# thucz/splatter360

Measured on AMD Instinct MI355X. Metric: Msplats/s fwd+bwd @1M Gaussians, 1024x512 ERP, higher is better.
Workload: dtype f32; 1 GPU; BASELINE configs[2]: 1048576 encoder-like synthetic Gaussians (seed 0, deg-4 SH, from 2 context panoramas 1024x512), 1024x512 ERP = 6 faces 256x256 + stitch, fwdbwd, L2 loss on faces (fused epilogue, scalar reduced in the backward's first launch), lean tile lists; gaussians=1048576, face=256, views_per_gpu=1, parallelism=view-sharded x1, num_rendered=2237238, visible_pairs=1096454, split_lists=auto, split_quadrants=0, wide_rectangles=0, workspace_bytes_forward=1086434304, workspace_bytes_backward=1062934272, max_instances=2862083

## Files before the change

include/s360.h:

```cpp
#ifndef S360_H
#define S360_H

#include <stddef.h>
#include <stdint.h>

#ifdef __cplusplus
extern "C" {
#endif

#define S360_ABI_VERSION 24
#define S360_MAX_VIEWS 8
#define S360_TILE 16

enum {
    S360_OK = 0,
    S360_E_BADARG = -1,
    S360_E_WORKSPACE = -2,
    S360_E_LAUNCH = -3,
    S360_E_UNSUPPORTED = -4
};

#define S360_FLAG_SHARED_CAMPOS 1u
#define S360_FLAG_FORWARD_ONLY 8u
#define S360_FLAG_COV9 2u
#define S360_FLAG_SH_CHANNEL_MAJOR 4u

#define S360_FLAG_SH_DEG4_IGNORED 16u

#define S360_FLAG_SPHERICAL 32u

#define S360_FLAG_LEAN_LISTS 64u

#define S360_FLAG_DEFER_LOSS 128u

#define S360_FLAG_ATOMIC_GRADS 256u

#define S360_FLAG_SPLIT_LISTS 512u

#define S360_FLAG_RAW_INPUTS 1024u

#define S360_FLAG_COOP_WALK 2048u

typedef struct S360View {
    float viewmatrix[16];
    float projmatrix[16];
    float campos[3];
    float tanfovx, tanfovy;
    float bg[3];
    float scale;
    float near_plane, far_plane;
    float _pad;
} S360View;

typedef struct S360Params {
    int32_t P;
    int32_t V;
    int32_t H, W;
    int32_t sh_degree;
    int32_t M;
    uint32_t flags;
    uint32_t max_instances;
    uint32_t max_segments;
    uint32_t _reserved;
    void* header_mirror;
} S360Params;

typedef struct S360Layout {
    size_t total_bytes;
    size_t header;
    size_t tiles_touched;
    size_t vis_mask;
    size_t slot_base;
    size_t rec_a;
    size_t rec_b;
    size_t rec_c;
    size_t clamped;
    size_t depths;
    size_t tile_count;
    size_t slot_ticket;
    size_t merge_done;
    size_t seg_flag;
    size_t seg_arrive;
    size_t seg_arrive2;
    size_t tile_start;
    size_t tile_cursor;
    size_t chunk_start;
    size_t tile_order;
    size_t keys;
    size_t keys_alt;
    size_t list;
    size_t final_T;
    size_t n_contrib;
    size_t tile_max_contrib;
    size_t strip_last;
    size_t slot_pair;
    size_t long_pairs;
    size_t rgbc;
    size_t sh_jac;
    size_t surv;
    size_t surv_count;
    size_t part_c;
    size_t part_t;
    size_t part_e;
    size_t part_l;
    size_t part_n;
    size_t seg_c;
    size_t seg_t;
    size_t seg_cnt;
    size_t seg_info;
    size_t geo7;
    size_t backward_bytes;
} S360Layout;

typedef struct S360RawInputs {
    const float* extrinsics;
    const float* depths;
    const float* raw_gaussians;
    const float* sh_rotation;
    int32_t n_views, per_view;
    int32_t H, W, per_ray;
    int32_t erp_convention;
    float scale_min, scale_max, eps;
} S360RawInputs;

int s360_abi_version(void);
const char* s360_error_string(int code);

int s360_layout(const S360Params* prm, S360Layout* out);

int s360_forward(const S360Params* prm, const S360View* views, const float* means3D,
                 const float* cov6, const float* opacities, const float* shs,
                 const float* colors_precomp, float* images, int32_t* radii, void* workspace,
                 size_t workspace_bytes, void* stream);

#define S360_DEPTH_DEPTH 0
#define S360_DEPTH_DISPARITY 1
#define S360_DEPTH_RELATIVE_DISPARITY 2
#define S360_DEPTH_LOG 3
int s360_forward_depth(const S360Params* prm, const S360View* views, const float* means3D,
                       const float* cov6, const float* opacities, const float* shs,
                       const float* colors_precomp, float* images, float* depth_maps, int32_t depth_mode,
                       int32_t* radii, void* workspace, size_t workspace_bytes, void* stream);

int s360_forward_mse(const S360Params* prm, const S360View* views, const float* means3D,
                     const float* cov6, const float* opacities, const float* shs,
                     const float* colors_precomp, float* images, float* depth_maps, int32_t depth_mode,
                     int32_t* radii, const float* target, float grad_scale, float* d_images, float* partials,
                     float* loss_out, void* workspace, size_t workspace_bytes, void* stream);

int s360_backward(const S360Params* prm, const S360View* views, const float* means3D,
                  const float* cov6, const float* opacities, const float* shs,
                  const float* colors_precomp, const void* workspace, size_t workspace_bytes,
                  const float* dL_dimages, const float* dL_dimages_scale,
                  const float* dL_ddepth, int32_t depth_mode, float* d_means3D, float* d_means2D,
                  float* d_cov6, float* d_opacities, float* d_shs, float* d_colors, void* bwd_workspace,
                  size_t bwd_workspace_bytes, void* stream);

int s360_backward_split(const S360Params* prm, const S360View* views, const float* means3D,
                        const float* cov6, const float* opacities, const float* shs,
                        const void* workspace, size_t workspace_bytes,
                        const float* dL_dimages, const float* dL_dimages_scale, const float* dL_ddepth,
                        int32_t depth_mode, float* d_means3D, float* d_means2D, float* d_cov6,
                        float* d_opacities, float* d_rgb_sum, void* bwd_workspace,
                        size_t bwd_workspace_bytes, void* stream);
int s360_sh_backward(const S360Params* prm, int32_t n_groups, const S360View* views,
                     const float* means3D, const float* d_rgb_sums , float* d_shs,
                     void* stream);

int s360_backward_composite(const S360Params* prm, const S360View* views, const void* workspace, size_t workspace_bytes,
                            const float* dL_dimages, const float* dL_dimages_scale, const float* dL_ddepth, int32_t depth_mode,
                            void* bwd_workspace, size_t bwd_workspace_bytes, void* stream);
int s360_backward_gaussians(const S360Params* prm, const S360View* views, const float* means3D, const float* cov6,
                            const float* shs, const void* workspace, size_t workspace_bytes, int32_t with_depth,
                            int32_t depth_mode, int32_t g_begin, int32_t g_count, int32_t rank_stamp, float* d_packed,
                            float* d_means2D, float* d_rgb_sum, void* bwd_workspace, size_t bwd_workspace_bytes, void* stream);
int s360_unpack_gradients(const float* packed, int32_t P, int32_t cov9, float* d_means3D, float* d_cov, float* d_opacities,
                          void* stream);
int s360_reduce_unpack_gradients(const float* packed_blocks, int32_t n_blocks, int32_t g_begin, int32_t g_count, int32_t cov9,
                                 float* d_means3D, float* d_cov, float* d_opacities, void* stream);

int s360_pack_views(const float* extrinsics, const float* intrinsics, const float* near_planes,
                    const float* far_planes, const float* background, int32_t background_per_view,
                    int32_t n_views, int32_t scale_invariant, S360View* views_out, void* stream);
// ... 79 lines not shown
```

splatter360_amd/_lib.py:

```python
from __future__ import annotations

import ctypes as C
import os
import shutil
import subprocess
from pathlib import Path

_PKG = Path(__file__).resolve().parent
_CSRC = _PKG / "csrc"
LIB_PATH = _PKG / "libs360.so"
SOURCES = ("s360_forward.hip", "s360_backward.hip", "s360_backward_em.hip", "s360_stitch.hip", "s360_views.hip", "s360_adapter.hip", "s360_metrics.hip",
           "s360_depth_loss.hip", "s360_eval_scores.hip", "s360_cost_volume.hip")
SOURCE_FLAGS = {"s360_backward_em.hip": ("-fno-slp-vectorize",)}
HIPCC_FLAGS = ("--offload-arch=gfx950", "-O3", "-std=c++17", "-ffp-contract=off", "-fPIC", "-Wno-unused-result")

S360_MAX_VIEWS = 8
FLAG_SHARED_CAMPOS = 1
FLAG_COV9 = 2
FLAG_SH_CHANNEL_MAJOR = 4
FLAG_FORWARD_ONLY = 8
FLAG_SH_DEG4_IGNORED = 16
FLAG_SPHERICAL = 32
FLAG_LEAN_LISTS = 64
FLAG_DEFER_LOSS = 128
FLAG_ATOMIC_GRADS = 256
FLAG_SPLIT_LISTS = 512
FLAG_RAW_INPUTS = 1024
FLAG_COOP_WALK = 2048
ABI_VERSION = 24


class S360Params(C.Structure):
    _fields_ = [("P", C.c_int32), ("V", C.c_int32), ("H", C.c_int32), ("W", C.c_int32),
                ("sh_degree", C.c_int32), ("M", C.c_int32), ("flags", C.c_uint32),
                ("max_instances", C.c_uint32), ("max_segments", C.c_uint32), ("_reserved", C.c_uint32),
                ("header_mirror", C.c_void_p)]


class S360Layout(C.Structure):
    _fields_ = [(n, C.c_size_t) for n in (
        "total_bytes", "header", "tiles_touched", "vis_mask", "slot_base", "rec_a", "rec_b", "rec_c",
        "clamped", "depths", "tile_count", "slot_ticket", "merge_done", "seg_flag", "seg_arrive", "seg_arrive2", "tile_start", "tile_cursor", "chunk_start", "tile_order", "keys", "keys_alt", "list", "final_T", "n_contrib",
        "tile_max_contrib", "strip_last", "slot_pair", "long_pairs", "rgbc", "sh_jac", "surv", "surv_count", "part_c", "part_t", "part_e", "part_l", "part_n", "seg_c", "seg_t", "seg_cnt", "seg_info", "geo7", "backward_bytes")]


class S360RawInputs(C.Structure):
    _fields_ = [("extrinsics", C.c_void_p), ("depths", C.c_void_p), ("raw_gaussians", C.c_void_p), ("sh_rotation", C.c_void_p),
                ("n_views", C.c_int32), ("per_view", C.c_int32), ("H", C.c_int32), ("W", C.c_int32), ("per_ray", C.c_int32),
                ("erp_convention", C.c_int32), ("scale_min", C.c_float), ("scale_max", C.c_float), ("eps", C.c_float)]


EXPORTS = ("s360_forward_raw", "s360_backward_raw", "s360_backward_raw_tail", "s360_abi_version", "s360_error_string", "s360_layout", "s360_forward", "s360_forward_depth", "s360_forward_mse", "s360_backward", "s360_backward_split", "s360_backward_composite", "s360_backward_gaussians", "s360_unpack_gradients", "s360_reduce_unpack_gradients", "s360_sh_backward", "s360_pack_views", "s360_adapter_forward", "s360_adapter_backward", "s360_sh_rotation_blocks",
           "s360_cube2erp_forward", "s360_cube2erp_backward", "s360_count_contributions", "s360_count_backward_slots", "s360_profile_slots", "s360_profile_slot_name",
           "s360_profile_enable", "s360_profile_collect", "s360_ssim", "s360_erode", "s360_l1_sphere_forward",
           "s360_l1_sphere_backward", "s360_depth_metrics", "s360_psnr", "s360_cost_volume_forward", "s360_cost_volume_backward",
           "s360_cost_volume_warp")


def _hipcc() -> str:
    for cand in (os.environ.get("HIPCC"), shutil.which("hipcc"), "/opt/rocm/bin/hipcc"):
        if cand and Path(cand).exists():
            return cand
    raise RuntimeError("hipcc not found; cannot build libs360.so")


def needs_build() -> bool:
    if not LIB_PATH.exists():
        return True
    t = LIB_PATH.stat().st_mtime
    return any(d.stat().st_mtime > t for d in _dep_files())


def _dep_files():
    return sorted(list(_CSRC.glob("*.hip")) + list(_CSRC.glob("*.h")) + list((_PKG.parent / "include").glob("*.h")))


def source_hash() -> str:
    import hashlib
    h = hashlib.sha256()
    for f in _dep_files():
        h.update(f.name.encode())
        h.update(f.read_bytes())
    return h.hexdigest()[:16]


def build(force: bool = False, verbose: bool = False, out: Path = None, extra=()) -> Path:
    target = LIB_PATH if out is None else Path(out)
    if out is None and not force and not needs_build():
        return LIB_PATH
    extra = [*os.environ.get("S360_HIPCC_EXTRA", "").split(), *extra]
    from concurrent.futures import ThreadPoolExecutor
    objdir = _PKG / "build" if out is None else target.parent / "build"
    objdir.mkdir(parents=True, exist_ok=True)

    def compile_one(src: str):
        obj = objdir / (src + ".o")
        cmd = [_hipcc(), *HIPCC_FLAGS, *SOURCE_FLAGS.get(src, ()), *extra, "-c", str(_CSRC / src), "-o", str(obj)]
        r = subprocess.run(cmd, capture_output=True, text=True)
        return obj, cmd, r

    with ThreadPoolExecutor(max_workers=len(SOURCES)) as pool:
        results = list(pool.map(compile_one, SOURCES))
    for obj, cmd, r in results:
        if verbose or r.returncode:
            print(" ".join(cmd))
            print(r.stdout, r.stderr)
        if r.returncode:
            raise RuntimeError("hipcc failed building libs360.so:\n" + r.stderr[-4000:])
    cmd = [_hipcc(), "--offload-arch=gfx950", "-shared", "-fPIC", *[str(o) for o, _, _ in results], "-o", str(target)]
    r = subprocess.run(cmd, capture_output=True, text=True)
    if verbose or r.returncode:
        print(" ".join(cmd))
        print(r.stdout, r.stderr)
    if r.returncode:
        raise RuntimeError("hipcc failed linking libs360.so:\n" + r.stderr[-4000:])
    return target


_lib = None


def lib() -> C.CDLL:
    global _lib
    if _lib is not None:
        return _lib
    import torch
# ... 104 lines not shown
```

splatter360_amd/csrc/s360_backward.hip:

```cpp
#include "s360_device.h"
#include "s360_prof.h"
#include "s360_bwd_em.h"
#include "s360_adapter_math.h"

#include <cstdio>
#include <cstdlib>

namespace s360 {

constexpr int GREC = 4 * PREC_F4;

__device__ __forceinline__ void slot_sum(const float4* __restrict__ part, const uint32_t* __restrict__ valid_words, uint32_t i,
                                         float* s) {
    const uint32_t vw4 = valid_words[i];
#pragma unroll
    for (int k = 0; k < 10; ++k) s[k] = 0.f;
#pragma unroll
    for (int q = 0; q < 4; ++q) {
        if ((vw4 >> (8 * q)) & 0xFFu) {
            const float4* r = part + ((size_t)i * 4 + q) * PREC_F4;
            const float4 r0 = r[0], r1 = r[1], r2 = r[2];
            s[0] += r0.x; s[1] += r0.y; s[2] += r0.z; s[3] += r0.w;
            s[4] += r1.x; s[5] += r1.y; s[6] += r1.z; s[7] += r1.w;
            s[8] += r2.x; s[9] += r2.y;
// ... 625 lines not shown
#pragma unroll
            for (int k = 0; k < 25; ++k) orec[k] = acc[k];
        }
    }
    __syncthreads();
    const int nfl = nb * RAWB_C;
    float* dst = rb.d_raw + (size_t)g0 * RAWB_C;
    if ((((uintptr_t)dst) & 15) == 0) {
        const int n4 = nfl >> 2;
        typedef float f4v __attribute__((ext_vector_type(4)));
        for (int i = tid; i < n4; i += 192) __builtin_nontemporal_store(reinterpret_cast<const f4v*>(s_out)[i], reinterpret_cast<f4v*>(dst) + i);
        for (int i = (n4 << 2) + tid; i < nfl; i += 192) dst[i] = s_out[i];
    } else {
        for (int i = tid; i < nfl; i += 192) dst[i] = s_out[i];
    }
}

}

using namespace s360;

#ifdef S360_DEBUG_LAUNCH
#define S360_LAUNCH_DIAG(e) fprintf(stderr, "s360: %s at %s:%d\n", hipGetErrorString(e), __FILE__, __LINE__)
#else
#define S360_LAUNCH_DIAG(e) ((void)0)
#endif
#define S360_CHECK_LAUNCH()                                                                          \
    do {                                                                                             \
        hipError_t e_ = hipGetLastError();                                                           \
        if (e_ != hipSuccess) {                                                                      \
            S360_LAUNCH_DIAG(e_);                                                                    \
            return S360_E_LAUNCH;                                                                    \
        }                                                                                            \
    } while (0)

static int launch_sh_bwd(const KParams& kp, const S360View* views, const float* means3D, const float4* drgb, int n_groups,
                         float* d_shs, hipStream_t st) {
    const int wblk = (kp.P + 63) / 64;
    const size_t wlds = (size_t)64 * kp.M * 3 * 4;
    if (wlds > 64 * 1024) return S360_E_UNSUPPORTED;
    ProfScope ps(PS_SH_BWD, st);
    if (kp.flags & S360_FLAG_SH_CHANNEL_MAJOR)
        hipLaunchKernelGGL((k_sh_bwd<true>), dim3(wblk), dim3(64), wlds, st, kp, views, means3D, drgb, n_groups, d_shs);
    else
        hipLaunchKernelGGL((k_sh_bwd<false>), dim3(wblk), dim3(64), wlds, st, kp, views, means3D, drgb, n_groups, d_shs);
    return S360_OK;
}

struct BwdCtx {
    KParams kp;
    S360Layout L;
    int nt;
    float4* part;
    uint32_t* valid_words;
    uint32_t* order;
    float4* pairgrad;
    uint32_t* seg_list;
    size_t n_slots;
};

static int bwd_ctx(const S360Params* prm, const void* workspace, size_t workspace_bytes, void* bwd_workspace,
                   size_t bwd_workspace_bytes, BwdCtx& c) {
    if (!prm || !workspace || !bwd_workspace) return S360_E_BADARG;
    if (prm->flags & S360_FLAG_FORWARD_ONLY) return S360_E_BADARG;
    int rc = s360_layout(prm, &c.L);
    if (rc) return rc;
    if (workspace_bytes < c.L.total_bytes || bwd_workspace_bytes < c.L.backward_bytes) return S360_E_WORKSPACE;
    KParams& kp = c.kp;
    kp.P = prm->P; kp.V = prm->V; kp.H = prm->H; kp.W = prm->W; kp.deg = s360_effective_degree(prm); kp.M = prm->M;
    kp.gx = (prm->W + 15) / 16; kp.gy = (prm->H + 15) / 16; kp.T = kp.gx * kp.gy;
    kp.flags = prm->flags; kp.cap = prm->max_instances;
    const bool sph = (kp.flags & S360_FLAG_SPHERICAL) != 0;
    if (sph && (kp.V & 1)) return S360_E_BADARG;
    c.nt = (sph ? kp.V / 2 : kp.V) * kp.T;
    if (kp.flags & S360_FLAG_ATOMIC_GRADS) {
        c.part = nullptr;
        c.valid_words = nullptr;
        c.order = (uint32_t*)bwd_workspace;
    } else {
        c.part = (float4*)bwd_workspace;
        c.valid_words = (uint32_t*)((char*)bwd_workspace + (size_t)kp.cap * 4 * GREC * 4);
        c.order = c.valid_words + kp.cap;
    }
    c.pairgrad = (float4*)((char*)(c.order + c.nt * 4) + 256 - ((uintptr_t)(c.order + c.nt * 4) & 255));
    c.seg_list = nullptr;
    c.n_slots = seg_slots_of(prm);
    if (kp.flags & S360_FLAG_SPLIT_LISTS) {
        char* e = (char*)(c.pairgrad + (size_t)kp.V * (kp.P > 0 ? kp.P : 1) * 3 + (size_t)(kp.P > 0 ? kp.P : 1));
        c.seg_list = (uint32_t*)(e + 256 - ((uintptr_t)e & 255)) + 32;
    }
    return S360_OK;
}

static int backward_composite(const BwdCtx& c, const S360View* views, const void* workspace, const float* dL_dimages,
                              const float* dL_dimages_scale, const float* dL_ddepth, int depth_mode, hipStream_t st) {
    const KParams& kp = c.kp;
    const S360Layout& L = c.L;
    const char* ws = (const char*)workspace;
    const uint32_t* header = (const uint32_t*)(ws + L.header);
    const bool with_depth = dL_ddepth != nullptr;
    const uint32_t* surv_count = (const uint32_t*)(ws + L.surv_count);
    SegBwd sb{};
    if (c.seg_list) {
        sb.seg_flag = (const uint32_t*)(ws + L.seg_flag);
        sb.chunk_start = (const uint32_t*)(ws + L.chunk_start);
        sb.seg_c = (const float4*)(ws + L.seg_c);
        sb.seg_t = (const float*)(ws + L.seg_t);
        sb.seg_cnt = (const uint32_t*)(ws + L.seg_cnt);
        sb.seg_info = (const uint2*)(ws + L.seg_info);
        sb.seg_list = c.seg_list;
        sb.n_seg_blocks = (uint32_t)min((size_t)S360_SEG_BWD_BLOCKS, c.n_slots * 4);
        sb.dbg_base = (uint32_t)c.nt * 4u;
    }
    {
        ProfScope ps(PS_ORDER, st);
        hipLaunchKernelGGL(k_order_units, dim3(1 + 512), dim3(1024), 0, st, surv_count, c.order, c.nt * 4, c.valid_words, header, kp.cap,
                           (kp.flags & S360_FLAG_ATOMIC_GRADS) ? c.pairgrad : (float4*)nullptr, (const uint8_t*)(ws + L.vis_mask), kp.P, kp.V,
                           (const uint32_t*)(ws + L.seg_cnt), (const uint32_t*)(ws + L.chunk_start), c.seg_list, (const uint2*)(ws + L.seg_info), sb);
    }
    {
        ProfScope ps(PS_RENDER_BWD, st);
        launch_render_bwd_em(with_depth, c.nt * 4, st, kp, views, (const uint32_t*)(ws + L.tile_start), (const float4*)(ws + L.surv),
                             surv_count, (const uint2*)(ws + L.slot_base), (const float*)(ws + L.depths),
                             (const float*)(ws + L.final_T), (const uint32_t*)(ws + L.n_contrib), dL_dimages, dL_dimages_scale,
                             dL_ddepth, c.part, (uint8_t*)c.valid_words, c.order, depth_mode,
                             (kp.flags & S360_FLAG_ATOMIC_GRADS) ? (float*)c.pairgrad : (float*)nullptr,
#ifdef S360_DBG_TIMING
                             (uint32_t*)(ws + L.keys_alt), c.seg_list ? &sb : (const SegBwd*)nullptr, sb.n_seg_blocks);
#else
                             (uint32_t*)nullptr, c.seg_list ? &sb : (const SegBwd*)nullptr, sb.n_seg_blocks);
#endif
    }
    S360_CHECK_LAUNCH();
    if (kp.flags & S360_FLAG_ATOMIC_GRADS) return S360_OK;
    ProfScope ps(PS_GATHER, st);
    hipLaunchKernelGGL(k_gather_slots, dim3((unsigned)(((size_t)kp.cap + S360_BLOCK - 1) / S360_BLOCK)), dim3(S360_BLOCK), 0, st,
                       kp.cap, header, (const uint32_t*)(ws + L.slot_pair), c.part, c.valid_words, c.pairgrad,
                       (const uint32_t*)(ws + L.long_pairs), (const uint2*)(ws + L.slot_base), (const uint32_t*)(ws + L.tiles_touched));
    S360_CHECK_LAUNCH();
    return S360_OK;
}

static int backward_gaussians(const BwdCtx& c, const S360View* views, const float* means3D, const float* cov6, const float* shs,
                              const void* workspace, bool with_depth, int depth_mode, int g_begin, int g_end, float* d_means3D,
                              float* d_means2D, float* d_cov6, float* d_opacities, float* d_shs, float* d_colors, float* d_rgb_sum,
                              float* d_packed, int view_stamp, hipStream_t st) {
    const KParams& kp = c.kp;
    const S360Layout& L = c.L;
    const char* ws = (const char*)workspace;
    const uint8_t* vis_mask = (const uint8_t*)(ws + L.vis_mask);
    const uint8_t* clamped = (const uint8_t*)(ws + L.clamped);
    const int dmode = with_depth ? depth_mode : -1;
    const int n = g_end - g_begin;
    if (n <= 0) return S360_OK;
    const int nblk = (n + S360_BLOCK - 1) / S360_BLOCK;
    float4* drgb = d_rgb_sum ? (float4*)d_rgb_sum : c.pairgrad + (size_t)kp.V * kp.P * 3;
    if (shs) {
        const bool shared = (kp.flags & S360_FLAG_SHARED_CAMPOS) != 0;
        if ((d_rgb_sum || d_packed) && !shared) return S360_E_UNSUPPORTED;
        if (shared) {
            {
                ProfScope ps(PS_PREPROCESS_BWD, st);
                hipLaunchKernelGGL((k_preprocess_bwd<true, false>), dim3(nblk), dim3(S360_BLOCK), 0, st, kp, views, means3D, cov6, shs,
                                   vis_mask, clamped, c.pairgrad, d_means3D, d_means2D, d_cov6, d_opacities, d_shs,
                                   d_colors, drgb, dmode, (const float*)(ws + L.sh_jac), g_begin, g_end, d_packed, view_stamp);
            }
            if (!d_rgb_sum && d_shs) {
                if (g_begin != 0 || g_end != kp.P) return S360_E_UNSUPPORTED;
                const int rc2 = launch_sh_bwd(kp, views, means3D, drgb, 1, d_shs, st);
                if (rc2) return rc2;
            }
        } else {
            if (g_begin != 0 || g_end != kp.P) return S360_E_UNSUPPORTED;
            size_t lds = (size_t)S360_BLOCK * kp.M * 3 * 4 + (size_t)S360_BLOCK * kp.V * 3 * 4;
            if (lds > 160 * 1024) return S360_E_UNSUPPORTED;
            {
                static bool attr_done[64] = {};
                int dev = 0;
                if (hipGetDevice(&dev) == hipSuccess && dev >= 0 && dev < 64 && !attr_done[dev]) {
                    (void)hipFuncSetAttribute((const void*)k_preprocess_bwd<true, true>, hipFuncAttributeMaxDynamicSharedMemorySize, 160 * 1024);
                    (void)hipGetLastError();
                    attr_done[dev] = true;
                }
            }
            ProfScope ps(PS_PREPROCESS_BWD, st);
            hipLaunchKernelGGL((k_preprocess_bwd<true, true>), dim3(nblk), dim3(S360_BLOCK), lds, st, kp, views, means3D, cov6, shs,
                               vis_mask, clamped, c.pairgrad, d_means3D, d_means2D, d_cov6, d_opacities, d_shs,
                               d_colors, (float4*)nullptr, dmode, (const float*)nullptr, 0, kp.P, (float*)nullptr, -1);
        }
    } else {
        if (d_packed) return S360_E_UNSUPPORTED;
        ProfScope ps(PS_PREPROCESS_BWD, st);
        hipLaunchKernelGGL((k_preprocess_bwd<false, false>), dim3(nblk), dim3(S360_BLOCK), 0, st, kp, views, means3D, cov6, shs,
                           vis_mask, clamped, c.pairgrad, d_means3D, d_means2D, d_cov6, d_opacities, d_shs,
                           d_colors, (float4*)nullptr, dmode, (const float*)nullptr, g_begin, g_end, (float*)nullptr, -1);
    }
    S360_CHECK_LAUNCH();
    return S360_OK;
}

static int backward_impl(const S360Params* prm, const S360View* views, const float* means3D, const float* cov6,
                         const float* opacities, const float* shs, const float* colors_precomp,
                         const void* workspace, size_t workspace_bytes, const float* dL_dimages,
                         const float* dL_dimages_scale, const float* dL_ddepth, int depth_mode, float* d_means3D,
                         float* d_means2D, float* d_cov6, float* d_opacities, float* d_shs, float* d_colors,
                         float* d_rgb_sum, void* bwd_workspace, size_t bwd_workspace_bytes, void* stream_) {
    (void)opacities;
    if (!prm || !views || !workspace || !dL_dimages || !bwd_workspace) return S360_E_BADARG;
    if (prm->flags & S360_FLAG_FORWARD_ONLY) return S360_E_BADARG;
    if (prm->P > 0 && (shs == nullptr) == (colors_precomp == nullptr)) return S360_E_BADARG;
    if (prm->P > 0 && (!means3D || !cov6 || !d_means3D || !d_cov6 || !d_opacities)) return S360_E_BADARG;
    const bool with_depth = dL_ddepth != nullptr;
    if (with_depth && (depth_mode < 0 || depth_mode > 3)) return S360_E_BADARG;
// ... 389 lines not shown
```

splatter360_amd/csrc/s360_backward_em.hip:

```cpp
#define S360_EM_KERNEL_TU 1
#include "s360_bwd_em.h"

namespace s360 {

void launch_render_bwd_em(bool with_depth, int n_units, hipStream_t st, const KParams& kp, const S360View* views,
                          const uint32_t* tile_start, const float4* surv, const uint32_t* surv_count, const uint2* slot_info,
                          const float* depths, const float* final_T, const uint32_t* n_contrib, const float* dL_dimages,
                          const float* dL_dimages_scale, const float* dL_ddepth, float4* part, uint8_t* valid, const uint32_t* order, int depth_mode,
                          float* pairgrad_atomic, uint32_t* dbg, const SegBwd* sbp_host, uint32_t n_seg_blocks) {
    const SegBwd sbv = sbp_host ? *sbp_host : SegBwd{};
#define S360_LAUNCH_BWD(WD, SG)                                                                                                              \
    hipLaunchKernelGGL((k_render_bwd_em<WD, SG>), dim3(n_units + (SG ? n_seg_blocks : 0u)), dim3(64), 0, st, kp, views, tile_start, surv, surv_count, \
                       slot_info, depths, final_T, n_contrib, dL_dimages, dL_dimages_scale, dL_ddepth, part, valid, order, depth_mode,          \
                       pairgrad_atomic, dbg, sbv, SG ? n_seg_blocks : 0u)
    const bool seg = sbp_host != nullptr;
    if (with_depth) { if (seg) S360_LAUNCH_BWD(true, true); else S360_LAUNCH_BWD(true, false); }
    else { if (seg) S360_LAUNCH_BWD(false, true); else S360_LAUNCH_BWD(false, false); }
#undef S360_LAUNCH_BWD
}

}
```

splatter360_amd/csrc/s360_bwd_em.h:

```cpp
#pragma once
#include "s360_device.h"

namespace s360 {

constexpr int EM_QCAP = 128;


#define S360_SCAN4_STEP(op, ctrl)                                                                      \
    op " %0, %0, %0 " ctrl "\n" op " %1, %1, %1 " ctrl "\n" op " %2, %2, %2 " ctrl "\n" op " %3, %3, %3 " ctrl "\n"
#define S360_SCAN4(op, a, b, c, d)                                                        \
    asm volatile("s_nop 1\n"                                                              \
                 S360_SCAN4_STEP(op, "row_shr:1 row_mask:0xf bank_mask:0xf")              \
                 S360_SCAN4_STEP(op, "row_shr:2 row_mask:0xf bank_mask:0xf")              \
                 S360_SCAN4_STEP(op, "row_shr:4 row_mask:0xf bank_mask:0xf")              \
                 S360_SCAN4_STEP(op, "row_shr:8 row_mask:0xf bank_mask:0xf")              \
                 S360_SCAN4_STEP(op, "row_bcast:15 row_mask:0xa bank_mask:0xf")           \
                 S360_SCAN4_STEP(op, "row_bcast:31 row_mask:0xc bank_mask:0xf")           \
                 "s_nop 1\n"                                                              \
                 : "+v"(a), "+v"(b), "+v"(c), "+v"(d))

__device__ __forceinline__ void wave_shr1x4_zero(float& a, float& b, float& c, float& d) {
    float oa, ob, oc, od;
    asm volatile("s_nop 1\n"
                 "v_mov_b32_dpp %0, %4 wave_shr:1 row_mask:0xf bank_mask:0xf bound_ctrl:0\n"
                 "v_mov_b32_dpp %1, %5 wave_shr:1 row_mask:0xf bank_mask:0xf bound_ctrl:0\n"
                 "v_mov_b32_dpp %2, %6 wave_shr:1 row_mask:0xf bank_mask:0xf bound_ctrl:0\n"
                 "v_mov_b32_dpp %3, %7 wave_shr:1 row_mask:0xf bank_mask:0xf bound_ctrl:0\n"
                 : "=&v"(oa), "=&v"(ob), "=&v"(oc), "=&v"(od)
                 : "v"(a), "v"(b), "v"(c), "v"(d));
    a = oa; b = ob; c = oc; d = od;
}
__device__ __forceinline__ void wave_one_minus_shr1x4(float a, float b, float c, float d, float& oa, float& ob, float& oc,
                                                      float& od) {
    const float one = 1.0f;
    asm volatile("s_nop 1\n"
                 "v_subrev_f32_dpp %0, %4, %8 wave_shr:1 row_mask:0xf bank_mask:0xf bound_ctrl:0\n"
                 "v_subrev_f32_dpp %1, %5, %8 wave_shr:1 row_mask:0xf bank_mask:0xf bound_ctrl:0\n"
                 "v_subrev_f32_dpp %2, %6, %8 wave_shr:1 row_mask:0xf bank_mask:0xf bound_ctrl:0\n"
                 "v_subrev_f32_dpp %3, %7, %8 wave_shr:1 row_mask:0xf bank_mask:0xf bound_ctrl:0\n"
                 : "=&v"(oa), "=&v"(ob), "=&v"(oc), "=&v"(od)
                 : "v"(a), "v"(b), "v"(c), "v"(d), "v"(one));
}

__device__ __forceinline__ void wave_scan4_mul(float& a, float& b, float& c, float& d) { S360_SCAN4("v_mul_f32_dpp", a, b, c, d); }
__device__ __forceinline__ void wave_scan4_add(float& a, float& b, float& c, float& d) { S360_SCAN4("v_add_f32_dpp", a, b, c, d); }

__device__ __forceinline__ float depth_value_grad(float z, float nearp, float farp, int mode) {
    if (mode == 1) return -1.0f / (z * z);
    if (mode == 2) {
        const float eps = 1e-10f;
        const float disp_near = 1.0f / (nearp + eps), disp_far = 1.0f / (farp + eps), disp = 1.0f / (z + eps);
        return (disp * disp) / (disp_near - disp_far + eps);
    }
    if (mode == 3) return (z < nearp && z > farp) ? 1.0f / z : 0.0f;
    return 1.0f;
}

typedef SegBwdPod SegBwd;

#ifdef S360_EM_KERNEL_TU
template <bool WITH_DEPTH, bool SEG>
__global__ __launch_bounds__(64) void k_render_bwd_em(
    KParams kp, const S360View* __restrict__ views, const uint32_t* __restrict__ tile_start,
    const float4* __restrict__ surv, const uint32_t* __restrict__ surv_count, const uint2* __restrict__ slot_info,
    const float* __restrict__ depths, const float* __restrict__ final_T, const uint32_t* __restrict__ n_contrib,
    const float* __restrict__ dL_dimages, const float* __restrict__ dL_dimages_scale, const float* __restrict__ dL_ddepth,
    float4* __restrict__ part,
    uint8_t* __restrict__ valid, const uint32_t* __restrict__ order, int depth_mode, float* __restrict__ pairgrad_atomic,
    uint32_t* __restrict__ dbg, SegBwd sb, uint32_t n_seg_blocks) {
    static_assert(SUB_W == 8, "entry-major backward assumes 8x8 quadrants");
    __shared__ __attribute__((aligned(16))) float s_gr[64], s_gg[64], s_gb[64], s_gd[64];
    __shared__ __attribute__((aligned(16))) float s_T[64], s_R[64];
    __shared__ __attribute__((aligned(16))) float s_B[64];
    __shared__ __attribute__((aligned(16))) uint32_t s_last[64];

    const bool seg_blk = SEG && blockIdx.x < n_seg_blocks;
    const int lane = threadIdx.x;
  for (uint32_t sj = blockIdx.x;; sj += n_seg_blocks) {
#ifdef S360_DBG_TIMING
    const long long t_begin = wall_clock64();
#endif
    uint32_t unit, n_surv, kseg = 0;
    bool split_unit = false;
    size_t sli = 0;
    if (seg_blk) {
        if (sj >= sb.seg_list[0]) return;
        uint2 info = sb.seg_info[sb.seg_list[1 + sj]];
        info.y &= ~S360_SEG_CLAIM;
        unit = 4u * info.x + (info.y & 3u);
        kseg = info.y >> 2;
        const size_t su = ((size_t)SEG_PER_CHUNK * sb.chunk_start[info.x] + kseg) * 4 + (info.y & 3u);
        n_surv = sb.seg_cnt[su];
        split_unit = true;
        sli = su * 64;
    } else {
        unit = order ? order[blockIdx.x - n_seg_blocks] : blockIdx.x - n_seg_blocks;
        n_surv = surv_count[unit];
        if (n_surv == 0) return;
        if (SEG && sb.seg_flag[unit] == 1u) {
            split_unit = true;
            sli = ((size_t)SEG_PER_CHUNK * sb.chunk_start[unit >> 2] * 4 + (unit & 3u)) * 64;
        }
    }
    const int t = (int)(unit >> 2), wave = (int)(unit & 3u);
    const int v = t / kp.T, rem = t - v * kp.T;
    const int ty = rem / kp.gx, tx = rem - ty * kp.gx;
    const int qx = tx * 16 + sub_ox(wave), qy = ty * 16 + sub_oy(wave);
    const uint32_t start = min(tile_start[t], kp.cap), end = min(tile_start[t + 1], kp.cap);
    const float4* const sv = surv + 3 * ((size_t)4 * start + (size_t)wave * (end - start) + (size_t)kseg * SEG_LEN);
    const S360View& vw = views[view_of_image(kp, v)];

    int64_t top = (int64_t)n_surv - 1;
    float4 na = make_float4(0.f, 0.f, 0.f, 0.f), nb = na, nc = na;
    if (top - lane >= 0) {
        const float4* r = sv + 3 * (size_t)(top - lane);
        na = r[0]; nb = r[1]; nc = r[2];
    }

    {
        const int px = qx + (lane & 7), py = qy + (lane >> 3);
        const size_t hw = (size_t)kp.H * kp.W;
        float4 pa = make_float4(0.f, 0.f, 0.f, 0.f), pb = make_float4(1.0f, 0.f, 0.f, 0.f);
        uint32_t last = 0;
        if (px < kp.W && py < kp.H) {
            const size_t pix = (size_t)py * kp.W + px;
            const float T_final = final_T[(size_t)v * hw + pix];
            last = n_contrib[(size_t)v * hw + pix];
            const float* dimg = dL_dimages + (size_t)v * 3 * hw;
            const float gs = dL_dimages_scale ? *dL_dimages_scale : 1.0f;
            pa.x = dimg[pix] * gs;
            pa.y = dimg[hw + pix] * gs;
            pa.z = dimg[2 * hw + pix] * gs;
            if (WITH_DEPTH) pa.w = dL_ddepth[(size_t)v * hw + pix];
            pb.x = T_final;
            pb.z = T_final * (vw.bg[0] * pa.x + vw.bg[1] * pa.y + vw.bg[2] * pa.z);
            if (SEG && split_unit) {
                const float4 cb = sb.seg_c[sli + lane];
                pb.x = sb.seg_t[sli + lane];
                float r0 = cb.z * pa.z + (cb.y * pa.y + cb.x * pa.x);
                if (WITH_DEPTH) r0 = cb.w * pa.w + r0;
                pb.y = r0;
            }
        }
        s_gr[lane] = pa.x; s_gg[lane] = pa.y; s_gb[lane] = pa.z;
        if (WITH_DEPTH) s_gd[lane] = pa.w;
        s_T[lane] = pb.x; s_R[lane] = pb.y; s_B[lane] = pb.z;
        s_last[lane] = last;
    }
    f2 pxc[4];
#pragma unroll
    for (int c = 0; c < 4; ++c) pxc[c] = f2{(float)(qx + 2 * c), (float)(qx + 2 * c + 1)};
    const float inv_scale = WITH_DEPTH ? 1.0f / vw.scale : 0.f;
    const float v_near = WITH_DEPTH ? vw.near_plane : 0.f, v_far = WITH_DEPTH ? vw.far_plane : 0.f;

#ifdef S360_DBG_TIMING
    uint32_t dbg_halves = 0;
#endif
    for (; top >= 0; top -= 64) {
        const uint32_t n = (uint32_t)(top + 1 < 64 ? top + 1 : 64);
        const float4 qa = na, qb = nb, qc = nc;
        if (top - 64 - lane >= 0) {
            const float4* r = sv + 3 * (size_t)(top - 64 - lane);
            na = r[0]; nb = r[1]; nc = r[2];
        }
        const bool lane_ok = (uint32_t)lane < n;
        const float ex = qa.x, ey = qa.y, cA = qa.z, cB = qa.w, cC = qb.x, op = qb.y, c0 = qb.z, c1 = qb.w, c2 = qc.x;
        const int erad = __float_as_int(qc.y);
        const uint32_t pos = lane_ok ? __float_as_uint(qc.z) : 0xFFFFFFFFu;
        const uint32_t pair = __float_as_uint(qc.w);
        uint2 sinfo = make_uint2(0u, 0u);
        float zv = 0.f;
        if (lane_ok) {
            if (!pairgrad_atomic) sinfo = slot_info[pair];
            if (WITH_DEPTH) zv = depth_value(depths[pair] * inv_scale, v_near, v_far, depth_mode);
        }
        const uint32_t pos_min = (uint32_t)__builtin_amdgcn_readlane((int)pos, (int)n - 1);
        f2 g_op = f2{0.f, 0.f}, X = g_op, Y = g_op, XX = g_op, XY = g_op, YY = g_op, g_r = g_op, g_g = g_op, g_b = g_op, g_z = g_op;
        bool anyc = false;
        uint32_t qmask;
        {
            const uint4 l4 = *reinterpret_cast<const uint4*>(&s_last[(lane & 15) * 4]);
            qmask = (uint32_t)__ballot(max(max(l4.x, l4.y), max(l4.z, l4.w)) > pos_min) & 0xFFFFu;
        }
        const f2 ex2 = f2{ex, ex}, cA2 = f2{cA, cA}, cB2 = f2{cB, cB}, op2 = f2{op, op}, c02 = f2{c0, c0}, c12 = f2{c1, c1},
                 c22 = f2{c2, c2}, zv2 = f2{zv, zv}, one2 = f2{1.0f, 1.0f};
#pragma unroll 1
        for (int row = 0; row < 8; ++row) {
            const float pyf = (float)(qy + row);
            const float dy = ey - pyf;
            const float cdy = cC * dy;
            const float cdy2 = cdy * dy;
            const float cdy_2 = 2.0f * cdy;
            const f2 dy2 = f2{dy, dy}, cdy2_2 = f2{cdy2, cdy2}, cdy_22 = f2{cdy_2, cdy_2};
#pragma unroll
            for (int half = 0; half < 2; ++half) {
                const int p0 = row * 8 + half * 4;
                if (!((qmask >> (row * 2 + half)) & 1u)) continue;
#ifdef S360_DBG_TIMING
                ++dbg_halves;
#endif
                const float4 vr = *reinterpret_cast<const float4*>(&s_gr[p0]), vg = *reinterpret_cast<const float4*>(&s_gg[p0]),
                             vb = *reinterpret_cast<const float4*>(&s_gb[p0]), vT = *reinterpret_cast<const float4*>(&s_T[p0]),
                             vR = *reinterpret_cast<const float4*>(&s_R[p0]), vB = *reinterpret_cast<const float4*>(&s_B[p0]);
                const uint4 vL = *reinterpret_cast<const uint4*>(&s_last[p0]);
                float4 vd = make_float4(0.f, 0.f, 0.f, 0.f);
                if (WITH_DEPTH) vd = *reinterpret_cast<const float4*>(&s_gd[p0]);
                const f2 gr[2] = {f2{vr.x, vr.y}, f2{vr.z, vr.w}}, gg[2] = {f2{vg.x, vg.y}, f2{vg.z, vg.w}},
                         gb[2] = {f2{vb.x, vb.y}, f2{vb.z, vb.w}}, gd[2] = {f2{vd.x, vd.y}, f2{vd.z, vd.w}},
                         Tr[2] = {f2{vT.x, vT.y}, f2{vT.z, vT.w}}, Rr[2] = {f2{vR.x, vR.y}, f2{vR.z, vR.w}},
                         Bg[2] = {f2{vB.x, vB.y}, f2{vB.z, vB.w}};
                const uint32_t lastk[4] = {vL.x, vL.y, vL.z, vL.w};
                f2 dx[2], pxd[2], Gm[2], a2[2];
                float a[4];
#pragma unroll
                for (int j = 0; j < 2; ++j) {
                    dx[j] = ex2 - pxc[half * 2 + j];
                    const f2 adx = cA2 * dx[j];
                    const f2 tq = pk_fma(cB2, dy2, adx);
                    pxd[j] = tq + adx;
                    const f2 pw = pk_fma(tq, dx[j], cdy2_2);
                    const f2 G = f2{__builtin_amdgcn_exp2f(pw.x), __builtin_amdgcn_exp2f(pw.y)};
                    const f2 og = op2 * G;
                    const float al0 = fminf(0.99f, og.x), al1 = fminf(0.99f, og.y);
                    const bool act0 = pos < lastk[2 * j] && !(pw.x > 0.0f) && !(al0 < 1.0f / 255.0f);
                    const bool act1 = pos < lastk[2 * j + 1] && !(pw.y > 0.0f) && !(al1 < 1.0f / 255.0f);
// ... 6 lines not shown
                float Qx[4];
                wave_one_minus_shr1x4(a[0], a[1], a[2], a[3], Qx[0], Qx[1], Qx[2], Qx[3]);
                wave_scan4_mul(Qx[0], Qx[1], Qx[2], Qx[3]);
                f2 Tj[2], rc[2], cdp[2], w[2];
                float S[4];
#pragma unroll
                for (int j = 0; j < 2; ++j) {
                    const f2 Qx2 = f2{Qx[2 * j], Qx[2 * j + 1]};
                    const f2 Q = Qx2 * (one2 - a2[j]);
                    f2 r = f2{__builtin_amdgcn_rcpf(Q.x), __builtin_amdgcn_rcpf(Q.y)};
                    r = pk_fma(pk_fma(-Q, r, one2), r, r);
                    Tj[j] = Tr[j] * r;
                    rc[j] = Qx2 * r;
                    f2 d = pk_fma(c22, gb[j], pk_fma(c12, gg[j], c02 * gr[j]));
                    if (WITH_DEPTH) d = pk_fma(zv2, gd[j], d);
                    cdp[j] = d;
                    w[j] = a2[j] * Tj[j];
                    const f2 s2 = w[j] * d;
                    S[2 * j] = s2.x;
                    S[2 * j + 1] = s2.y;
                }
                wave_scan4_add(S[0], S[1], S[2], S[3]);
                float Sx[4] = {S[0], S[1], S[2], S[3]};
                wave_shr1x4_zero(Sx[0], Sx[1], Sx[2], Sx[3]);
#pragma unroll
                for (int j = 0; j < 2; ++j) {
                    const f2 Rj = Rr[j] + f2{Sx[2 * j], Sx[2 * j + 1]};
                    const f2 dLda = pk_fma(Tj[j], cdp[j], -((Rj + Bg[j]) * rc[j]));
                    g_op = pk_fma(Gm[j], dLda, g_op);
                    const f2 h = (op2 * dLda) * Gm[j];
                    const f2 hx = h * dx[j], hy = h * dy2;
                    X = pk_fma(h, pxd[j], X);
                    Y = pk_fma(h, pk_fma(cB2, dx[j], cdy_22), Y);
                    XX = pk_fma(hx, dx[j], XX);
                    XY = pk_fma(hx, dy2, XY);
                    YY = pk_fma(hy, dy2, YY);
                    g_r = pk_fma(w[j], gr[j], g_r);
                    g_g = pk_fma(w[j], gg[j], g_g);
                    g_b = pk_fma(w[j], gb[j], g_b);
                    if (WITH_DEPTH) g_z = pk_fma(w[j], gd[j], g_z);
                }
                if (lane == 63) {
                    *reinterpret_cast<float4*>(&s_T[p0]) = make_float4(Tj[0].x, Tj[0].y, Tj[1].x, Tj[1].y);
                    *reinterpret_cast<float4*>(&s_R[p0]) = make_float4(vR.x + S[0], vR.y + S[1], vR.z + S[2], vR.w + S[3]);
                }
            }
        }
        if (pairgrad_atomic) {
            if (lane_ok && anyc) {
                const float ln2 = 0.6931471805599453f;
                float* pg = pairgrad_atomic + 12 * (size_t)pair;
                unsafeAtomicAdd(pg + 0, ln2 * (X.x + X.y));
                unsafeAtomicAdd(pg + 1, ln2 * (Y.x + Y.y));
                unsafeAtomicAdd(pg + 2, -0.5f * (XX.x + XX.y));
                unsafeAtomicAdd(pg + 3, -(XY.x + XY.y));
                unsafeAtomicAdd(pg + 4, -0.5f * (YY.x + YY.y));
                unsafeAtomicAdd(pg + 5, g_op.x + g_op.y);
                unsafeAtomicAdd(pg + 6, g_r.x + g_r.y);
                unsafeAtomicAdd(pg + 7, g_g.x + g_g.y);
                unsafeAtomicAdd(pg + 8, g_b.x + g_b.y);
                if (WITH_DEPTH) unsafeAtomicAdd(pg + 9, g_z.x + g_z.y);
            }
            continue;
        }
        uint32_t inst = 0xFFFFFFFFu;
        if (lane_ok && anyc) {
            int minx, miny, maxx, maxy;
            tile_rect(ex, ey, erad, kp.gx, kp.gy, minx, miny, maxx, maxy);
            const uint32_t idx = (uint32_t)((ty - miny) * (maxx - minx) + (tx - minx));
            const bool masked = (kp.flags & S360_FLAG_LEAN_LISTS) && (maxx - minx) * (maxy - miny) <= 32;
            inst = sinfo.x + (masked ? (uint32_t)__builtin_popcount(sinfo.y & ((1u << idx) - 1u)) : idx);
        }
        if (lane_ok && anyc && inst < kp.cap) {
            const float ln2 = 0.6931471805599453f;
            float4* o = part + ((size_t)inst * 4 + wave) * PREC_F4;
            o[0] = make_float4(ln2 * (X.x + X.y), ln2 * (Y.x + Y.y), -0.5f * (XX.x + XX.y), -(XY.x + XY.y));
            o[1] = make_float4(-0.5f * (YY.x + YY.y), g_op.x + g_op.y, g_r.x + g_r.y, g_g.x + g_g.y);
            o[2] = make_float4(g_b.x + g_b.y, g_z.x + g_z.y, 0.f, 0.f);
            valid[(size_t)inst * 4 + wave] = 1;
        }
    }
#ifdef S360_DBG_TIMING
    if (lane == 0 && dbg) {
        const size_t di = seg_blk ? (size_t)sb.dbg_base + sb.seg_list[1 + sj] : (size_t)unit;
        dbg[4 * di] = (uint32_t)t_begin;
        dbg[4 * di + 1] = (uint32_t)(wall_clock64() - t_begin);
        dbg[4 * di + 2] = n_surv;
        dbg[4 * di + 3] = (dbg_halves << 16) | min(n_surv, 65535u);
    }
#endif
    if (!SEG || !seg_blk) return;
  }
}
#endif

void launch_render_bwd_em(bool with_depth, int n_units, hipStream_t st, const KParams& kp, const S360View* views,
                          const uint32_t* tile_start, const float4* surv, const uint32_t* surv_count, const uint2* slot_info,
                          const float* depths, const float* final_T, const uint32_t* n_contrib, const float* dL_dimages,
                          const float* dL_dimages_scale, const float* dL_ddepth, float4* part, uint8_t* valid, const uint32_t* order, int depth_mode,
                          float* pairgrad_atomic, uint32_t* dbg, const SegBwd* sbp_host, uint32_t n_seg_blocks);

}
```

splatter360_amd/csrc/s360_device.h:

```cpp
#pragma once
#include <hip/hip_runtime.h>
#include <stdint.h>

#include "../../include/s360.h"

#define S360_WAVE 64
#define S360_BLOCK 256

#ifndef S360_SUB_W
#define S360_SUB_W 8
#endif

static inline int s360_effective_degree(const S360Params* prm) {
    return (prm->sh_degree > 3 && (prm->flags & S360_FLAG_SH_DEG4_IGNORED)) ? 3 : prm->sh_degree;
}

#ifndef S360_PREC_F4
#define S360_PREC_F4 4
#endif

namespace s360 {

constexpr int PREC_F4 = S360_PREC_F4;
constexpr int SUB_W = S360_SUB_W, SUB_H = 64 / S360_SUB_W;
__device__ __forceinline__ int sub_ox(int w) { return SUB_W == 16 ? 0 : 8 * (w & 1); }
__device__ __forceinline__ int sub_oy(int w) { return SUB_W == 16 ? 4 * w : 8 * (w >> 1); }


struct KParams {
    int P, V, H, W, deg, M;
    int gx, gy, T;
    uint32_t flags, cap;
};

#ifndef S360_SEG_LEN
#define S360_SEG_LEN 512
#endif
#ifndef S360_SEG_HEAD
#define S360_SEG_HEAD 1024
#endif
#ifndef S360_SEG_BWD_BLOCKS
#define S360_SEG_BWD_BLOCKS 256
#endif
#ifndef S360_SEG_MIN_REST
#define S360_SEG_MIN_REST 512
#endif
constexpr uint32_t SEG_LEN = S360_SEG_LEN, SEG_HEAD = S360_SEG_HEAD, SEG_MIN_REST = S360_SEG_MIN_REST, SEG_PER_CHUNK = 4096 / SEG_LEN;
constexpr uint32_t SEG_K0 = SEG_HEAD / SEG_LEN;
static_assert(4096 % SEG_LEN == 0 && SEG_HEAD % SEG_LEN == 0 && SEG_LEN % 64 == 0 && SEG_K0 >= 1, "segments tile the sort's 4 096-key chunks; slot 0 holds the head's state");
__device__ constexpr float SEG_T_FAR = 1.0f / 16.0f;
__host__ __device__ inline size_t seg_slots(size_t cap) { return (size_t)SEG_PER_CHUNK * (cap / 2048 + 1); }
__host__ __device__ inline size_t seg_slots_of(const S360Params* prm) {
    return prm->max_segments ? (size_t)prm->max_segments : seg_slots(prm->max_instances ? prm->max_instances : 1);
}
#define S360_HDR_SPLIT 5
#define S360_HDR_SEGWORK 6
#define S360_HDR_TILES_DONE 24
#define S360_HDR_NLONG 25
#define S360_SEG_CLAIM 0x80000000u
#define S360_HDR_SEGBUFS 32

inline int device_cu_count() {
    static int cached[64] = {};
    int dev = 0;
    if (hipGetDevice(&dev) != hipSuccess || dev < 0 || dev >= 64) return 256;
    if (!cached[dev]) {
        int n = 0;
        if (hipDeviceGetAttribute(&n, hipDeviceAttributeMultiprocessorCount, dev) != hipSuccess || n <= 0) { (void)hipGetLastError(); n = 256; }
        cached[dev] = n;
    }
    return cached[dev];
}

inline int resident_blocks(const void* fn, int block_threads, int slot) {
    static int cached[64][16] = {};
    int dev = 0;
    if (hipGetDevice(&dev) != hipSuccess || dev < 0 || dev >= 64 || slot < 0 || slot >= 16) return 4 * 256;
    if (!cached[dev][slot]) {
        int per_cu = 0;
        if (hipOccupancyMaxActiveBlocksPerMultiprocessor(&per_cu, fn, block_threads, 0) != hipSuccess || per_cu <= 0) { (void)hipGetLastError(); per_cu = 4; }
        cached[dev][slot] = per_cu * device_cu_count();
    }
    return cached[dev][slot];
}

__device__ constexpr float kC0 = 0.28209479177387814f;
__device__ constexpr float kC1 = 0.4886025119029199f;
__device__ constexpr float kC2[5] = {1.0925484305920792f, -1.0925484305920792f, 0.31539156525252005f,
                                     -1.0925484305920792f, 0.5462742152960396f};
__device__ constexpr float kC3[7] = {-0.5900435899266435f, 2.890611442640554f, -0.4570457994644658f,
                                     0.3731763325901154f, -0.4570457994644658f, 1.445305721320277f,
                                     -0.5900435899266435f};
__device__ constexpr float kC4[9] = {2.5033429417967046f, -1.7701307697799304f, 0.9461746957575601f,
                                     -0.6690465435572892f, 0.10578554691520431f, -0.6690465435572892f,
                                     0.47308734787878004f, -1.7701307697799304f, 0.6258357354491761f};

__device__ __forceinline__ void sh_basis(int deg, float x, float y, float z, float* Y) {
    Y[0] = kC0;
    if (deg > 0) {
        Y[1] = -kC1 * y;
        Y[2] = kC1 * z;
        Y[3] = -kC1 * x;
        if (deg > 1) {
            float xx = x * x, yy = y * y, zz = z * z, xy = x * y, yz = y * z, xz = x * z;
            Y[4] = kC2[0] * xy;
            Y[5] = kC2[1] * yz;
            Y[6] = kC2[2] * (2.0f * zz - xx - yy);
            Y[7] = kC2[3] * xz;
            Y[8] = kC2[4] * (xx - yy);
            if (deg > 2) {
                Y[9] = kC3[0] * y * (3.0f * xx - yy);
                Y[10] = kC3[1] * xy * z;
                Y[11] = kC3[2] * y * (4.0f * zz - xx - yy);
                Y[12] = kC3[3] * z * (2.0f * zz - 3.0f * xx - 3.0f * yy);
                Y[13] = kC3[4] * x * (4.0f * zz - xx - yy);
                Y[14] = kC3[5] * z * (xx - yy);
                Y[15] = kC3[6] * x * (xx - 3.0f * yy);
                if (deg > 3) {
                    Y[16] = kC4[0] * xy * (xx - yy);
                    Y[17] = kC4[1] * yz * (3.0f * xx - yy);
                    Y[18] = kC4[2] * xy * (7.0f * zz - 1.0f);
                    Y[19] = kC4[3] * yz * (7.0f * zz - 3.0f);
                    Y[20] = kC4[4] * (zz * (35.0f * zz - 30.0f) + 3.0f);
                    Y[21] = kC4[5] * xz * (7.0f * zz - 3.0f);
                    Y[22] = kC4[6] * (xx - yy) * (7.0f * zz - 1.0f);
                    Y[23] = kC4[7] * xz * (xx - 3.0f * yy);
                    Y[24] = kC4[8] * (xx * (xx - 3.0f * yy) - yy * (3.0f * xx - yy));
                }
            }
        }
    }
}

__device__ __forceinline__ void sh_basis_grad(int deg, float x, float y, float z, float* dx, float* dy,
                                              float* dz) {
#pragma unroll
    for (int k = 0; k < 25; ++k) dx[k] = dy[k] = dz[k] = 0.0f;
    if (deg > 0) {
        dy[1] = -kC1;
        dz[2] = kC1;
        dx[3] = -kC1;
        if (deg > 1) {
// ... 271 lines not shown

__device__ __forceinline__ float depth_value(float z, float nearp, float farp, int mode) {
    if (mode == 1) return 1.0f / z;
    if (mode == 2) {
        const float eps = 1e-10f;
        const float disp_near = 1.0f / (nearp + eps), disp_far = 1.0f / (farp + eps), disp = 1.0f / (z + eps);
        return 1.0f - (disp - disp_far) / (disp_near - disp_far + eps);
    }
    if (mode == 3) return __logf(fmaxf(fminf(z, nearp), farp));
    return z;
}

__device__ __forceinline__ void tile_rect(float px, float py, int radius, int gx, int gy, int& minx, int& miny,
                                          int& maxx, int& maxy) {
    const float rr = (float)radius;
    minx = min(gx, max(0, (int)((px - rr) / 16.0f)));
    miny = min(gy, max(0, (int)((py - rr) / 16.0f)));
    maxx = min(gx, max(0, (int)((px + rr + 15.0f) / 16.0f)));
    maxy = min(gy, max(0, (int)((py + rr + 15.0f) / 16.0f)));
}

__device__ __forceinline__ float rl(float v, int l) {
    return __int_as_float(__builtin_amdgcn_readlane(__float_as_int(v), l));
}

__device__ __forceinline__ float wave_sum1_lane63(float a) {
    asm volatile(
        "s_nop 1\n"
        "v_add_f32_dpp %0, %0, %0 quad_perm:[1,0,3,2] row_mask:0xf bank_mask:0xf\n"
        "s_nop 1\n"
        "v_add_f32_dpp %0, %0, %0 quad_perm:[2,3,0,1] row_mask:0xf bank_mask:0xf\n"
        "s_nop 1\n"
        "v_add_f32_dpp %0, %0, %0 row_half_mirror row_mask:0xf bank_mask:0xf\n"
        "s_nop 1\n"
        "v_add_f32_dpp %0, %0, %0 row_mirror row_mask:0xf bank_mask:0xf\n"
        "s_nop 1\n"
        "v_add_f32_dpp %0, %0, %0 row_bcast:15 row_mask:0xa bank_mask:0xf\n"
        "s_nop 1\n"
        "v_add_f32_dpp %0, %0, %0 row_bcast:31 row_mask:0xc bank_mask:0xf\n"
        "s_nop 1\n"
        : "+v"(a));
    return a;
}

__device__ __forceinline__ uint32_t wave_max_u32(uint32_t v) {
#pragma unroll
    for (int o = 32; o > 0; o >>= 1) v = max(v, (uint32_t)__shfl_xor((int)v, o));
    return v;
}

__device__ __forceinline__ int lane_id() { return threadIdx.x & 63; }

template <int THREADS>
__device__ __forceinline__ void order_units_body(const uint32_t* __restrict__ weight, uint32_t* __restrict__ order, int n) {
    __shared__ uint32_t s_max;
    __shared__ uint32_t s_cnt[64];
    __shared__ uint32_t s_base[64];
    if (threadIdx.x == 0) s_max = 1;
    if (threadIdx.x < 64) s_cnt[threadIdx.x] = 0;
    __syncthreads();
    uint32_t mx = 0;
    for (int i = threadIdx.x; i < n; i += THREADS) mx = max(mx, weight[i]);
    mx = wave_max_u32(mx);
    if ((threadIdx.x & 63) == 0) atomicMax(&s_max, mx);
    __syncthreads();
    const uint32_t wmax = s_max;
    for (int i = threadIdx.x; i < n; i += THREADS) atomicAdd(&s_cnt[63 - (uint32_t)(((uint64_t)weight[i] * 63) / wmax)], 1u);
    __syncthreads();
    if (threadIdx.x == 0) {
        uint32_t run = 0;
        for (int b = 0; b < 64; ++b) {
            s_base[b] = run;
            run += s_cnt[b];
        }
    }
    __syncthreads();
    for (int i = threadIdx.x; i < n; i += THREADS) {
        const uint32_t b = 63 - (uint32_t)(((uint64_t)weight[i] * 63) / wmax);
        order[atomicAdd(&s_base[b], 1u)] = (uint32_t)i;
    }
}

template <int THREADS>
__device__ __forceinline__ void order_quadrants_body(const uint32_t* __restrict__ weight, uint32_t* __restrict__ order, int nt) {
    __shared__ uint32_t s_max;
    __shared__ uint32_t s_cnt[64];
    __shared__ uint32_t s_base[64];
    if (threadIdx.x == 0) s_max = 1;
    if (threadIdx.x < 64) s_cnt[threadIdx.x] = 0;
    __syncthreads();
    uint32_t mx = 0;
    for (int i = threadIdx.x; i < nt; i += THREADS) {
        const uint4 w = reinterpret_cast<const uint4*>(weight)[i];
        mx = max(mx, max(max(w.x, w.y), max(w.z, w.w)));
    }
    mx = wave_max_u32(mx);
    if ((threadIdx.x & 63) == 0) atomicMax(&s_max, mx);
    __syncthreads();
    const uint32_t wmax = s_max;
    for (int i = threadIdx.x; i < nt; i += THREADS) {
        const uint4 w = reinterpret_cast<const uint4*>(weight)[i];
        atomicAdd(&s_cnt[63 - (uint32_t)(((uint64_t)max(max(w.x, w.y), max(w.z, w.w)) * 63) / wmax)], 1u);
    }
    __syncthreads();
    if (threadIdx.x == 0) {
        uint32_t run = 0;
        for (int b = 0; b < 64; ++b) {
            s_base[b] = run;
            run += s_cnt[b];
        }
    }
    __syncthreads();
    const uint32_t full = (uint32_t)nt / 8u * 8u, tail = (uint32_t)nt - full;
    for (int i = threadIdx.x; i < nt; i += THREADS) {
        const uint4 w = reinterpret_cast<const uint4*>(weight)[i];
        const uint32_t b = 63 - (uint32_t)(((uint64_t)max(max(w.x, w.y), max(w.z, w.w)) * 63) / wmax);
        const uint32_t r = atomicAdd(&s_base[b], 1u);
#pragma unroll
        for (uint32_t q = 0; q < 4; ++q) {
            const uint32_t slot = r < full ? (r / 8u) * 32u + q * 8u + (r & 7u) : full * 4u + q * tail + (r - full);
            order[slot] = 4u * (uint32_t)i + q;
        }
    }
}

constexpr int MSE_BLOCK = 1024;
__device__ __forceinline__ void mse_finish_body(const float* __restrict__ partials, int n_per_view, int V, float loss_scale,
                                                float inv_elems, float* __restrict__ out) {
    constexpr int VG = 8;
    __shared__ float s_w[MSE_BLOCK / 64][VG][2];
    const int lane = lane_id(), wave = threadIdx.x >> 6;
    float total = 0.f;
    for (int v0 = 0; v0 < V; v0 += VG) {
        float a[VG], b[VG];
#pragma unroll
        for (int j = 0; j < VG; ++j) a[j] = b[j] = 0.f;
        for (int i = threadIdx.x; i < n_per_view; i += MSE_BLOCK) {
            float2 q[VG];
#pragma unroll
            for (int j = 0; j < VG; ++j)
                q[j] = v0 + j < V ? reinterpret_cast<const float2*>(partials)[(size_t)(v0 + j) * n_per_view + i] : make_float2(0.f, 0.f);
#pragma unroll
            for (int j = 0; j < VG; ++j) {
                a[j] += q[j].x;
                b[j] += q[j].y;
            }
        }
#pragma unroll
        for (int j = 0; j < VG; ++j) {
#pragma unroll
            for (int o = 32; o > 0; o >>= 1) {
                a[j] += __shfl_xor(a[j], o);
                b[j] += __shfl_xor(b[j], o);
            }
            if (lane == 0) {
                s_w[wave][j][0] = a[j];
                s_w[wave][j][1] = b[j];
            }
        }
        __syncthreads();
        if (threadIdx.x == 0) {
            for (int j = 0; j < VG && v0 + j < V; ++j) {
                float sa = 0.f, sb = 0.f;
                for (int w = 0; w < MSE_BLOCK / 64; ++w) {
                    sa += s_w[w][j][0];
                    sb += s_w[w][j][1];
                }
                total += sa;
                out[1 + v0 + j] = sb * inv_elems;
            }
        }
        __syncthreads();
    }
    if (threadIdx.x == 0) out[0] = total * loss_scale;
}


#define S360_HDR_LOSS 16

struct SegBwdPod {
    const uint32_t* seg_flag;
    const uint32_t* chunk_start;
    const float4* seg_c;
    const float* seg_t;
    const uint32_t* seg_cnt;
    const uint2* seg_info;
    const uint32_t* seg_list;
    uint32_t n_seg_blocks;
    uint32_t dbg_base;
};
static_assert(sizeof(SegBwdPod) <= 32 * 4, "parked in the 32 words in front of seg_list");

static __global__ __launch_bounds__(1024) void k_order_units(const uint32_t* __restrict__ weight, uint32_t* __restrict__ order, int n,
                                                     uint32_t* __restrict__ valid_words, const uint32_t* __restrict__ header,
                                                     uint32_t cap, float4* __restrict__ pairgrad_atomic,
                                                     const uint8_t* __restrict__ vis_mask, int P, int V,
                                                     const uint32_t* __restrict__ seg_cnt, const uint32_t* __restrict__ chunk_start,
                                                     uint32_t* __restrict__ seg_list, const uint2* __restrict__ seg_info, SegBwdPod sbpod) {
    if (blockIdx.x == 2 && seg_list) {
        if (threadIdx.x == 0) *reinterpret_cast<SegBwdPod*>(seg_list - 32) = sbpod;
        __shared__ uint32_t s_n;
        if (threadIdx.x == 0) s_n = 0u;
        __syncthreads();
        const uint32_t n = header[S360_HDR_SEGWORK];
        for (uint32_t i = threadIdx.x; i < n; i += 1024) {
            uint2 w = seg_info[i];
            w.y &= ~S360_SEG_CLAIM;
            if (seg_cnt[((size_t)SEG_PER_CHUNK * chunk_start[w.x] + (w.y >> 2)) * 4 + (w.y & 3u)]) seg_list[1u + atomicAdd(&s_n, 1u)] = i;
        }
        __syncthreads();
        if (threadIdx.x == 0) seg_list[0] = s_n;
    }
    if (blockIdx.x == 1) {
        const uint64_t pp = (uint64_t)header[S360_HDR_LOSS] | ((uint64_t)header[S360_HDR_LOSS + 1] << 32);
        const uint64_t po = (uint64_t)header[S360_HDR_LOSS + 2] | ((uint64_t)header[S360_HDR_LOSS + 3] << 32);
        if (pp && po)
            mse_finish_body(reinterpret_cast<const float*>(pp), (int)header[S360_HDR_LOSS + 4], (int)header[S360_HDR_LOSS + 5],
                            __uint_as_float(header[S360_HDR_LOSS + 6]), __uint_as_float(header[S360_HDR_LOSS + 7]), reinterpret_cast<float*>(po));
    }
    if (blockIdx.x > 0) {
        const size_t stride = (size_t)(gridDim.x - 1) * 1024;
        if (pairgrad_atomic) {
            const float4 z = make_float4(0.f, 0.f, 0.f, 0.f);
            for (size_t g = (size_t)(blockIdx.x - 1) * 1024 + threadIdx.x; g < (size_t)P; g += stride)
                for (uint32_t m = vis_mask[g]; m; m &= m - 1) {
                    float4* r = pairgrad_atomic + 3 * ((size_t)__builtin_ctz(m) * P + g);
                    r[0] = z; r[1] = z; r[2] = z;
                }
            return;
        }
        const size_t nv = (size_t)min(header[0], cap);
        for (size_t i = (size_t)(blockIdx.x - 1) * 1024 + threadIdx.x; i < nv; i += stride) valid_words[i] = 0u;
        return;
    }
    if (!order) return;
    order_quadrants_body<1024>(weight, order, n / 4);
}


}
```

splatter360_amd/csrc/s360_forward.hip:

```cpp
#include "s360_device.h"
#include "s360_prof.h"
#include "s360_adapter_math.h"

#include <cstdio>
#include <cstdlib>

namespace s360 {

typedef float f4v __attribute__((ext_vector_type(4)));

template <bool CH_MAJOR, bool JAC>
__global__ __launch_bounds__(S360_BLOCK) void k_sh_eval(KParams kp, const S360View* __restrict__ views,
                                                       const float* __restrict__ means, const float* __restrict__ shs,
                                                       float4* __restrict__ rgbc, float* __restrict__ sh_jac,
                                                       uint32_t* __restrict__ zero_ptr, int zero_words) {
    const int g = blockIdx.x * S360_BLOCK + threadIdx.x;
    if (g < zero_words) zero_ptr[g] = 0u;
    if (g >= kp.P) return;
    const bool fast = kp.M == 25 && kp.deg == 4;
    const float* sh = shs + (size_t)g * kp.M * 3;
    float c[75];
    if (fast) load75(sh, c);
    const S360View& vw = views[0];
    const float sc = vw.scale;
// ... 634 lines not shown
constexpr int LDSM_E = 32;
__device__ __forceinline__ uint32_t merge_passes_of(uint32_t nch) { return nch <= 1 ? 0u : nch <= LDSM_CHUNKS ? 1u : ceil_log2_u32(nch); }

struct SegBufs {
    const uint32_t* chunk_start;
    uint32_t* seg_flag;
    uint32_t* seg_arrive;
    uint32_t* seg_arrive2;
    uint32_t n_slots;
    float4* part_c;
    float* part_t;
    float* part_e;
    uint32_t* part_l;
    uint32_t* part_n;
    float4* seg_c;
    float* seg_t;
    uint32_t* seg_cnt;
    uint2* seg_info;
    uint32_t* header;
};
static_assert(sizeof(SegBufs) <= (64 - S360_HDR_SEGBUFS) * 4, "SegBufs is parked in the workspace header");

constexpr int TS_BLOCK = 1024;
__global__ __launch_bounds__(TS_BLOCK) void k_tile_scan(const uint32_t* __restrict__ tile_count, uint32_t* __restrict__ tile_start,
                                                         uint32_t* __restrict__ tile_cursor, uint32_t* __restrict__ tile_max_contrib,
                                                         int nt, uint32_t cap, uint32_t* __restrict__ header,
                                                         uint32_t* __restrict__ chunk_start, unsigned long long* __restrict__ header_mirror,
                                                         SegBufs sg_in) {
    __shared__ uint32_t lds[TS_BLOCK / 64];
    __shared__ uint32_t lds_max, lds_nlong;
    if (threadIdx.x == 0) { lds_max = 0; lds_nlong = 0; }
    __syncthreads();
    uint32_t carry = 0, mx = 0, ccarry = 0;
    for (int b = 0; b < nt; b += 2 * TS_BLOCK) {
        const int i0 = b + 2 * (int)threadIdx.x, i1 = i0 + 1;
        uint32_t v0 = 0u, v1 = 0u;
        if (i1 < nt) {
            const uint2 vv = *reinterpret_cast<const uint2*>(tile_count + i0);
            v0 = vv.x; v1 = vv.y;
        } else if (i0 < nt) {
            v0 = tile_count[i0];
        }
        mx = max(mx, max(v0, v1));
        uint32_t tot;
        const uint32_t ex0 = block_exclusive_scan<TS_BLOCK / 64>(v0 + v1, lds, tot), ex1 = ex0 + v0;
        const uint32_t nc0 = min(carry + ex0 + v0, cap) - min(carry + ex0, cap), nc1 = min(carry + ex1 + v1, cap) - min(carry + ex1, cap);
        const uint32_t nch0 = nc0 > SORT_SHORT ? (nc0 + SORT_CHUNK - 1) / SORT_CHUNK : 0u;
        const uint32_t nch1 = nc1 > SORT_SHORT ? (nc1 + SORT_CHUNK - 1) / SORT_CHUNK : 0u;
        if (nch0 || nch1) atomicAdd(&lds_nlong, (nch0 ? 1u : 0u) + (nch1 ? 1u : 0u));
        uint32_t ctot;
        const uint32_t cex0 = block_exclusive_scan<TS_BLOCK / 64>(nch0 + nch1, lds, ctot), cex1 = cex0 + nch0;
        if (i0 < nt) {
            tile_start[i0] = carry + ex0;
            tile_cursor[i0] = 0;
            tile_max_contrib[i0] = 0;
            chunk_start[i0] = ccarry + cex0;
        }
        if (i1 < nt) {
            tile_start[i1] = carry + ex1;
            tile_cursor[i1] = 0;
            tile_max_contrib[i1] = 0;
            chunk_start[i1] = ccarry + cex1;
        }
        carry += tot;
        ccarry += ctot;
    }
    atomicMax(&lds_max, mx);
    __syncthreads();
    if (threadIdx.x == 0) {
        chunk_start[nt] = ccarry;
        tile_start[nt] = carry;
        header[0] = carry;
        header[1] = carry > cap ? 1u : 0u;
        header[2] = lds_max;
        {
            const uint32_t nmax = min(lds_max, cap);
            const uint32_t nch = nmax > SORT_SHORT ? (nmax + SORT_CHUNK - 1) / SORT_CHUNK : 0u;
            header[3] = merge_passes_of(nch);
        }
        header[4] = 0;
        *reinterpret_cast<SegBufs*>(header + S360_HDR_SEGBUFS) = sg_in;
        header[S360_HDR_SPLIT] = 0;
        header[6] = header[7] = 0;
        if (header_mirror) __hip_atomic_store(header_mirror, (unsigned long long)carry | ((unsigned long long)(carry > cap ? 1u : 0u) << 32) |
                                                             ((unsigned long long)ccarry << 33),
                                              __ATOMIC_RELAXED, __HIP_MEMORY_SCOPE_SYSTEM);
        header[S360_HDR_NLONG] = lds_nlong;
        for (int i = 8; i < 25; ++i) header[i] = 0;
    }
}

#ifndef S360_EMIT_PPT
#define S360_EMIT_PPT 4
#endif
constexpr int EMIT_PPT = S360_EMIT_PPT;

template <bool LDS_BIN, bool COOP = false>
__global__ __launch_bounds__(S360_BLOCK) void k_emit(KParams kp, const uint32_t* __restrict__ tiles_touched,
                                                    const uint8_t* __restrict__ vis_mask, const float4* __restrict__ recA, const float4* __restrict__ recC,
                                                    const float* __restrict__ depths, const uint32_t* __restrict__ tile_start,
                                                    uint32_t* __restrict__ tile_cursor, uint64_t* __restrict__ keys,
                                                    uint2* __restrict__ slot_info, uint32_t* __restrict__ slot_pair,
                                                    uint32_t* __restrict__ slot_ticket, uint32_t* __restrict__ header,
                                                    uint32_t* __restrict__ long_pairs) {
    extern __shared__ __attribute__((aligned(16))) uint32_t lds_bin[];
    __shared__ uint32_t s_scan[S360_BLOCK / 64];
    __shared__ uint32_t s_slot0;
    const int v = blockIdx.y;
    const int g0 = blockIdx.x * (S360_BLOCK * EMIT_PPT) + threadIdx.x;
    const size_t tb = (size_t)image_of_view(kp, v) * kp.T;
    uint32_t* cnt = lds_bin;
    uint32_t* base = lds_bin + kp.T;
    const bool lean = (kp.flags & S360_FLAG_LEAN_LISTS) != 0;
    if (LDS_BIN) {
        for (int i = threadIdx.x; i < kp.T; i += S360_BLOCK) cnt[i] = 0u;
        __syncthreads();
    }
    __shared__ uint32_t s_p[S360_BLOCK * EMIT_PPT];
    uint32_t vis = 0;
#pragma unroll
    for (int j = 0; j < EMIT_PPT; ++j) {
        const int g = g0 + j * S360_BLOCK;
        if (g < kp.P && ((vis_mask[g] >> v) & 1u)) vis |= 1u << j;
    }
    uint32_t nvis;
    {
        uint32_t off = block_exclusive_scan((uint32_t)__builtin_popcount(vis), s_scan, nvis);
        for (uint32_t m = vis; m; m &= m - 1) s_p[off++] = (uint32_t)v * (uint32_t)kp.P + (uint32_t)(g0 + __builtin_ctz(m) * S360_BLOCK);
    }
    __syncthreads();
    uint32_t pr[EMIT_PPT], tt[EMIT_PPT], rlo[EMIT_PPT], rhi[EMIT_PPT], dbits[EMIT_PPT], hm[EMIT_PPT];
#pragma unroll
    for (int j = 0; j < EMIT_PPT; ++j) {
        const uint32_t e = threadIdx.x + j * S360_BLOCK;
        tt[j] = 0u; pr[j] = 0u; rlo[j] = rhi[j] = dbits[j] = 0u; hm[j] = 0xFFFFFFFFu;
        if (e < nvis) {
            const uint32_t p = s_p[e];
            const float4 rc = recA[3 * (size_t)p + 2];
            const float4 ra = recA[3 * (size_t)p];
            pr[j] = p;
            tt[j] = tiles_touched[p];
            dbits[j] = __float_as_uint(depths[p]);
            int minx, miny, maxx, maxy;
            tile_rect(ra.x, ra.y, __float_as_int(rc.y), kp.gx, kp.gy, minx, miny, maxx, maxy);
            rlo[j] = (uint32_t)minx | ((uint32_t)miny << 16);
            rhi[j] = (uint32_t)maxx | ((uint32_t)maxy << 16);
            if (lean && (maxx - minx) * (maxy - miny) <= 32) hm[j] = slot_info[p].y;
        }
    }
    uint32_t sl[EMIT_PPT], ticket = 0;
#pragma unroll
    for (int j = 0; j < EMIT_PPT; ++j) sl[j] = 0u;
    if (slot_pair) {
        uint32_t carry = 0;
#pragma unroll
        for (int j = 0; j < EMIT_PPT; ++j) {
            if ((uint32_t)j * S360_BLOCK >= nvis) break;
            uint32_t tot;
            sl[j] = carry + block_exclusive_scan(tt[j], s_scan, tot);
            carry += tot;
        }
        if (threadIdx.x == 0 && carry) ticket = tile_start[tb] + atomicAdd(&slot_ticket[image_of_view(kp, v) * 64], carry);
    }
    const int lane = threadIdx.x & 63;
    if (LDS_BIN) {
#pragma unroll
// ... 655 lines not shown
                        const float test_T = T * om[e];
                        const bool stop = v && test_T < 0.0001f;
                        const bool contrib = v && !stop;
                        done = done || stop;
                        const float w = contrib ? al[e] * T : 0.0f;
                        const f2 w2 = f2{w, w};
                        C01 = C01 + rg[e] * w2;
                        if (WITH_DEPTH) C2D = C2D + bz[e] * w2;
                        else C2D.x = C2D.x + bz[e].x * w;
                        T = contrib ? test_T : T;
                        last = contrib ? posk[e] : last;
                    }
                }
            }
        } else {
            unsigned long long am = act;
            while (am) {
                const int pl = __builtin_ctzll(am);
                am &= am - 1;
                const float ppx = rl(pxf, pl), ppy = rl(pyf, pl);
                const float dx = ea.x - ppx, dy = ea.y - ppy;
                const float power = power2(ea.z, ea.w, eb.x, dx, dy);
                const float alpha = fminf(0.99f, eb.y * __builtin_amdgcn_exp2f(power));
                unsigned long long vm = __ballot(hit && !(power > 0.0f) && !(alpha < 1.0f / 255.0f));
                const bool mine = lane == pl;
                while (vm) {
                    const int eb_ = __builtin_ctzll(vm);
                    vm &= vm - 1;
                    const float a_s = rl(alpha, eb_);
                    const float test_T = T * (1.0f - a_s);
                    const bool stop = mine && test_T < 0.0001f;
                    const bool contrib = mine && !stop;
                    if (!T_ONLY) {
                        const float w = contrib ? a_s * T : 0.0f;
                        C01.x += rl(eb.z, eb_) * w;
                        C01.y += rl(eb.w, eb_) * w;
                        C2D.x += rl(ec, eb_) * w;
                        if (WITH_DEPTH) C2D.y += rl(ez, eb_) * w;
                        last = contrib ? rel + (uint32_t)eb_ + 1u : last;
                    }
                    T = contrib ? test_T : T;
                    done = done || stop;
                    if (__ballot(stop) != 0ull) break;
                }
            }
        }
    }
}

template <bool WITH_DEPTH, bool COH>
__device__ __forceinline__ void seg_item(const KParams& kp, const S360View* __restrict__ views, const uint32_t* __restrict__ tile_start,
                                         const uint32_t* __restrict__ list, const float4* __restrict__ recA, float* __restrict__ images,
                                         float* __restrict__ final_T, uint32_t* __restrict__ n_contrib, uint32_t* __restrict__ tile_max_contrib,
                                         uint32_t* __restrict__ strip_last, const float* __restrict__ depths, float* __restrict__ depth_maps,
                                         int depth_mode, const MseEp& ep, float4* __restrict__ surv, uint32_t* __restrict__ surv_count,
                                         const SegBufs& sg, int nt, uint32_t* __restrict__ dbg, const WaveLds& L, int lane, uint2 item, uint32_t wi,
                                         uint32_t nwork);

#ifndef S360_SPLIT_WAVES
#define S360_SPLIT_WAVES 4
#endif
#ifndef S360_P1_GRID
#define S360_P1_GRID 1024
#endif
#ifndef S360_P1_FIRST
#define S360_P1_FIRST 0
#endif
#ifndef S360_P2_GRID
#define S360_P2_GRID 1024
#endif
#ifndef S360_SEGS_SPINS
#define S360_SEGS_SPINS 600
#endif
template <bool WITH_DEPTH, bool SPLIT>
__global__ __launch_bounds__(S360_BLOCK) __attribute__((amdgpu_waves_per_eu(SPLIT ? S360_SPLIT_WAVES : 6, SPLIT ? S360_SPLIT_WAVES : 6))) void k_render(KParams kp, const S360View* __restrict__ views,
                                                      const uint32_t* __restrict__ tile_start, const uint32_t* __restrict__ list,
                                                      const float4* __restrict__ recA, const float4* __restrict__ recB,
                                                      const float4* __restrict__ recC, float* __restrict__ images,
                                                      float* __restrict__ final_T, uint32_t* __restrict__ n_contrib,
                                                      uint32_t* __restrict__ tile_max_contrib, uint32_t* __restrict__ strip_last,
                                                      uint32_t* __restrict__ dbg, const float* __restrict__ depths,
                                                      float* __restrict__ depth_maps, int depth_mode, MseEp ep,
                                                      const uint32_t* __restrict__ tile_order, float4* __restrict__ surv,
                                                      uint32_t* __restrict__ surv_count, uint32_t* __restrict__ hdr_loss,
                                                      const SegBufs* __restrict__ sgp, const uint32_t* __restrict__ chunk_start,
                                                      unsigned long long* __restrict__ cand_mirror, int nt, const uint32_t* __restrict__ list_all,
                                                      const float* __restrict__ depths_all) {
#ifdef S360_DBG_TIMING
    const long long t_begin = wall_clock64();
#endif
    __shared__ __attribute__((aligned(16))) float s_x[S360_BLOCK / 64][68], s_y[S360_BLOCK / 64][68], s_a[S360_BLOCK / 64][68],
        s_b[S360_BLOCK / 64][68], s_c[S360_BLOCK / 64][68], s_o[S360_BLOCK / 64][68];
    __shared__ __attribute__((aligned(16))) float2 s_rg[S360_BLOCK / 64][68], s_bz[S360_BLOCK / 64][68];
    __shared__ __attribute__((aligned(16))) uint32_t s_pos[S360_BLOCK / 64][68];
    if (hdr_loss && blockIdx.x == 0 && threadIdx.x == 0) {
        const uint64_t pp = (uint64_t)(uintptr_t)ep.partials, po = (uint64_t)(uintptr_t)ep.loss_out;
        hdr_loss[0] = (uint32_t)pp; hdr_loss[1] = (uint32_t)(pp >> 32);
        hdr_loss[2] = (uint32_t)po; hdr_loss[3] = (uint32_t)(po >> 32);
        hdr_loss[4] = (uint32_t)(kp.T * 4); hdr_loss[5] = (uint32_t)kp.V;
        hdr_loss[6] = __float_as_uint(0.5f * ep.grad_scale);
        hdr_loss[7] = __float_as_uint(1.0f / (3.0f * (float)kp.H * (float)kp.W));
        for (int i = 0; i <= kp.V; ++i) ep.loss_out[i] = __uint_as_float(0x7FC00000u);
    }
    __shared__ uint32_t s_retired;
    uint32_t tile_slot = blockIdx.x;
    if (SPLIT) {
        const SegBufs& sgr = *sgp;
        const uint32_t n_long = S360_P1_FIRST ? sgr.header[S360_HDR_NLONG] : (uint32_t)nt;
        const uint32_t b = blockIdx.x;
        if (b >= n_long && b < n_long + (uint32_t)S360_P1_GRID) {
            const SegBufs sg = sgr;
            const int pwave = threadIdx.x >> 6, lane = threadIdx.x & 63;
            const WaveLds L{s_x[pwave], s_y[pwave], s_a[pwave], s_b[pwave], s_c[pwave], s_o[pwave], s_rg[pwave], s_bz[pwave], s_pos[pwave]};
            const uint32_t nunits = min((uint32_t)(SEG_PER_CHUNK * chunk_start[nt]), sg.n_slots);
            for (uint32_t u = b - n_long; u < nunits; u += (uint32_t)S360_P1_GRID) {
#ifdef S360_DBG_TIMING
                const long long t_p1 = wall_clock64();
#endif
                const ChunkUnit cu = chunk_unit(tile_start, chunk_start, nt, kp.cap, u / SEG_PER_CHUNK);
                const uint32_t k = cu.k * SEG_PER_CHUNK + (u % SEG_PER_CHUNK);
                if (!cu.valid || k < SEG_K0 || k * SEG_LEN >= cu.n || cu.n < SEG_HEAD + SEG_MIN_REST) continue;
                const int t1 = (int)cu.t, v1 = t1 / kp.T, rem1 = t1 - v1 * kp.T;
                const int ty1 = rem1 / kp.gx, tx1 = rem1 - ty1 * kp.gx;
                const int px1 = tx1 * 16 + sub_ox(pwave) + lane % SUB_W, py1 = ty1 * 16 + sub_oy(pwave) + lane / SUB_W;
                const bool inside1 = px1 < kp.W && py1 < kp.H;
                float T1 = 1.0f;
                f2 c01 = f2{0.f, 0.f}, c2d = f2{0.f, 0.f};
                uint32_t last1 = 0, cnt1 = 0;
                bool done1 = !inside1;
                const uint32_t b0 = cu.s + k * SEG_LEN, b1 = min(b0 + SEG_LEN, cu.s + cu.n);
                composite_segment<WITH_DEPTH, true>(list, recA, depths, cu.s, b0, b1, (float)px1, (float)py1, (float)(tx1 * 16 + sub_ox(pwave)),
                                                    (float)(ty1 * 16 + sub_oy(pwave)), lane, L, 0.f, 0.f, 0.f, depth_mode, T1, c01, c2d, last1, done1,
                                                    nullptr, cnt1);
                st_devf(sg.part_t + ((size_t)u * 4 + pwave) * 64 + lane, (done1 && inside1) ? 0.0f : T1);
                asm volatile("s_waitcnt vmcnt(0)" ::: "memory");
                if (lane == 0) __hip_atomic_fetch_add(&sg.seg_arrive[4 * t1 + pwave], 1u, __ATOMIC_RELAXED, __HIP_MEMORY_SCOPE_AGENT);
#ifdef S360_DBG_TIMING
                if (lane == 0) {
                    const size_t di = 4 * ((size_t)4 * nt + (size_t)4 * sg.n_slots + (size_t)u * 4 + pwave);
                    dbg[di] = (uint32_t)t_begin; dbg[di + 1] = (uint32_t)t_p1; dbg[di + 2] = (uint32_t)(wall_clock64() - t_p1);
                    dbg[di + 3] = ((uint32_t)t1 << 8) | k;
                }
#endif
            }
            return;
        }
        if (b >= (uint32_t)nt + (uint32_t)S360_P1_GRID) {
            const SegBufs sg = sgr;
            const int pwave = threadIdx.x >> 6, lane = threadIdx.x & 63;
            const WaveLds L{s_x[pwave], s_y[pwave], s_a[pwave], s_b[pwave], s_c[pwave], s_o[pwave], s_rg[pwave], s_bz[pwave], s_pos[pwave]};
            const uint32_t n_items_cap = sg.n_slots * 4u;
            const uint32_t stride = (S360_BLOCK / 64) * (uint32_t)S360_P2_GRID;
            uint32_t wi = (uint32_t)pwave * (uint32_t)S360_P2_GRID + (b - (uint32_t)nt - (uint32_t)S360_P1_GRID);
#ifdef S360_DBG_TIMING
            if (lane == 0) dbg[4 * ((size_t)4 * nt + (size_t)8 * sg.n_slots) + wi] = (uint32_t)t_begin;
#endif
            uint32_t spins = 0;
            while (wi < n_items_cap) {
                uint2 item = ld_dev64(sg.seg_info + wi);
                item.x = (uint32_t)__shfl((int)item.x, 0);
                item.y = (uint32_t)__shfl((int)item.y, 0);
                if (item.y == 0u) {
                    bool finished = false;
                    if ((spins & 3u) == 0u) {
                        uint32_t td = ld_dev32(sg.header + S360_HDR_TILES_DONE);
                        td = (uint32_t)__shfl((int)td, 0);
                        if (td >= (uint32_t)nt) {
                            uint32_t nw = ld_dev32(sg.header + S360_HDR_SEGWORK);
                            nw = (uint32_t)__shfl((int)nw, 0);
                            finished = wi >= nw;
                        }
                    }
                    if (finished || ++spins > (uint32_t)S360_SEGS_SPINS) break;
                    __builtin_amdgcn_s_sleep(64);
                    continue;
                }
                if (item.y & S360_SEG_CLAIM) { wi += stride; continue; }
                const int ti = (int)item.x, q = (int)(item.y & 3u);
                bool ready = (uint32_t)ti < (uint32_t)nt;
                if (ready) {
                    const uint32_t n = min(tile_start[ti + 1], kp.cap) - min(tile_start[ti], kp.cap);
                    const uint32_t need = (n + SEG_LEN - 1) / SEG_LEN - SEG_K0;
                    uint32_t w2 = 0;
                    for (;;) {
                        uint32_t got = ld_dev32(sg.seg_arrive + 4 * ti + q);
                        got = (uint32_t)__shfl((int)got, 0);
                        if (got >= need) break;
                        if (++w2 > (uint32_t)S360_SEGS_SPINS) { ready = false; break; }
                        __builtin_amdgcn_s_sleep(32);
                    }
                }
                if (!ready) break;
                uint32_t old = 0;
                if (lane == 0) old = __hip_atomic_fetch_or(reinterpret_cast<uint32_t*>(sg.seg_info + wi) + 1, S360_SEG_CLAIM, __ATOMIC_RELAXED, __HIP_MEMORY_SCOPE_AGENT);
                old = (uint32_t)__shfl((int)old, 0);
                if (!(old & S360_SEG_CLAIM))
                    seg_item<WITH_DEPTH, true>(kp, views, tile_start, list, recA, images, final_T, n_contrib, tile_max_contrib, strip_last, depths, depth_maps,
                                               depth_mode, ep, surv, surv_count, sg, nt, dbg, L, lane, item, wi, 0xFFFFFFFFu);
                wi += stride;
                spins = 0;
            }
            return;
        }
        tile_slot = b < n_long ? b : b - (uint32_t)S360_P1_GRID;
        if (threadIdx.x == 0) s_retired = 0u;
        __syncthreads();
    }
    const int t = tile_order ? (int)tile_order[tile_slot] : (int)tile_slot;
    const int v = t / kp.T, rem = t - v * kp.T;
    const int ty = rem / kp.gx, tx = rem - ty * kp.gx;
    const int wave = threadIdx.x >> 6, lane = threadIdx.x & 63;
    const int lx = sub_ox(wave) + lane % SUB_W, ly = sub_oy(wave) + lane / SUB_W;
    const int px = tx * 16 + lx, py = ty * 16 + ly;
    const bool inside = px < kp.W && py < kp.H;
    const float pxf = (float)px, pyf = (float)py;
    const float x0 = (float)(tx * 16 + sub_ox(wave)), ys0 = (float)(ty * 16 + sub_oy(wave));

    const uint32_t start = min(tile_start[t], kp.cap), end = min(tile_start[t + 1], kp.cap);
    float T = 1.0f;
    f2 C01 = f2{0.f, 0.f}, C2D = f2{0.f, 0.f};
    uint32_t last = 0;
    bool done = !inside;
    float4* const sv = surv ? surv + 3 * ((size_t)4 * start + (size_t)wave * (end - start)) : nullptr;
    uint32_t scount = 0, sv_cnt = 0, sv_rel = 0;
    unsigned long long sv_m = 0ull;
    const int vcam = view_of_image(kp, v);
    const float inv_scale = WITH_DEPTH ? 1.0f / views[vcam].scale : 0.f;
    const float v_near = WITH_DEPTH ? views[vcam].near_plane : 0.f, v_far = WITH_DEPTH ? views[vcam].far_plane : 0.f;

    uint32_t p_n1 = 0, p_n2 = 0;
    if (start + lane < end) p_n1 = list[start + lane];
    if (start + 64 + lane < end) p_n2 = list[start + 64 + lane];
    float4 na = make_float4(0.f, 0.f, 0.f, 0.f), nb = na, nc = na;
    float nz = 0.f;
    if (start + lane < end) {
        na = recA[3 * (size_t)(p_n1)];
        nb = recA[3 * (size_t)(p_n1) + 1];
        nc = recA[3 * (size_t)(p_n1) + 2];
        if (WITH_DEPTH) nz = depths[p_n1];
    }
    const uint32_t split_at = ((SPLIT || cand_mirror) && end - start >= SEG_HEAD + SEG_MIN_REST && end - start > SORT_SHORT) ? start + SEG_HEAD : 0xFFFFFFFFu;
    bool went = false;
    for (uint32_t b = start; b < end; b += 64) {
        const unsigned long long act = __ballot(!done);
        if (act == 0ull) break;
        if (b == split_at) {
            const bool far_px = !done && T >= SEG_T_FAR;
            if (__ballot(far_px) != 0ull) {
                if (cand_mirror && lane == 0) __hip_atomic_store(cand_mirror, 1ull, __ATOMIC_RELAXED, __HIP_MEMORY_SCOPE_SYSTEM);
                if (SPLIT && (SEG_PER_CHUNK * chunk_start[t] + (end - start + SEG_LEN - 1) / SEG_LEN) <= sgp->n_slots) {
                    went = true;
                    break;
                }
            }
        }
        const float4 ea = na, eb = nb;
        float ez = 0.f;
        if (WITH_DEPTH) ez = depth_value(nz * inv_scale, v_near, v_far, depth_mode);
        const float ec = nc.x, erad = nc.y, eka = nc.z, ekb = nc.w;
        const bool ev = b + lane < end;
        const uint32_t epair = p_n1;
        p_n1 = p_n2;
        if (b + 64 + lane < end) {
            na = recA[3 * (size_t)(p_n1)];
            nb = recA[3 * (size_t)(p_n1) + 1];
            nc = recA[3 * (size_t)(p_n1) + 2];
            if (WITH_DEPTH) nz = depths[p_n1];
        }
        if (b + 128 + lane < end) p_n2 = list[b + 128 + lane];

        const bool hit = ev && quadrant_hit(ea.x, ea.y, ea.z, ea.w, eb.x, eb.y, eka, ekb, x0, ys0);
        unsigned long long m = __ballot(hit);
#ifdef S360_DBG_COUNT
        {
            const unsigned long long qe = __ballot(ev);
            if (lane == 0) atomicAdd(&dbg[3], (uint32_t)__popcll(qe));
        }
#endif
        if (m == 0ull) continue;
        const uint32_t rel = b - start;
        const uint32_t rank = __builtin_amdgcn_mbcnt_hi((uint32_t)(m >> 32), __builtin_amdgcn_mbcnt_lo((uint32_t)m, 0u));
        if (sv && hit) {
            float4* o = sv + 3 * (size_t)(scount + rank);
            o[0] = ea;
            o[1] = eb;
            o[2] = make_float4(ec, erad, __uint_as_float(rel + (uint32_t)lane), __uint_as_float(epair));
        }
        if (__popcll(act) > SPARSE_PIXELS) {
            const uint32_t cnt = (uint32_t)__popcll(m);
            {
                if (hit) {
                    s_x[wave][rank] = ea.x; s_y[wave][rank] = ea.y; s_a[wave][rank] = ea.z; s_b[wave][rank] = ea.w;
                    s_c[wave][rank] = eb.x; s_o[wave][rank] = eb.y;
                    s_rg[wave][rank] = make_float2(eb.z, eb.w);
                    s_bz[wave][rank] = make_float2(ec, ez);
                    s_pos[wave][rank] = rel + (uint32_t)lane + 1u;
                }
                if (lane < 3) {
                    s_x[wave][cnt + lane] = 0.f; s_y[wave][cnt + lane] = 0.f; s_a[wave][cnt + lane] = 0.f; s_b[wave][cnt + lane] = 0.f;
                    s_c[wave][cnt + lane] = 0.f; s_o[wave][cnt + lane] = 0.f;
                    s_rg[wave][cnt + lane] = make_float2(0.f, 0.f);
                    s_bz[wave][cnt + lane] = make_float2(0.f, 0.f);
                    s_pos[wave][cnt + lane] = 0u;
                }
            }
            const f2 pxf2 = f2{pxf, pxf}, pyf2 = f2{pyf, pyf};
            for (uint32_t i = 0; i < cnt; i += 4) {
                const float4 vx = *reinterpret_cast<const float4*>(&s_x[wave][i]), vy = *reinterpret_cast<const float4*>(&s_y[wave][i]),
                             va = *reinterpret_cast<const float4*>(&s_a[wave][i]), vb = *reinterpret_cast<const float4*>(&s_b[wave][i]),
                             vc = *reinterpret_cast<const float4*>(&s_c[wave][i]), vo = *reinterpret_cast<const float4*>(&s_o[wave][i]);
                const float4 rg01 = *reinterpret_cast<const float4*>(&s_rg[wave][i]), rg23 = *reinterpret_cast<const float4*>(&s_rg[wave][i + 2]);
                const float4 bz01 = *reinterpret_cast<const float4*>(&s_bz[wave][i]), bz23 = *reinterpret_cast<const float4*>(&s_bz[wave][i + 2]);
                const uint4 vp = *reinterpret_cast<const uint4*>(&s_pos[wave][i]);
                float al[4], om[4];
                bool ok[4];
                bool any_ok = false;
#pragma unroll
                for (int j = 0; j < 2; ++j) {
                    const f2 X = j ? f2{vx.z, vx.w} : f2{vx.x, vx.y}, Y = j ? f2{vy.z, vy.w} : f2{vy.x, vy.y};
                    const f2 A = j ? f2{va.z, va.w} : f2{va.x, va.y}, B = j ? f2{vb.z, vb.w} : f2{vb.x, vb.y};
                    const f2 Cc = j ? f2{vc.z, vc.w} : f2{vc.x, vc.y}, O = j ? f2{vo.z, vo.w} : f2{vo.x, vo.y};
                    const f2 dx = X - pxf2, dy = Y - pyf2;
                    const f2 t = pk_fma(B, dy, A * dx);
                    const f2 pw = pk_fma(t, dx, (Cc * dy) * dy);
                    const f2 og = O * f2{__builtin_amdgcn_exp2f(pw.x), __builtin_amdgcn_exp2f(pw.y)};
                    al[2 * j] = fminf(0.99f, og.x);
                    al[2 * j + 1] = fminf(0.99f, og.y);
                    const f2 o2 = f2{1.0f, 1.0f} - f2{al[2 * j], al[2 * j + 1]};
                    om[2 * j] = o2.x;
                    om[2 * j + 1] = o2.y;
                    ok[2 * j] = !done && !(pw.x > 0.0f) && !(al[2 * j] < 1.0f / 255.0f);
                    ok[2 * j + 1] = !done && !(pw.y > 0.0f) && !(al[2 * j + 1] < 1.0f / 255.0f);
                    any_ok = any_ok || ok[2 * j] || ok[2 * j + 1];
                }
#ifdef S360_DBG_COUNT
                if (lane == 0) atomicAdd(&dbg[0], min(4u, cnt - i));
#endif
// ... 44 lines not shown
                    last = contrib ? rel + (uint32_t)eb_ + 1u : last;
                    done = done || stop;
                    if (__ballot(stop) != 0ull) break;
                }
            }
        }
        if (sv) {
            if (__ballot(last > rel) != 0ull) {
                sv_m = m;
                sv_cnt = scount;
                sv_rel = rel;
            }
            scount += (uint32_t)__popcll(m);
        }
    }
    if (SPLIT && went) {
        const SegBufs sg = *sgp;
        const size_t slot = (size_t)SEG_PER_CHUNK * chunk_start[t];
        const size_t li = (slot * 4 + wave) * 64 + lane;
        st_dev_f4(sg.part_c + li, make_float4(C01.x, C01.y, C2D.x, C2D.y));
        st_devf(sg.part_t + li, T);
        st_dev32(sg.part_l + li, last | (done ? 0x80000000u : 0u));
        const uint32_t wmh = wave_max_u32(inside ? last : 0u);
        const uint32_t nseg = (end - start + SEG_LEN - 1) / SEG_LEN - SEG_K0;
        uint32_t wbase = 0;
        if (lane == 0) {
            st_dev32(sg.part_n + slot * 4 + wave, scount);
            st_dev32(sg.seg_cnt + slot * 4 + wave, wmh ? sv_cnt + (uint32_t)__popcll(sv_m & ((2ull << (wmh - 1u - sv_rel)) - 1ull)) : 0u);
            st_dev32(sg.seg_flag + 4 * t + wave, 1u);
            atomicAdd(&sg.header[S360_HDR_SPLIT], 1u);
            wbase = atomicAdd(&sg.header[S360_HDR_SEGWORK], nseg);
        }
        wbase = (uint32_t)__shfl((int)wbase, 0);
        asm volatile("s_waitcnt vmcnt(0)" ::: "memory");
        for (uint32_t i = (uint32_t)lane; i < nseg; i += 64u) st_dev64(sg.seg_info + wbase + i, make_uint2((uint32_t)t, ((SEG_K0 + i) << 2) | (uint32_t)wave));
#ifdef S360_DBG_TIMING
        if (lane == 0) {
            dbg[4 * (4 * t + wave)] = (uint32_t)t_begin;
            dbg[4 * (4 * t + wave) + 1] = (uint32_t)(wall_clock64() - t_begin);
            dbg[4 * (4 * t + wave) + 2] = __builtin_amdgcn_s_getreg((31 << 11) | (0 << 6) | 4);
            dbg[4 * (4 * t + wave) + 3] = __builtin_amdgcn_s_getreg((31 << 11) | (0 << 6) | 20);
        }
#endif
        asm volatile("s_waitcnt vmcnt(0)" ::: "memory");
        if (lane == 0 && atomicAdd(&s_retired, 1u) == 3u) __hip_atomic_fetch_add(&sg.header[S360_HDR_TILES_DONE], 1u, __ATOMIC_RELAXED, __HIP_MEMORY_SCOPE_AGENT);
        return;
    }
    float sq = 0.f, sqc = 0.f;
    if (inside) {
        const S360View& vw = views[vcam];
        const size_t hw = (size_t)kp.H * kp.W;
        const size_t pix = (size_t)py * kp.W + px;
        float* img = images + (size_t)v * 3 * hw;
        const float o0 = C01.x + T * vw.bg[0], o1 = C01.y + T * vw.bg[1], o2 = C2D.x + T * vw.bg[2];
        img[pix] = o0;
        img[hw + pix] = o1;
        img[2 * hw + pix] = o2;
        if (ep.target) {
            const float* gt = ep.target + (size_t)v * 3 * hw;
            float* dg = ep.d_images + (size_t)v * 3 * hw;
            const float g0 = gt[pix], g1 = gt[hw + pix], g2 = gt[2 * hw + pix];
            const float d0 = o0 - g0, d1 = o1 - g1, d2 = o2 - g2;
            dg[pix] = ep.grad_scale * d0;
            dg[hw + pix] = ep.grad_scale * d1;
            dg[2 * hw + pix] = ep.grad_scale * d2;
            sq = d0 * d0 + d1 * d1 + d2 * d2;
            const float c0 = fminf(fmaxf(g0, 0.f), 1.f) - fminf(fmaxf(o0, 0.f), 1.f);
            const float c1 = fminf(fmaxf(g1, 0.f), 1.f) - fminf(fmaxf(o1, 0.f), 1.f);
            const float c2 = fminf(fmaxf(g2, 0.f), 1.f) - fminf(fmaxf(o2, 0.f), 1.f);
            sqc = c0 * c0 + c1 * c1 + c2 * c2;
        }
        final_T[(size_t)v * hw + pix] = T;
        n_contrib[(size_t)v * hw + pix] = last;
        if (WITH_DEPTH) depth_maps[(size_t)v * hw + pix] = C2D.y;
    }
    if (ep.target) {
        const float s0 = wave_sum1_lane63(sq), s1 = wave_sum1_lane63(sqc);
        if (lane == 63) {
            ep.partials[2 * (4 * (size_t)t + wave)] = s0;
            ep.partials[2 * (4 * (size_t)t + wave) + 1] = s1;
        }
    }
    const uint32_t wm = wave_max_u32(inside ? last : 0u);
    if (lane == 0) {
        strip_last[4 * t + wave] = wm;
        if (wm) atomicMax(&tile_max_contrib[t], wm);
        if (surv_count) surv_count[4 * t + wave] = wm ? sv_cnt + (uint32_t)__popcll(sv_m & ((2ull << (wm - 1u - sv_rel)) - 1ull)) : 0u;
    }
#ifdef S360_DBG_TIMING
    if (lane == 0) {
        dbg[4 * (4 * t + wave)] = (uint32_t)t_begin;
        dbg[4 * (4 * t + wave) + 1] = (uint32_t)(wall_clock64() - t_begin);
        dbg[4 * (4 * t + wave) + 2] = __builtin_amdgcn_s_getreg((31 << 11) | (0 << 6) | 4);
        dbg[4 * (4 * t + wave) + 3] = __builtin_amdgcn_s_getreg((31 << 11) | (0 << 6) | 20);
    }
#endif
    if (SPLIT) {
        if (lane == 0 && atomicAdd(&s_retired, 1u) == 3u)
            __hip_atomic_fetch_add(&sgp->header[S360_HDR_TILES_DONE], 1u, __ATOMIC_RELAXED, __HIP_MEMORY_SCOPE_AGENT);
    }
}


#ifndef S360_TAIL_GRID
#define S360_TAIL_GRID 1024
#endif
#ifndef S360_TAIL_WAVES
#define S360_TAIL_WAVES 4
#endif
template <bool WITH_DEPTH, bool COH>
__device__ __forceinline__ void seg_item(const KParams& kp, const S360View* __restrict__ views, const uint32_t* __restrict__ tile_start,
                                         const uint32_t* __restrict__ list, const float4* __restrict__ recA, float* __restrict__ images,
                                         float* __restrict__ final_T, uint32_t* __restrict__ n_contrib, uint32_t* __restrict__ tile_max_contrib,
                                         uint32_t* __restrict__ strip_last, const float* __restrict__ depths, float* __restrict__ depth_maps,
                                         int depth_mode, const MseEp& ep, float4* __restrict__ surv, uint32_t* __restrict__ surv_count,
                                         const SegBufs& sg, int nt, uint32_t* __restrict__ dbg, const WaveLds& L, int lane, uint2 item, uint32_t wi,
                                         uint32_t nwork) {
#ifdef S360_DBG_TIMING
        const long long t_begin = wall_clock64();
#endif
        const int t = (int)item.x, wave = (int)(item.y & 3u);
        const uint32_t k = item.y >> 2;
        if ((uint32_t)t >= (uint32_t)nt) {
            if (lane == 0 && atomicAdd(&sg.header[7], 0x10000u) == 0u) {
                sg.header[8] = item.x; sg.header[9] = item.y; sg.header[12] = wi; sg.header[13] = nwork;
            }
            return;
        }
        const uint32_t start = min(tile_start[t], kp.cap), end = min(tile_start[t + 1], kp.cap), n = end - start;
        if (k < SEG_K0 || k * SEG_LEN >= n || (COH ? ld_dev32(sg.seg_flag + 4 * t + wave) : sg.seg_flag[4 * t + wave]) != 1u) {
            if (lane == 0 && atomicAdd(&sg.header[7], 0x100u) == 0u) {
                sg.header[8] = item.x; sg.header[9] = item.y; sg.header[10] = n; sg.header[12] = wi; sg.header[13] = nwork;
            }
            return;
        }
        const size_t u = (size_t)SEG_PER_CHUNK * sg.chunk_start[t] + k;
        const int v = t / kp.T, rem = t - v * kp.T;
        const int ty = rem / kp.gx, tx = rem - ty * kp.gx;
        const int lx = sub_ox(wave) + lane % SUB_W, ly = sub_oy(wave) + lane / SUB_W;
        const int px = tx * 16 + lx, py = ty * 16 + ly;
        const bool inside = px < kp.W && py < kp.H;
        const float pxf = (float)px, pyf = (float)py;
        const float x0 = (float)(tx * 16 + sub_ox(wave)), ys0 = (float)(ty * 16 + sub_oy(wave));
        const int vcam = view_of_image(kp, v);
        const float inv_scale = WITH_DEPTH ? 1.0f / views[vcam].scale : 0.f;
        const float v_near = WITH_DEPTH ? views[vcam].near_plane : 0.f, v_far = WITH_DEPTH ? views[vcam].far_plane : 0.f;
        const uint32_t K = (n + SEG_LEN - 1) / SEG_LEN;
        const uint32_t b0 = start + k * SEG_LEN, b1 = min(b0 + SEG_LEN, end);
        const size_t slot0 = u - k;
        const size_t li0 = (slot0 * 4 + wave) * 64 + lane, li = ((size_t)u * 4 + wave) * 64 + lane;
        float T;
        bool head_done;
        {
            const uint32_t l = COH ? ld_dev32(sg.part_l + li0) : sg.part_l[li0];
            head_done = (l >> 31) != 0u || !inside;
            T = COH ? ld_devf(sg.part_t + li0) : sg.part_t[li0];
#pragma unroll 8
            for (uint32_t kk = SEG_K0; kk < k; ++kk) {
                const float* q = sg.part_t + ((slot0 + kk) * 4 + wave) * 64 + lane;
                T = T * (COH ? ld_devf(q) : *q);
            }
        }
        {
            f2 C01 = f2{0.f, 0.f}, C2D = f2{0.f, 0.f};
            uint32_t last = 0, scount = 0;
            bool done = head_done || T < 0.0001f;
            const bool live_in = !done;
            float4* const sv_unit = surv ? surv + 3 * ((size_t)4 * start + (size_t)wave * n) : nullptr;
            composite_segment<WITH_DEPTH, false>(list, recA, depths, start, b0, b1, pxf, pyf, x0, ys0, lane, L, inv_scale, v_near, v_far, depth_mode, T,
                                                 C01, C2D, last, done, sv_unit ? sv_unit + 3 * (size_t)(k * SEG_LEN) : nullptr, scount);
// ... 156 lines not shown
            dbg[di + 3] |= 0x80000000u;
        }
#endif
}

template <bool WITH_DEPTH>
__global__ __launch_bounds__(S360_BLOCK) __attribute__((amdgpu_waves_per_eu(S360_TAIL_WAVES, S360_TAIL_WAVES))) void k_render_tail(KParams kp, const S360View* __restrict__ views, const uint32_t* __restrict__ tile_start,
                                                            const uint32_t* __restrict__ list, const float4* __restrict__ recA,
                                                            float* __restrict__ images, float* __restrict__ final_T, uint32_t* __restrict__ n_contrib,
                                                            uint32_t* __restrict__ tile_max_contrib, uint32_t* __restrict__ strip_last,
                                                            const float* __restrict__ depths, float* __restrict__ depth_maps, int depth_mode, MseEp ep,
                                                            float4* __restrict__ surv, uint32_t* __restrict__ surv_count, SegBufs sg, int nt,
                                                            uint32_t* __restrict__ dbg) {
    __shared__ __attribute__((aligned(16))) float s_x[S360_BLOCK / 64][68], s_y[S360_BLOCK / 64][68], s_a[S360_BLOCK / 64][68],
        s_b[S360_BLOCK / 64][68], s_c[S360_BLOCK / 64][68], s_o[S360_BLOCK / 64][68];
    __shared__ __attribute__((aligned(16))) float2 s_rg[S360_BLOCK / 64][68], s_bz[S360_BLOCK / 64][68];
    __shared__ __attribute__((aligned(16))) uint32_t s_pos[S360_BLOCK / 64][68];
    if (sg.header[S360_HDR_SPLIT] == 0u) return;
    const int pwave = threadIdx.x >> 6, lane = threadIdx.x & 63;
    const WaveLds L{s_x[pwave], s_y[pwave], s_a[pwave], s_b[pwave], s_c[pwave], s_o[pwave], s_rg[pwave], s_bz[pwave], s_pos[pwave]};
    const uint32_t nwork = sg.header[S360_HDR_SEGWORK];
    for (uint32_t wi = (uint32_t)pwave * gridDim.x + blockIdx.x; wi < nwork; wi += (S360_BLOCK / 64) * gridDim.x) {
        uint2 item = sg.seg_info[wi];
        if (item.y & S360_SEG_CLAIM) continue;
        seg_item<WITH_DEPTH, false>(kp, views, tile_start, list, recA, images, final_T, n_contrib, tile_max_contrib, strip_last, depths, depth_maps,
                                    depth_mode, ep, surv, surv_count, sg, nt, dbg, L, lane, item, wi, nwork);
    }
}

}

using namespace s360;

static inline size_t align_up(size_t x, size_t a = 256) { return (x + a - 1) / a * a; }

extern "C" int s360_layout(const S360Params* prm, S360Layout* out) {
    if (!prm || !out) return S360_E_BADARG;
    if (prm->P < 0 || prm->V < 1 || prm->V > S360_MAX_VIEWS || prm->H < 1 || prm->W < 1) return S360_E_BADARG;
    if ((uint64_t)prm->V * (uint64_t)prm->P >= (1ull << 31)) return S360_E_BADARG;
    const size_t np = (size_t)prm->V * (size_t)(prm->P > 0 ? prm->P : 1);
    const size_t gx = (prm->W + 15) / 16, gy = (prm->H + 15) / 16;
    const size_t nt = (size_t)prm->V * gx * gy;
    const size_t cap = prm->max_instances ? prm->max_instances : 1;
    const size_t npix = (size_t)prm->V * prm->H * prm->W;
    const bool fwd_only = (prm->flags & S360_FLAG_FORWARD_ONLY) != 0;
    size_t o = 0;
    auto take = [&](size_t bytes) {
        size_t r = o;
        o = align_up(o + bytes);
        return r;
    };
    out->header = take(64 * 4);
    out->tiles_touched = take(np * 4);
    out->vis_mask = take((size_t)(prm->P > 0 ? prm->P : 1));
    out->slot_base = take(np * 8);
    out->rec_a = take(np * 48);
    out->rec_b = out->rec_a + 16;
    out->rec_c = out->rec_a + 32;
    out->clamped = take(np);
    out->depths = take(np * 4);
    out->tile_count = take(nt * 4);
    out->slot_ticket = take((size_t)prm->V * 256);
    out->merge_done = take((nt * MAX_PASSES + 1) * 4);
    out->seg_flag = take(nt * 4 * 4);
    out->seg_arrive = take(nt * 4 * 4);
    out->seg_arrive2 = take((nt * 4 + 1) * 4);
    out->tile_start = take((nt + 1) * 4);
    out->tile_cursor = take(nt * 4);
    out->chunk_start = take((nt + 1) * 4);
    out->tile_order = take(nt * 4);
    out->keys = take(cap * 8);
    out->keys_alt = take(cap * 8);
    out->list = take(cap * 4);
    out->final_T = take(npix * 4);
    out->n_contrib = take(npix * 4);
    out->tile_max_contrib = take(nt * 4);
    out->strip_last = take(nt * 4 * 4);
    out->slot_pair = take(cap * 4);
    out->long_pairs = take(fwd_only ? 16 : (cap / 32 + 1) * 4);
    out->rgbc = take((size_t)(prm->P > 0 ? prm->P : 1) * 16);
    out->sh_jac = take((size_t)(prm->P > 0 ? prm->P : 1) * 36);
    out->surv = take(fwd_only ? 16 : cap * 4 * 48);
    out->surv_count = take(nt * 4 * 4);
    {
        const bool split = (prm->flags & S360_FLAG_SPLIT_LISTS) != 0;
        const size_t ns = split ? seg_slots_of(prm) : 1, nl = ns * 4 * 64;
        out->part_c = take(nl * 16);
        out->part_t = take(nl * 4);
        out->part_e = take(nl * 4);
        out->part_l = take(nl * 4);
        out->part_n = take(ns * 4 * 4);
        out->seg_c = take(nl * 16);
        out->seg_t = take(nl * 4);
        out->seg_cnt = take(ns * 4 * 4);
        out->seg_info = take(ns * 4 * 8);
    }
    out->geo7 = take((prm->flags & S360_FLAG_RAW_INPUTS) && !fwd_only ? (size_t)(prm->P > 0 ? prm->P : 1) * 28 : 16);
    out->total_bytes = o;
    const bool atomic = (prm->flags & S360_FLAG_ATOMIC_GRADS) != 0;
    out->backward_bytes = (atomic ? 0 : align_up(cap * 4 * (size_t)(16 * S360_PREC_F4)) + align_up(cap * 4)) + align_up(nt * 4 * 4) + 512 +
                          align_up(np * 48) + align_up((size_t)(prm->P > 0 ? prm->P : 1) * 16) + 256 +
                          ((prm->flags & S360_FLAG_SPLIT_LISTS) ? align_up((seg_slots_of(prm) * 4 + 64 + 32) * 4) + 256 : 0);
    return S360_OK;
}

#ifdef S360_DEBUG_LAUNCH
#define S360_LAUNCH_DIAG(e) fprintf(stderr, "s360: %s at %s:%d\n", hipGetErrorString(e), __FILE__, __LINE__)
#else
#define S360_LAUNCH_DIAG(e) ((void)0)
#endif
#define S360_CHECK_LAUNCH()                                                                          \
    do {                                                                                             \
        hipError_t e_ = hipGetLastError();                                                           \
        if (e_ != hipSuccess) {                                                                      \
            S360_LAUNCH_DIAG(e_);                                                                    \
            return S360_E_LAUNCH;                                                                    \
        }                                                                                            \
    } while (0)

static int forward_impl(const S360Params* prm, const S360View* views, const float* means3D, const float* cov6,
                        const float* opacities, const float* shs, const float* colors_precomp, float* images,
                        float* depth_maps, int depth_mode, int32_t* radii, void* workspace, size_t workspace_bytes,
                        void* stream_, MseEp ep = MseEp{nullptr, nullptr, nullptr, 0.f, nullptr}, const RawIn* rawin = nullptr) {
    if (!prm || !views || !images || !workspace) return S360_E_BADARG;
    if (prm->P > 0 && (shs == nullptr) == (colors_precomp == nullptr)) return S360_E_BADARG;
    if (((prm->flags & S360_FLAG_RAW_INPUTS) != 0) != (rawin != nullptr)) return S360_E_BADARG;
    if (prm->P > 0 && (!means3D || !cov6 || !opacities)) return S360_E_BADARG;
    if (shs && (prm->M < 1 || prm->sh_degree < 0 || prm->sh_degree > 4 ||
                (prm->sh_degree + 1) * (prm->sh_degree + 1) > prm->M))
        return S360_E_BADARG;
    if (prm->W > 65535 * 16 || prm->H > 65535 * 16) return S360_E_UNSUPPORTED;
    S360Layout L;
    int rc = s360_layout(prm, &L);
    if (rc) return rc;
    if (workspace_bytes < L.total_bytes) return S360_E_WORKSPACE;
    hipStream_t st = (hipStream_t)stream_;
    char* ws = (char*)workspace;

    KParams kp;
    kp.P = prm->P; kp.V = prm->V; kp.H = prm->H; kp.W = prm->W; kp.deg = s360_effective_degree(prm); kp.M = prm->M;
    kp.gx = (prm->W + 15) / 16; kp.gy = (prm->H + 15) / 16; kp.T = kp.gx * kp.gy;
    kp.flags = prm->flags; kp.cap = prm->max_instances;
    const bool sph = (kp.flags & S360_FLAG_SPHERICAL) != 0;
    if (sph && (kp.V & 1)) return S360_E_BADARG;
    const int nt = (sph ? kp.V / 2 : kp.V) * kp.T;
    const size_t np = (size_t)kp.V * kp.P;

    uint32_t* header = (uint32_t*)(ws + L.header);
    uint32_t* tiles_touched = (uint32_t*)(ws + L.tiles_touched);
    uint8_t* vis_mask = (uint8_t*)(ws + L.vis_mask);
    uint2* slot_info = (uint2*)(ws + L.slot_base);
    uint32_t* slot_ticket = (uint32_t*)(ws + L.slot_ticket);
    float4* recA = (float4*)(ws + L.rec_a);
    float4* recB = (float4*)(ws + L.rec_b);
    float4* recC = (float4*)(ws + L.rec_c);
    uint8_t* clamped = (uint8_t*)(ws + L.clamped);
    float* depths = (float*)(ws + L.depths);
    uint32_t* tile_count = (uint32_t*)(ws + L.tile_count);
    uint32_t* tile_start = (uint32_t*)(ws + L.tile_start);
    uint32_t* tile_cursor = (uint32_t*)(ws + L.tile_cursor);
    uint64_t* keys = (uint64_t*)(ws + L.keys);
    uint64_t* keys_alt = (uint64_t*)(ws + L.keys_alt);
    uint32_t* chunk_start = (uint32_t*)(ws + L.chunk_start);
    uint32_t* tile_order = (uint32_t*)(ws + L.tile_order);
    uint32_t* list = (uint32_t*)(ws + L.list);
    float* final_T = (float*)(ws + L.final_T);
    uint32_t* n_contrib = (uint32_t*)(ws + L.n_contrib);
    uint32_t* tile_max_contrib = (uint32_t*)(ws + L.tile_max_contrib);
    uint32_t* strip_last = (uint32_t*)(ws + L.strip_last);

    const bool eager_sh = kp.P > 0 && shs && (kp.flags & S360_FLAG_SHARED_CAMPOS) && (!(kp.flags & S360_FLAG_FORWARD_ONLY) || kp.V >= 2 || rawin);
    const size_t zero_words_sz = (L.tile_start - L.tile_count) / 4;
    const bool fold_clear = eager_sh && zero_words_sz <= (size_t)kp.P;
    uint32_t* zero_ptr = fold_clear ? tile_count : (uint32_t*)nullptr;
    const int zero_words = fold_clear ? (int)zero_words_sz : 0;
    if (!fold_clear && hipMemsetAsync(tile_count, 0, L.tile_start - L.tile_count, st) != hipSuccess) return S360_E_LAUNCH;
    if (kp.P > 0) {
        {
        const int nblk = (kp.P + S360_BLOCK - 1) / S360_BLOCK;
        const int lds_hist = (size_t)nt * 4 <= 48 * 1024 ? 1 : ((size_t)kp.T * 4 <= 48 * 1024 ? 2 : 0);
        const size_t hist_bytes = lds_hist == 2 ? (size_t)kp.T * 4 : (size_t)nt * 4;
        const bool eager = eager_sh;
        float4* rgbc = (float4*)(ws + L.rgbc);
// ... 29 lines not shown
                                   opacities, shs, colors_precomp, radii, tiles_touched, recA, recB, recC, clamped, depths,
                                   tile_count, lds_hist, rgbc, vis_mask, slot_info);
            else if (eager)
                hipLaunchKernelGGL((k_preprocess<true, true, true>), dim3(nblk), dim3(S360_BLOCK), lds, st, kp, views, means3D, cov6,
                                   opacities, shs, colors_precomp, radii, tiles_touched, recA, recB, recC, clamped, depths,
                                   tile_count, lds_hist, rgbc, vis_mask, slot_info);
            else if (kp.flags & S360_FLAG_SH_CHANNEL_MAJOR)
                hipLaunchKernelGGL((k_preprocess<true, true>), dim3(nblk), dim3(S360_BLOCK), lds, st, kp, views, means3D, cov6,
                                   opacities, shs, colors_precomp, radii, tiles_touched, recA, recB, recC, clamped, depths,
                                   tile_count, lds_hist, rgbc, vis_mask, slot_info);
            else
                hipLaunchKernelGGL((k_preprocess<true, false>), dim3(nblk), dim3(S360_BLOCK), lds, st, kp, views, means3D, cov6,
                                   opacities, shs, colors_precomp, radii, tiles_touched, recA, recB, recC, clamped, depths,
                                   tile_count, lds_hist, rgbc, vis_mask, slot_info);
        } else {
            hipLaunchKernelGGL((k_preprocess<false, false>), dim3(nblk), dim3(S360_BLOCK), lds_hist ? hist_bytes : 0, st, kp, views,
                               means3D, cov6, opacities, shs, colors_precomp, radii, tiles_touched, recA, recB, recC, clamped,
                               depths, tile_count, lds_hist, rgbc, vis_mask, slot_info);
        }
        }
        S360_CHECK_LAUNCH();
    }
    {
        ProfScope ps(PS_TILE_SCAN, st);
        const bool split0 = kp.P > 0 && (kp.flags & S360_FLAG_SPLIT_LISTS);
        SegBufs sg0{split0 ? chunk_start : (const uint32_t*)nullptr, (uint32_t*)(ws + L.seg_flag), (uint32_t*)(ws + L.seg_arrive),
                    (uint32_t*)(ws + L.seg_arrive2), (uint32_t)seg_slots_of(prm),
                    (float4*)(ws + L.part_c), (float*)(ws + L.part_t), (float*)(ws + L.part_e), (uint32_t*)(ws + L.part_l), (uint32_t*)(ws + L.part_n),
                    (float4*)(ws + L.seg_c), (float*)(ws + L.seg_t), (uint32_t*)(ws + L.seg_cnt), (uint2*)(ws + L.seg_info), header};
        hipLaunchKernelGGL(k_tile_scan, dim3(1), dim3(TS_BLOCK), 0, st, tile_count, tile_start, tile_cursor, tile_max_contrib, nt, kp.cap, header,
                           chunk_start, (unsigned long long*)prm->header_mirror, sg0);
    }
    S360_CHECK_LAUNCH();
    if (kp.P > 0) {
        const dim3 egrid((kp.P + S360_BLOCK * EMIT_PPT - 1) / (S360_BLOCK * EMIT_PPT), kp.V);
        uint32_t* slot_pair = (kp.flags & S360_FLAG_FORWARD_ONLY) ? nullptr : (uint32_t*)(ws + L.slot_pair);
        {
        ProfScope ps(PS_EMIT, st);
        if ((size_t)kp.T * 8 <= 64 * 1024 && (kp.flags & S360_FLAG_COOP_WALK))
            hipLaunchKernelGGL((k_emit<true, true>), egrid, dim3(S360_BLOCK), (size_t)kp.T * 8, st, kp, tiles_touched, vis_mask, recA, recC,
                               depths, tile_start, tile_cursor, keys, slot_info, slot_pair, slot_ticket, header, (uint32_t*)(ws + L.long_pairs));
        else if ((size_t)kp.T * 8 <= 64 * 1024)
            hipLaunchKernelGGL(k_emit<true>, egrid, dim3(S360_BLOCK), (size_t)kp.T * 8, st, kp, tiles_touched, vis_mask, recA, recC,
                               depths, tile_start, tile_cursor, keys, slot_info, slot_pair, slot_ticket, header, (uint32_t*)(ws + L.long_pairs));
        else
            hipLaunchKernelGGL(k_emit<false>, egrid, dim3(S360_BLOCK), 0, st, kp, tiles_touched, vis_mask, recA, recC, depths, tile_start,
                               tile_cursor, keys, slot_info, slot_pair, slot_ticket, header, (uint32_t*)(ws + L.long_pairs));
        }
        S360_CHECK_LAUNCH();
        ProfScope ps(PS_SORT, st);
        {
            const size_t cap_keys = kp.cap < (uint32_t)kp.P ? kp.cap : (size_t)kp.P;
            uint32_t passes = 0;
            while (passes < MAX_PASSES && ((size_t)SORT_CHUNK << passes) < cap_keys) ++passes;
            const uint32_t global_lo = SORT_CHUNK << passes;
            const unsigned cgrid = (unsigned)min((size_t)1024, (size_t)kp.cap / SORT_CHUNK + (size_t)kp.cap / SORT_SHORT + 2);
            const size_t lds512 = (size_t)(SORT_CHUNK + SORT_CHUNK / 8) * 8;
            hipLaunchKernelGGL(k_sort_stage1, dim3(cgrid + nt + 1), dim3(SORT_THREADS), lds512, st, tile_start, chunk_start, nt, keys, keys_alt, list,
                               kp.cap, passes, cgrid, tile_count, tile_order, header,
                               prm->header_mirror ? (unsigned long long*)prm->header_mirror + 2 : (unsigned long long*)nullptr);
            if (passes > 0) {
                const unsigned mgrid = cgrid < (unsigned)S360_MERGE_GRID ? cgrid : (unsigned)S360_MERGE_GRID;
                {
                    static bool attr_done[64] = {};
                    int dev = 0;
                    if (hipGetDevice(&dev) == hipSuccess && dev >= 0 && dev < 64 && !attr_done[dev]) {
                        (void)hipFuncSetAttribute((const void*)k_merge_all, hipFuncAttributeMaxDynamicSharedMemorySize, (int)LDSM_LDS_BYTES);
                        (void)hipGetLastError();
                        attr_done[dev] = true;
                    }
                }
                hipLaunchKernelGGL(k_merge_all, dim3(mgrid), dim3(SORT_THREADS), LDSM_LDS_BYTES, st, tile_start, chunk_start, nt, keys, keys_alt, list,
                                   kp.cap, passes, header, (uint32_t*)(ws + L.merge_done), (size_t)global_lo < cap_keys ? global_lo : 0xFFFFFFFFu);
            }
        }
        S360_CHECK_LAUNCH();
    }
    {
        ProfScope ps(PS_RENDER, st);
        const dim3 rgrid(nt), rblock(S360_BLOCK);
        const bool training = !(kp.flags & S360_FLAG_FORWARD_ONLY);
        float4* surv = training ? (float4*)(ws + L.surv) : nullptr;
        uint32_t* surv_count = training ? (uint32_t*)(ws + L.surv_count) : nullptr;
#ifdef S360_DBG_TIMING
        uint32_t* dbg = (uint32_t*)keys_alt;
#else
        uint32_t* dbg = header + 8;
#endif
        const bool defer = training && kp.P > 0 && ep.target && ep.loss_out && (kp.flags & S360_FLAG_DEFER_LOSS);
        uint32_t* hdr_loss = defer ? header + S360_HDR_LOSS : nullptr;
        const bool split = kp.P > 0 && (kp.flags & S360_FLAG_SPLIT_LISTS);
        SegBufs sg{split ? chunk_start : (const uint32_t*)nullptr, (uint32_t*)(ws + L.seg_flag), (uint32_t*)(ws + L.seg_arrive),
                   (uint32_t*)(ws + L.seg_arrive2), (uint32_t)seg_slots_of(prm),
                   (float4*)(ws + L.part_c), (float*)(ws + L.part_t), (float*)(ws + L.part_e), (uint32_t*)(ws + L.part_l), (uint32_t*)(ws + L.part_n),
                   (float4*)(ws + L.seg_c), (float*)(ws + L.seg_t), (uint32_t*)(ws + L.seg_cnt), (uint2*)(ws + L.seg_info), header};
        unsigned long long* cand = prm->header_mirror ? (unsigned long long*)prm->header_mirror + 1 : nullptr;
        const SegBufs* sgp = split ? (const SegBufs*)(header + S360_HDR_SEGBUFS) : (const SegBufs*)nullptr;
        if (split && hipMemsetAsync(ws + L.seg_info, 0, seg_slots_of(prm) * 4 * 8, st) != hipSuccess) return S360_E_LAUNCH;
#define S360_LAUNCH_RENDER(WD, SP)                                                                                                         \
    hipLaunchKernelGGL((k_render<WD, SP>), SP ? dim3(nt + S360_P1_GRID + S360_P2_GRID) : rgrid, rblock, 0, st, kp, views, tile_start, list, recA, recB, recC, images, final_T, n_contrib,      \
                       tile_max_contrib, strip_last, dbg, depths, depth_maps, depth_mode, ep, kp.P > 0 ? tile_order : (const uint32_t*)nullptr, \
                       surv, surv_count, hdr_loss, sgp, chunk_start, cand, nt, list, depths)
        if (depth_maps) { if (split) S360_LAUNCH_RENDER(true, true); else S360_LAUNCH_RENDER(true, false); }
        else { if (split) S360_LAUNCH_RENDER(false, true); else S360_LAUNCH_RENDER(false, false); }
#undef S360_LAUNCH_RENDER
        if (split) {
            const unsigned tgrid = (unsigned)min((size_t)S360_TAIL_GRID, seg_slots_of(prm));
            if (depth_maps)
                hipLaunchKernelGGL(k_render_tail<true>, dim3(tgrid), rblock, 0, st, kp, views, tile_start, list, recA, images, final_T, n_contrib,
                                   tile_max_contrib, strip_last, depths, depth_maps, depth_mode, ep, surv, surv_count, sg, nt, dbg);
            else
                hipLaunchKernelGGL(k_render_tail<false>, dim3(tgrid), rblock, 0, st, kp, views, tile_start, list, recA, images, final_T, n_contrib,
                                   tile_max_contrib, strip_last, depths, depth_maps, depth_mode, ep, surv, surv_count, sg, nt, dbg);
        }
        if (ep.target && ep.loss_out && !defer)
            hipLaunchKernelGGL(k_mse_finish, dim3(1), dim3(MSE_BLOCK), 0, st, ep.partials, kp.T * 4, kp.V, 0.5f * ep.grad_scale,
                               1.0f / (3.0f * (float)kp.H * (float)kp.W), ep.loss_out);
    }
    S360_CHECK_LAUNCH();
    return S360_OK;
}

extern "C" int s360_forward(const S360Params* prm, const S360View* views, const float* means3D, const float* cov6,
                            const float* opacities, const float* shs, const float* colors_precomp, float* images,
                            int32_t* radii, void* workspace, size_t workspace_bytes, void* stream_) {
    return forward_impl(prm, views, means3D, cov6, opacities, shs, colors_precomp, images, nullptr, 0, radii, workspace,
                        workspace_bytes, stream_);
}

extern "C" int s360_forward_depth(const S360Params* prm, const S360View* views, const float* means3D, const float* cov6,
                                  const float* opacities, const float* shs, const float* colors_precomp, float* images,
                                  float* depth_maps, int32_t depth_mode, int32_t* radii, void* workspace,
                                  size_t workspace_bytes, void* stream_) {
    if (!depth_maps || depth_mode < 0 || depth_mode > 3) return S360_E_BADARG;
    return forward_impl(prm, views, means3D, cov6, opacities, shs, colors_precomp, images, depth_maps, depth_mode, radii,
                        workspace, workspace_bytes, stream_);
}

extern "C" int s360_forward_mse(const S360Params* prm, const S360View* views, const float* means3D, const float* cov6,
                                const float* opacities, const float* shs, const float* colors_precomp, float* images,
                                float* depth_maps, int32_t depth_mode, int32_t* radii, const float* target,
                                float grad_scale, float* d_images, float* partials, float* loss_out, void* workspace,
                                size_t workspace_bytes, void* stream_) {
    if (!target || !d_images || !partials) return S360_E_BADARG;
    if (depth_maps && (depth_mode < 0 || depth_mode > 3)) return S360_E_BADARG;
    return forward_impl(prm, views, means3D, cov6, opacities, shs, colors_precomp, images, depth_maps, depth_mode, radii,
                        workspace, workspace_bytes, stream_, s360::MseEp{target, d_images, partials, grad_scale, loss_out});
}

extern "C" int s360_forward_raw(const S360Params* prm, const S360View* views, const S360RawInputs* raw, const float* opacities,
                                float* means_out, float* cov6_out, float* images, float* depth_maps, int32_t depth_mode, int32_t* radii,
                                const float* target, float grad_scale, float* d_images, float* partials, float* loss_out, void* workspace,
                                size_t workspace_bytes, void* stream_) {
    if (!prm || !raw || !means_out || !cov6_out) return S360_E_BADARG;
    if (!(prm->flags & S360_FLAG_RAW_INPUTS) || !(prm->flags & S360_FLAG_SHARED_CAMPOS) || (prm->flags & (S360_FLAG_COV9 | S360_FLAG_SPHERICAL)))
        return S360_E_BADARG;
    if (prm->M != 25 || prm->sh_degree != 4) return S360_E_UNSUPPORTED;
    if (prm->P > 0 && (!raw->extrinsics || !raw->depths || !raw->raw_gaussians)) return S360_E_BADARG;
    if (raw->n_views < 0 || raw->per_view < 0 || raw->H < 1 || raw->W < 1 || raw->per_ray < 1 ||
        (long long)raw->n_views * raw->per_view != (long long)prm->P || (long long)raw->H * raw->W * raw->per_ray != (long long)raw->per_view)
        return S360_E_BADARG;
    if (raw->erp_convention < 0 || raw->erp_convention > 3 || (raw->erp_convention != 0 && (raw->H < 2 || raw->W < 2))) return S360_E_BADARG;
    if (depth_maps && (depth_mode < 0 || depth_mode > 3)) return S360_E_BADARG;
    if (target && (!d_images || !partials)) return S360_E_BADARG;
    s360::RawIn rin{raw->extrinsics, raw->depths, raw->raw_gaussians, raw->sh_rotation, means_out, cov6_out, nullptr,
                    raw->per_view > 0 ? raw->per_view : 1, raw->H, raw->W, raw->per_ray, raw->erp_convention, raw->scale_min, raw->scale_max, raw->eps};
    const float* dummy_sh = reinterpret_cast<const float*>(raw->raw_gaussians ? raw->raw_gaussians : (const float*)workspace);
    return forward_impl(prm, views, means_out, cov6_out, opacities, dummy_sh, nullptr, images, depth_maps, depth_mode, radii, workspace,
                        workspace_bytes, stream_, target ? s360::MseEp{target, d_images, partials, grad_scale, loss_out}
                                                         : s360::MseEp{nullptr, nullptr, nullptr, 0.f, nullptr}, &rin);
}
```

splatter360_amd/rasterizer.py:

```python
from __future__ import annotations

import ctypes as C
import os
from typing import NamedTuple, Optional

import torch
from torch import Tensor, nn

from . import _lib

VIEW_FLOATS = 44

SH_DEG4_IGNORED = bool(int(os.environ.get("S360_SH_DEG4_IGNORED", "0")))


class GaussianRasterizationSettings(NamedTuple):
    image_height: int
    image_width: int
    tanfovx: float
    tanfovy: float
    bg: Tensor
    scale_modifier: float
    viewmatrix: Tensor
    projmatrix: Tensor
    sh_degree: int
    campos: Tensor
    prefiltered: bool
    debug: bool


LEAN_LISTS = bool(int(os.environ.get("S360_LEAN_LISTS", "1")))

_sl = os.environ.get("S360_SPLIT_LISTS", "auto")
if _sl not in ("auto", "0", "1"):
    raise RuntimeError(f"S360_SPLIT_LISTS must be 'auto', '0' or '1', got {_sl!r}")
SPLIT_LONG_LISTS = "auto" if _sl == "auto" else bool(int(_sl))

DETERMINISTIC = bool(int(os.environ.get("S360_DETERMINISTIC", "0")))

LAZY_SHRINK = bool(int(os.environ.get("S360_LAZY_SHRINK", "0")))

ATOMIC_GRADS = bool(int(os.environ.get("S360_ATOMIC_GRADS", "0")))

DROPIN_CHECK = os.environ.get("S360_DROPIN_CHECK", "sync")
if DROPIN_CHECK not in ("sync", "lazy"):
    raise RuntimeError(f"S360_DROPIN_CHECK must be 'sync' or 'lazy', got {DROPIN_CHECK!r}")

DEPTH_MODES = {"depth": 0, "disparity": 1, "relative_disparity": 2, "log": 3}


def pack_views(viewmatrix: Tensor, projmatrix: Tensor, campos: Tensor, tanfovx, tanfovy, bg: Tensor,
               scale=1.0, near=0.0, far=0.0) -> Tensor:
    vm = viewmatrix.reshape(-1, 16).float()
    v = vm.shape[0]
    dev = vm.device
    pm = projmatrix.reshape(-1, 16).float().to(dev)
    cp = campos.reshape(-1, 3).float().to(dev)
    b = bg.reshape(-1, 3).float().to(dev).expand(v, 3)

    def col(t):
        if isinstance(t, Tensor):
            return t.reshape(-1, 1).float().to(dev).expand(v, 1)
        return torch.full((v, 1), float(t), dtype=torch.float32, device=dev)

    pad = torch.zeros((v, 1), dtype=torch.float32, device=dev)
    return torch.cat([vm, pm, cp.expand(v, 3), col(tanfovx), col(tanfovy), b, col(scale), col(near), col(far), pad],
                     dim=1).contiguous()


def pack_views_native(extrinsics: Tensor, intrinsics: Tensor, near: Tensor, far: Tensor, background: Tensor,
                      scale_invariant: bool = True) -> Tensor:
    ext = _f32c(extrinsics, "extrinsics").reshape(-1, 4, 4)
    n = int(ext.shape[0])
    dev = ext.device
    k = _f32c(intrinsics, "intrinsics").reshape(-1, 3, 3)
    nr = _f32c(near, "near").reshape(-1).expand(n).contiguous()
    fr = _f32c(far, "far").reshape(-1).expand(n).contiguous()
    bg = background.detach().float().to(dev).contiguous()
    per_view = bg.dim() == 2 and int(bg.shape[0]) == n
    if not per_view and bg.numel() != 3:
        raise RuntimeError(f"background must be [3] or [{n},3], got {tuple(bg.shape)}")
    if int(k.shape[0]) != n:
        raise RuntimeError("extrinsics / intrinsics view counts differ")
    out = torch.empty((n, VIEW_FLOATS), dtype=torch.float32, device=dev)
    with torch.cuda.device(dev):
        stream = C.c_void_p(torch.cuda.current_stream(dev).cuda_stream)
        rc = _lib.lib().s360_pack_views(_ptr(ext), _ptr(k), _ptr(nr), _ptr(fr), _ptr(bg), int(bool(per_view)), n,
                                        int(bool(scale_invariant)), _ptr(out), stream)
    _lib.check(rc, "s360_pack_views")
    return out


def pack_views_spherical(pano_c2w: Tensor, background: Tensor, scale=1.0, near=0.0, far=0.0) -> Tensor:
    c2w = pano_c2w.reshape(-1, 4, 4).float().clone()
    n = c2w.shape[0]
    dev = c2w.device
    sc = scale if isinstance(scale, Tensor) else torch.full((n,), float(scale), device=dev)
    sc = sc.reshape(-1).float().to(dev).expand(n)
    c2w[:, :3, 3] = c2w[:, :3, 3] * sc[:, None]
    vm = torch.linalg.inv_ex(c2w, check_errors=False).inverse.transpose(1, 2).contiguous()
    one = torch.ones(n, device=dev)
    v = pack_views(vm, torch.eye(4, device=dev).expand(n, 4, 4), c2w[:, :3, 3], one, one, background, scale=sc, near=near, far=far)
    return v.repeat_interleave(2, dim=0).contiguous()


_CAPACITY_HINT: dict = {}


def _hint_key(dev, p: int, v: int, h: int, w: int, lean: bool):
    d = torch.device(dev) if dev is not None else None
    return (None if d is None else (d.type, d.index), p, v, h, w, bool(lean))


_MIRRORS: dict = {}


def _mirror(key) -> Tensor:
    m = _MIRRORS.get(key)
    if m is None:
        m = torch.tensor([-1, 0, -1], dtype=torch.int64).pin_memory()
        _MIRRORS[key] = m
    return m


def _poll_mirror(key, warn: bool = True) -> None:
    m = _MIRRORS.get(key)
    if m is None:
        return
    word = int(m[0])
# ... 31 lines not shown
def coop_decision(key, mode=None) -> bool:
    mode = COOP_WALK if mode is None else mode
    if mode is True or mode is False:
        return mode
    m = _MIRRORS.get(key)
    return m is not None and int(m[2]) >= AUTO_COOP_MIN_PAIRS


AUTO_SPLIT_MAX_WAVES = 24576


def split_decision(key, mode, quadrant_waves: int = 0) -> bool:
    if mode is True or mode is False:
        return mode
    if quadrant_waves > AUTO_SPLIT_MAX_WAVES:
        return False
    if DETERMINISTIC:
        return True
    m = _MIRRORS.get(key)
    if m is not None and int(m[1]) != 0:
        m[1] = 0
        _SPLIT_AGE[key] = 0
    else:
        _SPLIT_AGE[key] = _SPLIT_AGE.get(key, 1 << 30) + 1
    return _SPLIT_AGE[key] <= 16


def default_segments(key) -> int:
    c = _CHUNK_HINT.get(key)
    return 0 if (c is None or DETERMINISTIC) else SEG_PER_CHUNK * (2 * c + 64)


def default_capacity(p: int, v: int, h: int = 0, w: int = 0, *, device=None, lean: bool = False, lazy: bool = False) -> int:
    first = (3 * p * v) // 2 + (1 << 18)
    guess = first
    key = _hint_key(device, p, v, h, w, lean)
    if lazy:
        _poll_mirror(key)
    hint = _CAPACITY_HINT.get(key)
    if hint is not None:
        guess = hint + hint // 4 + (1 << 16)
        if lazy and (DETERMINISTIC or not LAZY_SHRINK):
            guess = max(guess, first)
    return int(min(2**32 - 1, max(1 << 16, guess)))


class RasterState:

    def __init__(self, prm: _lib.S360Params, lay: _lib.S360Layout, workspace: Tensor):
        self.prm, self.layout, self.workspace = prm, lay, workspace

    def _arr(self, off: int, count: int, dtype: torch.dtype) -> Tensor:
        nbytes = count * torch.empty((), dtype=dtype).element_size()
        return self.workspace[off:off + nbytes].view(dtype)

    def header(self) -> Tensor:
        return self._arr(self.layout.header, 64, torch.int32)

    def tensors(self) -> dict:
        p, l = self.prm, self.layout
        npair = p.V * p.P
        gx, gy = (p.W + 15) // 16, (p.H + 15) // 16
        nt = p.V * gx * gy
        cap = p.max_instances
        return dict(
            header=self.header(),
            tiles_touched=self._tiles_touched(),
            vis_mask=self._arr(l.vis_mask, p.P, torch.uint8),
            slot_base=self._arr(l.slot_base, 2 * npair, torch.int32).view(p.V, p.P, 2)[..., 0],
            hit_mask=self._arr(l.slot_base, 2 * npair, torch.int32).view(p.V, p.P, 2)[..., 1],
            slot_pair=self._arr(l.slot_pair, cap, torch.int32),
            rec_a=self._arr(l.rec_a, npair * 12, torch.float32).view(p.V, p.P, 12)[..., 0:4],
            rec_b=self._arr(l.rec_a, npair * 12, torch.float32).view(p.V, p.P, 12)[..., 4:8],
            rec_c=self._arr(l.rec_a, npair * 12, torch.float32).view(p.V, p.P, 12)[..., 8:12],
            clamped=self._arr(l.clamped, npair, torch.uint8).view(p.V, p.P),
            depths=self._arr(l.depths, npair, torch.float32).view(p.V, p.P),
            tile_count=self._arr(l.tile_count, nt, torch.int32),
            tile_start=self._arr(l.tile_start, nt + 1, torch.int32),
            keys=self._arr(l.keys, cap, torch.int64),
            list=self._arr(l.list, cap, torch.int32),
            final_T=self._arr(l.final_T, p.V * p.H * p.W, torch.float32).view(p.V, p.H, p.W),
            n_contrib=self._arr(l.n_contrib, p.V * p.H * p.W, torch.int32).view(p.V, p.H, p.W),
            tile_max_contrib=self._arr(l.tile_max_contrib, nt, torch.int32),
            seg_flag=self._arr(l.seg_flag, nt * 4, torch.int32),
        )

    def _tiles_touched(self) -> Tensor:
        p, l = self.prm, self.layout
        raw = self._arr(l.tiles_touched, p.V * p.P, torch.int32).view(p.V, p.P)
        vis = self._arr(l.vis_mask, p.P, torch.uint8).to(torch.int32)
        bits = (vis[None, :] >> torch.arange(p.V, device=vis.device, dtype=torch.int32)[:, None]) & 1
        return torch.where(bits.bool(), raw, torch.zeros_like(raw))

    def _read_header(self):
        h = self.header()[:2].cpu()
        n, over = int(h[0]) & 0xFFFFFFFF, bool(int(h[1]))
        p = self.prm
        key = _hint_key(self.workspace.device, p.P, p.V, p.H, p.W, bool(p.flags & _lib.FLAG_LEAN_LISTS))
        _CAPACITY_HINT[key] = max(n, _CAPACITY_HINT.get(key, 0))
        _poll_mirror(key, warn=False)
        return n, over

    def count_contributions(self):
        out = torch.zeros(2, dtype=torch.int64, device=self.workspace.device)
        with torch.cuda.device(self.workspace.device):
            stream = C.c_void_p(torch.cuda.current_stream(self.workspace.device).cuda_stream)
            _lib.check(_lib.lib().s360_count_contributions(C.byref(self.prm), _ptr(self.workspace), self.layout.total_bytes, _ptr(out), stream),
                       "s360_count_contributions")
        a, b = out.cpu().tolist()
        return int(a), int(b)

    def count_backward_slots(self) -> dict:
        out = torch.zeros(32, dtype=torch.int64, device=self.workspace.device)
        with torch.cuda.device(self.workspace.device):
            stream = C.c_void_p(torch.cuda.current_stream(self.workspace.device).cuda_stream)
            _lib.check(_lib.lib().s360_count_backward_slots(C.byref(self.prm), _ptr(self.workspace), self.layout.total_bytes, _ptr(out), stream),
                       "s360_count_backward_slots")
        c = [int(x) for x in out.cpu().tolist()]
        return dict(executed=c[0], padding=c[1], stopped=c[2], miss=c[3], contributing=c[4], skipped_runs=c[5], units=c[6], groups=c[7],
                    by_unit_hit_decile=c[8:18], runs_by_active_records=dict(zip(("0", "1-4", "5-8", "9-16", "17-24", "25-32", "33-48", "49-64"), c[18:26])),
                    records=c[29], reach_upper_half=c[26], reach_lower_half=c[27], reach_both_halves=c[28], half_wave_iterations=c[30])

    def split_errors(self) -> int:
        return int(self.header()[7].item())

    def mopup_items(self) -> int:
        n = int(self.header()[6].item())
        if n == 0:
            return 0
        second = self._arr(self.layout.seg_info, 2 * n, torch.int32).view(n, 2)[:, 1].to(torch.int64)
        return int(((second & 0x80000000) == 0).sum().item())

    def num_rendered(self) -> int:
        return self._read_header()[0]

    def overflowed(self) -> bool:
        return self._read_header()[1]


def _ptr(t: Optional[Tensor]):
    return None if t is None else C.c_void_p(t.data_ptr())


def _f32c(t: Tensor, name: str) -> Tensor:
    if not t.is_cuda:
        raise RuntimeError(f"{name} must live on the GPU (hip device); the rasteriser has no CPU path")
    return t.detach().float().contiguous()


def _forward_call(prm, views, means3D, cov6, opac, shs, colors, want_radii: bool, depth_mode=None, mse=None):
    lay = _lib.layout(prm)
    dev = means3D.device
    ws = torch.empty(lay.total_bytes, dtype=torch.uint8, device=dev)
    n_img = prm.V // 2 if (prm.flags & _lib.FLAG_SPHERICAL) else prm.V
    images = torch.empty((n_img, 3, prm.H, prm.W), dtype=torch.float32, device=dev)
    radii = torch.empty((prm.V, prm.P), dtype=torch.int32, device=dev) if want_radii else None
    stream = C.c_void_p(torch.cuda.current_stream(dev).cuda_stream)
    depth = None
    if mse is not None:
        target, grad_scale = mse
        if depth_mode is not None:
            depth = torch.empty((prm.V, prm.H, prm.W), dtype=torch.float32, device=dev)
        d_images = torch.empty_like(images)
        nquads = prm.V * ((prm.H + 15) // 16) * ((prm.W + 15) // 16) * 4
        partials = torch.empty((nquads, 2), dtype=torch.float32, device=dev)
        loss_out = torch.empty((1 + prm.V,), dtype=torch.float32, device=dev)
        rc = _lib.lib().s360_forward_mse(C.byref(prm), _ptr(views), _ptr(means3D), _ptr(cov6), _ptr(opac), _ptr(shs),
                                         _ptr(colors), _ptr(images), _ptr(depth), DEPTH_MODES.get(depth_mode, 0), _ptr(radii),
                                         _ptr(target), C.c_float(grad_scale), _ptr(d_images), _ptr(partials), _ptr(loss_out),
                                         _ptr(ws), lay.total_bytes, stream)
        _lib.check(rc, "s360_forward_mse")
        st = RasterState(prm, lay, ws)
        st.d_images, st.mse_partials, st.mse_out = d_images, partials, loss_out
        return images, radii, st, depth
    if depth_mode is None:
        rc = _lib.lib().s360_forward(C.byref(prm), _ptr(views), _ptr(means3D), _ptr(cov6), _ptr(opac), _ptr(shs),
                                     _ptr(colors), _ptr(images), _ptr(radii), _ptr(ws), lay.total_bytes, stream)
    else:
        depth = torch.empty((n_img, prm.H, prm.W), dtype=torch.float32, device=dev)
        rc = _lib.lib().s360_forward_depth(C.byref(prm), _ptr(views), _ptr(means3D), _ptr(cov6), _ptr(opac), _ptr(shs),
                                           _ptr(colors), _ptr(images), _ptr(depth), DEPTH_MODES[depth_mode], _ptr(radii),
                                           _ptr(ws), lay.total_bytes, stream)
    _lib.check(rc, "s360_forward")
    return images, radii, RasterState(prm, lay, ws), depth


class _RasterizeViews(torch.autograd.Function):

    @staticmethod
    def forward(ctx, means3D, means2D, shs, colors_precomp, opacities, cov6, views, cfg, mse_target=None):
        (h, w, sh_degree, shared_campos, max_instances, check, want_radii, cov9, sh_channel_major, keep_slots, depth_mode,
         defer_sh, mse_weight, mse_count, spherical, exchange, lean, mse_defer, atomic_grads, split_lists) = cfg
        if exchange is not None and (shs is None or not (shared_campos or int(views.shape[0]) == 1) or defer_sh):
            raise RuntimeError("exchange=: the chunked gradient exchange needs SH colours and views sharing one camera centre "
                               "(and replaces defer_sh)")
        ctx.exchange = exchange
        if spherical and (mse_target is not None or int(views.shape[0]) % 2):
            raise RuntimeError("spherical mode: views come in (camera, seam ghost) pairs; the fused loss epilogue is cube-face only")
        if not means3D.is_cuda:
            raise RuntimeError("means3D must live on the GPU (hip device); the rasteriser has no CPU path")
        with torch.cuda.device(means3D.device):
            m3 = _f32c(means3D, "means3D")
            c6 = _f32c(cov6, "cov3D_precomp")
            op = _f32c(opacities, "opacities").reshape(-1)
            sh = None if shs is None else _f32c(shs, "shs")
            col = None if colors_precomp is None else _f32c(colors_precomp, "colors_precomp")
            vw = _f32c(views, "views")
            p, v = int(m3.shape[0]), int(vw.shape[0])
            if v > _lib.S360_MAX_VIEWS:
                raise RuntimeError(f"at most {_lib.S360_MAX_VIEWS} views per call")
            prm = _lib.S360Params()
            prm.P, prm.V, prm.H, prm.W = p, v, int(h), int(w)
            prm.sh_degree = int(sh_degree)
            prm.M = 0 if sh is None else int(sh.shape[2] if sh_channel_major else sh.shape[1])
            if sh is not None and p == 0:
                prm.M = max(prm.M, (int(sh_degree) + 1) ** 2)
            needs_bwd = any(ctx.needs_input_grad[:6])
            hkey = _hint_key(m3.device, p, v, int(h), int(w), lean)
            _mirror(hkey)
            split_lists = split_decision(hkey, split_lists, v * ((int(h) + 15) // 16) * ((int(w) + 15) // 16) * 4) and not spherical
            prm.flags = (_lib.FLAG_SHARED_CAMPOS if (shared_campos or v == 1) else 0) | (
                _lib.FLAG_COV9 if cov9 else 0) | (_lib.FLAG_SH_CHANNEL_MAJOR if sh_channel_major else 0) | (
                0 if (needs_bwd or keep_slots) else _lib.FLAG_FORWARD_ONLY) | (
                _lib.FLAG_SH_DEG4_IGNORED if SH_DEG4_IGNORED else 0) | (_lib.FLAG_SPHERICAL if spherical else 0) | (
                _lib.FLAG_LEAN_LISTS if lean else 0) | (
                _lib.FLAG_DEFER_LOSS if (mse_defer and mse_target is not None and needs_bwd) else 0) | (
                _lib.FLAG_ATOMIC_GRADS if (atomic_grads and needs_bwd) else 0) | (
                _lib.FLAG_SPLIT_LISTS if (split_lists and not (atomic_grads and needs_bwd)) else 0) | (
                _lib.FLAG_COOP_WALK if coop_decision(hkey) else 0)
            prm.max_instances = int(max_instances) if max_instances else default_capacity(
                p, v, int(h), int(w), device=m3.device, lean=lean, lazy=(check != "sync"))
            prm.header_mirror = _mirror(hkey).data_ptr()
            prm.max_segments = default_segments(hkey) if split_lists else 0
            mse = None
            if mse_target is not None:
                tgt = _f32c(mse_target, "mse_target")
                if tuple(tgt.shape) != (v, 3, int(h), int(w)):
                    raise RuntimeError(f"mse_target must be [{v},3,{h},{w}], got {tuple(tgt.shape)}")
                n_mean = int(mse_count) if mse_count else v * 3 * int(h) * int(w)
                mse = (tgt, 2.0 * float(mse_weight) / n_mean)
            images, radii, state, depth = _forward_call(prm, vw, m3, c6, op, sh, col, want_radii, depth_mode, mse)
            if check == "sync" and state.overflowed():
                prm.max_instances = state.num_rendered()
                images, radii, state, depth = _forward_call(prm, vw, m3, c6, op, sh, col, want_radii, depth_mode, mse)
            if mse is not None:
                loss = state.mse_out[0]
                clipped_mse = state.mse_out[1:]
            else:
                loss = torch.empty(0, dtype=torch.float32, device=images.device)
                clipped_mse = loss
        ctx.set_materialize_grads(False)
        ctx.state = state
        ctx.holder = {}
        _RasterizeViews.last_holder = ctx.holder
        ctx.defer_sh = bool(defer_sh) and sh is not None
        ctx.has_means2D = means2D is not None
        ctx.depth_mode = depth_mode if depth is not None else None
        _RasterizeViews.last_state = state
        if radii is None:
            radii = torch.empty(0, dtype=torch.int32, device=images.device)
        if depth is None:
            depth = torch.empty(0, dtype=torch.float32, device=images.device)
            ctx.mark_non_differentiable(radii, depth, clipped_mse)
        else:
            ctx.mark_non_differentiable(radii, clipped_mse)
        ctx.save_for_backward(m3, c6, op, sh, col, vw)
        return images, radii, depth, loss, clipped_mse

    @staticmethod
    def backward(ctx, grad_images, _grad_radii, grad_depth, grad_loss, _grad_clipped):
        m3, c6, op, sh, col, vw = ctx.saved_tensors
        state: RasterState = ctx.state
        prm, lay = state.prm, state.layout
        dev = m3.device
        with torch.cuda.device(dev):
            g = None if grad_images is None else grad_images.detach().float()
            g_scale = None
            if grad_loss is not None and getattr(state, "d_images", None) is not None:
                if g is None:
                    g, g_scale = state.d_images, grad_loss.detach().float().reshape(1).contiguous()
                else:
                    g = g + state.d_images * grad_loss.detach().float()
            if g is None:
                n_img = prm.V // 2 if (prm.flags & _lib.FLAG_SPHERICAL) else prm.V
                g = torch.zeros((n_img, 3, prm.H, prm.W), dtype=torch.float32, device=dev)
            g = g.contiguous()
            gd, dm = None, 0
            if grad_depth is not None and ctx.depth_mode is not None:
                gd, dm = grad_depth.detach().float().contiguous(), DEPTH_MODES[ctx.depth_mode]
            p, v = prm.P, prm.V
            d_m3 = torch.empty((p, 3), dtype=torch.float32, device=dev)
            d_c6 = torch.empty_like(c6)
            d_op = torch.empty((p,), dtype=torch.float32, device=dev)
            need = ctx.needs_input_grad
            d_m2 = torch.empty((v, p, 3), dtype=torch.float32, device=dev) if (ctx.has_means2D and need[1]) else None
            d_sh = torch.empty_like(sh) if (sh is not None and need[2]) else None
            d_col = torch.empty((p, 3), dtype=torch.float32, device=dev) if (col is not None and need[3]) else None
            bws = torch.empty(lay.backward_bytes, dtype=torch.uint8, device=dev)
            stream = C.c_void_p(torch.cuda.current_stream(dev).cuda_stream)
            if ctx.exchange is not None:
                from . import distributed
                ex = ctx.exchange
                lib = _lib.lib()
                rc = lib.s360_backward_composite(C.byref(prm), _ptr(vw), _ptr(state.workspace), lay.total_bytes, _ptr(g), _ptr(g_scale),
                                                 _ptr(gd), dm, _ptr(bws), lay.backward_bytes, stream)
                _lib.check(rc, "s360_backward_composite")
                packed = torch.empty((p, 10), dtype=torch.float32, device=dev)
                rgb = torch.empty((p, 4), dtype=torch.float32, device=dev)
                rank = ex.rank()

                def produce(lo, hi):
                    _lib.check(lib.s360_backward_gaussians(C.byref(prm), _ptr(vw), _ptr(m3), _ptr(c6), _ptr(sh), _ptr(state.workspace),
                                                           lay.total_bytes, int(gd is not None), dm, lo, hi - lo, rank, _ptr(packed),
                                                           _ptr(d_m2), _ptr(rgb), _ptr(bws), lay.backward_bytes, stream),
                               "s360_backward_gaussians")

                slab = sh.shape[1] * sh.shape[2]

                def rebuild_sh(lo, hi, rgb_all, rep_all):
                    sub = _lib.S360Params()
                    C.memmove(C.byref(sub), C.byref(prm), C.sizeof(sub))
                    sub.P, sub.V = hi - lo, int(rep_all.shape[0])
                    st2 = C.c_void_p(torch.cuda.current_stream(dev).cuda_stream)
                    _lib.check(lib.s360_sh_backward(C.byref(sub), int(rgb_all.shape[0]), _ptr(rep_all.contiguous()),
                                                    C.c_void_p(m3.data_ptr() + 12 * lo), _ptr(rgb_all.contiguous()),
                                                    C.c_void_p(d_sh.data_ptr() + 4 * slab * lo), st2), "s360_sh_backward")

                def reduce_rows(lo, hi, rows):
                    _lib.check(lib.s360_reduce_unpack_gradients(_ptr(rows), int(rows.shape[0]), lo, hi - lo, int(c6.dim() == 3), _ptr(d_m3), _ptr(d_c6),
                                                                _ptr(d_op), C.c_void_p(torch.cuda.current_stream(dev).cuda_stream)),
                               "s360_reduce_unpack_gradients")

                form = distributed.exchange_chunked(p, packed, rgb, vw[0], produce, rebuild_sh if d_sh is not None else None,
                                                    n_chunks=ex.n_chunks, group=ex.group, group_gather=ex.group_gather,
                                                    force_collectives=getattr(ex, "force_collectives", False), mode=getattr(ex, "mode", None),
                                                    reduce_rows=reduce_rows)
                if form != "gather":
                    _lib.check(lib.s360_unpack_gradients(_ptr(packed), p, int(c6.dim() == 3), _ptr(d_m3), _ptr(d_c6), _ptr(d_op), stream),
                               "s360_unpack_gradients")
                if d_m2 is not None:
                    d_m2 = d_m2.sum(0) if v > 1 else d_m2[0]
                return d_m3, d_m2, d_sh, None, d_op.view(-1, 1), d_c6, None, None, None
            if ctx.defer_sh:
                d_rgb = torch.empty((p, 4), dtype=torch.float32, device=dev)
                rc = _lib.lib().s360_backward_split(
                    C.byref(prm), _ptr(vw), _ptr(m3), _ptr(c6), _ptr(op), _ptr(sh), _ptr(state.workspace), lay.total_bytes,
                    _ptr(g), _ptr(g_scale), _ptr(gd), dm, _ptr(d_m3), _ptr(d_m2), _ptr(d_c6), _ptr(d_op), _ptr(d_rgb),
                    _ptr(bws), lay.backward_bytes, stream)
                _lib.check(rc, "s360_backward_split")
                ctx.holder["deferred"] = _RasterizeViews.last_deferred = DeferredSH(prm, vw, m3, sh, d_rgb)
                if d_m2 is not None:
                    d_m2 = d_m2.sum(0) if v > 1 else d_m2[0]
                return d_m3, d_m2, None, None, d_op.view(-1, 1), d_c6, None, None, None
            rc = _lib.lib().s360_backward(
                C.byref(prm), _ptr(vw), _ptr(m3), _ptr(c6), _ptr(op), _ptr(sh), _ptr(col), _ptr(state.workspace),
                lay.total_bytes, _ptr(g), _ptr(g_scale), _ptr(gd), dm, _ptr(d_m3), _ptr(d_m2), _ptr(d_c6),
                _ptr(d_op), _ptr(d_sh), _ptr(d_col), _ptr(bws), lay.backward_bytes, stream)
            _lib.check(rc, "s360_backward")
        if d_m2 is not None:
            d_m2 = d_m2.sum(0) if v > 1 else d_m2[0]
        return d_m3, d_m2, d_sh, d_col, d_op.view(-1, 1), d_c6, None, None, None


class _RasterizeRaw(torch.autograd.Function):

    @staticmethod
    def forward(ctx, depths, opacities, raw, ctx_extrinsics, sh_rot, views, cfg, mse_target=None):
        (h, w, ch, cw, per_ray, smin, smax, eps, conv, diff_means, max_instances, check, depth_mode, mse_weight, mse_count, lean, mse_defer,
         split_lists, exchange) = cfg
        ctx.exchange = exchange
        if not depths.is_cuda:
            raise RuntimeError("depths must live on the GPU (hip device); the rasteriser has no CPU path")
        dev = depths.device
        with torch.cuda.device(dev):
            dep = _f32c(depths, "depths").reshape(-1)
            op = _f32c(opacities, "opacities").reshape(-1)
            rw = _f32c(raw, "raw_gaussians")
            ext = _f32c(ctx_extrinsics, "extrinsics").reshape(-1, 4, 4)
            rot = None if sh_rot is None else _f32c(sh_rot, "sh_rotation")
            vw = _f32c(views, "views")
            nv = int(ext.shape[0])
            p, v = int(dep.shape[0]), int(vw.shape[0])
            if rw.shape[-1] != 82 or rw.numel() != p * 82 or p % max(nv, 1) or (p // max(nv, 1)) != ch * cw * per_ray:
                raise RuntimeError("rasterize_raw: raw_gaussians must be [views * h * w * per_ray, 82] (degree-4 harmonics) matching depths / extrinsics")
            if v > _lib.S360_MAX_VIEWS:
                raise RuntimeError(f"at most {_lib.S360_MAX_VIEWS} views per call")
            needs_bwd = any(ctx.needs_input_grad[:3])
            hkey = _hint_key(dev, p, v, int(h), int(w), lean)
            _mirror(hkey)
            split_lists = split_decision(hkey, split_lists, v * ((int(h) + 15) // 16) * ((int(w) + 15) // 16) * 4)
            prm = _lib.S360Params()
            prm.P, prm.V, prm.H, prm.W, prm.sh_degree, prm.M = p, v, int(h), int(w), 4, 25
            prm.flags = _lib.FLAG_SHARED_CAMPOS | _lib.FLAG_RAW_INPUTS | (0 if needs_bwd else _lib.FLAG_FORWARD_ONLY) | (
                _lib.FLAG_LEAN_LISTS if lean else 0) | (_lib.FLAG_SPLIT_LISTS if split_lists else 0) | (
                _lib.FLAG_DEFER_LOSS if (mse_defer and mse_target is not None and needs_bwd) else 0) | (
                _lib.FLAG_COOP_WALK if coop_decision(hkey) else 0)
            prm.max_instances = int(max_instances) if max_instances else default_capacity(p, v, int(h), int(w), device=dev, lean=lean,
                                                                                          lazy=(check != "sync"))
            prm.header_mirror = _mirror(hkey).data_ptr()
            prm.max_segments = default_segments(hkey) if split_lists else 0
            rin = _lib.S360RawInputs(ext.data_ptr(), dep.data_ptr(), rw.data_ptr(), None if rot is None else rot.data_ptr(), nv, p // max(nv, 1),
                                     int(ch), int(cw), int(per_ray), int(conv), float(smin), float(smax), float(eps))
            means = torch.empty((p, 3), dtype=torch.float32, device=dev)
            cov6 = torch.empty((p, 6), dtype=torch.float32, device=dev)
            stream = C.c_void_p(torch.cuda.current_stream(dev).cuda_stream)

            def call():
                lay = _lib.layout(prm)
                ws = torch.empty(lay.total_bytes, dtype=torch.uint8, device=dev)
                images = torch.empty((v, 3, prm.H, prm.W), dtype=torch.float32, device=dev)
                depth = torch.empty((v, prm.H, prm.W), dtype=torch.float32, device=dev) if depth_mode is not None else None
                st = RasterState(prm, lay, ws)
                tgt = d_images = partials = loss_out = None
                gs = 0.0
                if mse_target is not None:
                    tgt = _f32c(mse_target, "mse_target")
                    n_mean = int(mse_count) if mse_count else v * 3 * int(h) * int(w)
                    gs = 2.0 * float(mse_weight) / n_mean
                    d_images = torch.empty_like(images)
                    partials = torch.empty((v * ((prm.H + 15) // 16) * ((prm.W + 15) // 16) * 4, 2), dtype=torch.float32, device=dev)
                    loss_out = torch.empty((1 + v,), dtype=torch.float32, device=dev)
                    st.d_images, st.mse_partials, st.mse_out = d_images, partials, loss_out
                rc = _lib.lib().s360_forward_raw(C.byref(prm), _ptr(vw), C.byref(rin), _ptr(op), _ptr(means), _ptr(cov6), _ptr(images), _ptr(depth),
                                                 DEPTH_MODES.get(depth_mode, 0), None, _ptr(tgt), C.c_float(gs), _ptr(d_images), _ptr(partials),
                                                 _ptr(loss_out), _ptr(ws), lay.total_bytes, stream)
                _lib.check(rc, "s360_forward_raw")
                return images, depth, st

            images, depth, state = call()
            if check == "sync" and state.overflowed():
                prm.max_instances = state.num_rendered()
                images, depth, state = call()
        ctx.set_materialize_grads(False)
        ctx.state, ctx.rin_cfg, ctx.depth_mode, ctx.diff_means = state, (nv, ch, cw, per_ray, conv, smin, smax, eps), depth_mode, bool(diff_means)
        ctx.in_shapes = (tuple(depths.shape), tuple(opacities.shape), tuple(raw.shape))
        _RasterizeViews.last_state = state
        loss = state.mse_out[0] if mse_target is not None else torch.empty(0, dtype=torch.float32, device=dev)
        clipped = state.mse_out[1:] if mse_target is not None else loss
        if depth is None:
            depth = torch.empty(0, dtype=torch.float32, device=dev)
            ctx.mark_non_differentiable(depth, clipped, means, cov6)
        else:
            ctx.mark_non_differentiable(clipped, means, cov6)
        ctx.save_for_backward(dep, op, rw, ext, rot, vw, means, cov6)
        return images, depth, loss, clipped, means, cov6

    @staticmethod
    def backward(ctx, grad_images, grad_depth, grad_loss, _gc, _gm, _gv):
        dep, op, rw, ext, rot, vw, means, cov6 = ctx.saved_tensors
        state: RasterState = ctx.state
        prm, lay = state.prm, state.layout
        nv, ch, cw, per_ray, conv, smin, smax, eps = ctx.rin_cfg
        dev = dep.device
        p = prm.P
        with torch.cuda.device(dev):
            g = None if grad_images is None else grad_images.detach().float()
            g_scale = None
            if grad_loss is not None and getattr(state, "d_images", None) is not None:
                if g is None:
                    g, g_scale = state.d_images, grad_loss.detach().float().reshape(1).contiguous()
                else:
                    g = g + state.d_images * grad_loss.detach().float()
            if g is None:
                g = torch.zeros((prm.V, 3, prm.H, prm.W), dtype=torch.float32, device=dev)
            g = g.contiguous()
            gd, dm = None, 0
            if grad_depth is not None and ctx.depth_mode is not None:
                gd, dm = grad_depth.detach().float().contiguous(), DEPTH_MODES[ctx.depth_mode]
            rin = _lib.S360RawInputs(ext.data_ptr(), dep.data_ptr(), rw.data_ptr(), None if rot is None else rot.data_ptr(), nv, p // max(nv, 1),
                                     int(ch), int(cw), int(per_ray), int(conv), float(smin), float(smax), float(eps))
            d_m3 = torch.empty((p, 3), dtype=torch.float32, device=dev)
            d_c6 = torch.empty((p, 6), dtype=torch.float32, device=dev)
            d_op = torch.empty((p,), dtype=torch.float32, device=dev)
            d_rgb = torch.empty((p, 4), dtype=torch.float32, device=dev)
            d_dep = torch.empty((p,), dtype=torch.float32, device=dev)
            d_raw = torch.empty((p, 82), dtype=torch.float32, device=dev)
            bws = torch.empty(lay.backward_bytes, dtype=torch.uint8, device=dev)
            stream = C.c_void_p(torch.cuda.current_stream(dev).cuda_stream)
            if ctx.exchange is not None:
# ... 170 lines not shown
```

Before: 1357 Msplats/s.

## Split long backward quadrant walks at a forward-checkpointed depth into two units

```diff
diff --git a/include/s360.h b/include/s360.h
--- a/include/s360.h
+++ b/include/s360.h
@@ -40,6 +40,10 @@
 #define S360_FLAG_RAW_INPUTS 1024u
 
 #define S360_FLAG_COOP_WALK 2048u
+
+#define S360_DEPTH_SPLIT_SHIFT 24
+#define S360_DEPTH_SPLIT_OFF 255u
+#define S360_DEPTH_SPLIT_DEFAULT 192u
 
 typedef struct S360View {
     float viewmatrix[16];
@@ -99,6 +103,8 @@
     size_t sh_jac;
     size_t surv;
     size_t surv_count;
+    size_t ck_k;
+    size_t ck_state;
     size_t part_c;
     size_t part_t;
     size_t part_e;
diff --git a/splatter360_amd/_lib.py b/splatter360_amd/_lib.py
--- a/splatter360_amd/_lib.py
+++ b/splatter360_amd/_lib.py
@@ -27,6 +27,8 @@
 FLAG_SPLIT_LISTS = 512
 FLAG_RAW_INPUTS = 1024
 FLAG_COOP_WALK = 2048
+DEPTH_SPLIT_SHIFT = 24
+DEPTH_SPLIT_OFF = 255
 ABI_VERSION = 24
 
 
@@ -41,7 +43,7 @@
     _fields_ = [(n, C.c_size_t) for n in (
         "total_bytes", "header", "tiles_touched", "vis_mask", "slot_base", "rec_a", "rec_b", "rec_c",
         "clamped", "depths", "tile_count", "slot_ticket", "merge_done", "seg_flag", "seg_arrive", "seg_arrive2", "tile_start", "tile_cursor", "chunk_start", "tile_order", "keys", "keys_alt", "list", "final_T", "n_contrib",
-        "tile_max_contrib", "strip_last", "slot_pair", "long_pairs", "rgbc", "sh_jac", "surv", "surv_count", "part_c", "part_t", "part_e", "part_l", "part_n", "seg_c", "seg_t", "seg_cnt", "seg_info", "geo7", "backward_bytes")]
+        "tile_max_contrib", "strip_last", "slot_pair", "long_pairs", "rgbc", "sh_jac", "surv", "surv_count", "ck_k", "ck_state", "part_c", "part_t", "part_e", "part_l", "part_n", "seg_c", "seg_t", "seg_cnt", "seg_info", "geo7", "backward_bytes")]
 
 
 class S360RawInputs(C.Structure):
diff --git a/splatter360_amd/csrc/s360_backward.hip b/splatter360_amd/csrc/s360_backward.hip
--- a/splatter360_amd/csrc/s360_backward.hip
+++ b/splatter360_amd/csrc/s360_backward.hip
@@ -731,7 +731,7 @@
         c.valid_words = (uint32_t*)((char*)bwd_workspace + (size_t)kp.cap * 4 * GREC * 4);
         c.order = c.valid_words + kp.cap;
     }
-    c.pairgrad = (float4*)((char*)(c.order + c.nt * 4) + 256 - ((uintptr_t)(c.order + c.nt * 4) & 255));
+    c.pairgrad = (float4*)((char*)(c.order + c.nt * 8) + 256 - ((uintptr_t)(c.order + c.nt * 8) & 255));
     c.seg_list = nullptr;
     c.n_slots = seg_slots_of(prm);
     if (kp.flags & S360_FLAG_SPLIT_LISTS) {
@@ -749,6 +749,8 @@
     const uint32_t* header = (const uint32_t*)(ws + L.header);
     const bool with_depth = dL_ddepth != nullptr;
     const uint32_t* surv_count = (const uint32_t*)(ws + L.surv_count);
+    const uint32_t* ck_k = (kp.flags & S360_FLAG_SPLIT_LISTS) || depth_split_k(kp.flags) == 0xFFFFFFFFu || kp.P <= 0 ? (const uint32_t*)nullptr
+                                                                                                                   : (const uint32_t*)(ws + L.ck_k);
     SegBwd sb{};
     if (c.seg_list) {
         sb.seg_flag = (const uint32_t*)(ws + L.seg_flag);
@@ -765,7 +767,7 @@
         ProfScope ps(PS_ORDER, st);
         hipLaunchKernelGGL(k_order_units, dim3(1 + 512), dim3(1024), 0, st, surv_count, c.order, c.nt * 4, c.valid_words, header, kp.cap,
                            (kp.flags & S360_FLAG_ATOMIC_GRADS) ? c.pairgrad : (float4*)nullptr, (const uint8_t*)(ws + L.vis_mask), kp.P, kp.V,
-                           (const uint32_t*)(ws + L.seg_cnt), (const uint32_t*)(ws + L.chunk_start), c.seg_list, (const uint2*)(ws + L.seg_info), sb);
+                           (const uint32_t*)(ws + L.seg_cnt), (const uint32_t*)(ws + L.chunk_start), c.seg_list, (const uint2*)(ws + L.seg_info), sb, ck_k);
     }
     {
         ProfScope ps(PS_RENDER_BWD, st);
@@ -775,9 +777,9 @@
                              dL_ddepth, c.part, (uint8_t*)c.valid_words, c.order, depth_mode,
                              (kp.flags & S360_FLAG_ATOMIC_GRADS) ? (float*)c.pairgrad : (float*)nullptr,
 #ifdef S360_DBG_TIMING
-                             (uint32_t*)(ws + L.keys_alt), c.seg_list ? &sb : (const SegBwd*)nullptr, sb.n_seg_blocks);
+                             (uint32_t*)(ws + L.keys_alt), c.seg_list ? &sb : (const SegBwd*)nullptr, sb.n_seg_blocks, ck_k, (const float4*)(ws + L.ck_state));
 #else
-                             (uint32_t*)nullptr, c.seg_list ? &sb : (const SegBwd*)nullptr, sb.n_seg_blocks);
+                             (uint32_t*)nullptr, c.seg_list ? &sb : (const SegBwd*)nullptr, sb.n_seg_blocks, ck_k, (const float4*)(ws + L.ck_state));
 #endif
     }
     S360_CHECK_LAUNCH();
diff --git a/splatter360_amd/csrc/s360_backward_em.hip b/splatter360_amd/csrc/s360_backward_em.hip
--- a/splatter360_amd/csrc/s360_backward_em.hip
+++ b/splatter360_amd/csrc/s360_backward_em.hip
@@ -7,12 +7,13 @@
                           const uint32_t* tile_start, const float4* surv, const uint32_t* surv_count, const uint2* slot_info,
                           const float* depths, const float* final_T, const uint32_t* n_contrib, const float* dL_dimages,
                           const float* dL_dimages_scale, const float* dL_ddepth, float4* part, uint8_t* valid, const uint32_t* order, int depth_mode,
-                          float* pairgrad_atomic, uint32_t* dbg, const SegBwd* sbp_host, uint32_t n_seg_blocks) {
+                          float* pairgrad_atomic, uint32_t* dbg, const SegBwd* sbp_host, uint32_t n_seg_blocks, const uint32_t* ck_k,
+                          const float4* ck_state) {
     const SegBwd sbv = sbp_host ? *sbp_host : SegBwd{};
 #define S360_LAUNCH_BWD(WD, SG)                                                                                                              \
-    hipLaunchKernelGGL((k_render_bwd_em<WD, SG>), dim3(n_units + (SG ? n_seg_blocks : 0u)), dim3(64), 0, st, kp, views, tile_start, surv, surv_count, \
+    hipLaunchKernelGGL((k_render_bwd_em<WD, SG>), dim3((!SG && ck_k ? 2 * n_units : n_units) + (SG ? n_seg_blocks : 0u)), dim3(64), 0, st, kp, views, tile_start, surv, surv_count, \
                        slot_info, depths, final_T, n_contrib, dL_dimages, dL_dimages_scale, dL_ddepth, part, valid, order, depth_mode,          \
-                       pairgrad_atomic, dbg, sbv, SG ? n_seg_blocks : 0u)
+                       pairgrad_atomic, dbg, sbv, SG ? n_seg_blocks : 0u, SG ? (const uint32_t*)nullptr : ck_k, ck_state)
     const bool seg = sbp_host != nullptr;
     if (with_depth) { if (seg) S360_LAUNCH_BWD(true, true); else S360_LAUNCH_BWD(true, false); }
     else { if (seg) S360_LAUNCH_BWD(false, true); else S360_LAUNCH_BWD(false, false); }
diff --git a/splatter360_amd/csrc/s360_bwd_em.h b/splatter360_amd/csrc/s360_bwd_em.h
--- a/splatter360_amd/csrc/s360_bwd_em.h
+++ b/splatter360_amd/csrc/s360_bwd_em.h
@@ -67,7 +67,7 @@
     const float* __restrict__ dL_dimages, const float* __restrict__ dL_dimages_scale, const float* __restrict__ dL_ddepth,
     float4* __restrict__ part,
     uint8_t* __restrict__ valid, const uint32_t* __restrict__ order, int depth_mode, float* __restrict__ pairgrad_atomic,
-    uint32_t* __restrict__ dbg, SegBwd sb, uint32_t n_seg_blocks) {
+    uint32_t* __restrict__ dbg, SegBwd sb, uint32_t n_seg_blocks, const uint32_t* __restrict__ ck_k, const float4* __restrict__ ck_state) {
     static_assert(SUB_W == 8, "entry-major backward assumes 8x8 quadrants");
     __shared__ __attribute__((aligned(16))) float s_gr[64], s_gg[64], s_gb[64], s_gd[64];
     __shared__ __attribute__((aligned(16))) float s_T[64], s_R[64];
@@ -80,8 +80,8 @@
 #ifdef S360_DBG_TIMING
     const long long t_begin = wall_clock64();
 #endif
-    uint32_t unit, n_surv, kseg = 0;
-    bool split_unit = false;
+    uint32_t unit, n_surv, kseg = 0, rec0 = 0;
+    bool split_unit = false, ck_front = false;
     size_t sli = 0;
     if (seg_blk) {
         if (sj >= sb.seg_list[0]) return;
@@ -95,7 +95,20 @@
         sli = su * 64;
     } else {
         unit = order ? order[blockIdx.x - n_seg_blocks] : blockIdx.x - n_seg_blocks;
+        if (!SEG && ck_k) {
+            ck_front = (unit >> 31) != 0u;
+            unit &= 0x7FFFFFFFu;
+        }
         n_surv = surv_count[unit];
+        if (!SEG && ck_k) {
+            const uint32_t ks = ck_k[unit];
+            if (ck_front) {
+                n_surv = ks;
+            } else if (ks) {
+                rec0 = ks;
+                n_surv -= ks;
+            }
+        }
         if (n_surv == 0) return;
         if (SEG && sb.seg_flag[unit] == 1u) {
             split_unit = true;
@@ -107,7 +120,7 @@
     const int ty = rem / kp.gx, tx = rem - ty * kp.gx;
     const int qx = tx * 16 + sub_ox(wave), qy = ty * 16 + sub_oy(wave);
     const uint32_t start = min(tile_start[t], kp.cap), end = min(tile_start[t + 1], kp.cap);
-    const float4* const sv = surv + 3 * ((size_t)4 * start + (size_t)wave * (end - start) + (size_t)kseg * SEG_LEN);
+    const float4* const sv = surv + 3 * ((size_t)4 * start + (size_t)wave * (end - start) + (size_t)kseg * SEG_LEN + rec0);
     const S360View& vw = views[view_of_image(kp, v)];
 
     int64_t top = (int64_t)n_surv - 1;
@@ -141,6 +154,14 @@
                 if (WITH_DEPTH) r0 = cb.w * pa.w + r0;
                 pb.y = r0;
             }
+            if (!SEG && ck_front) {
+                const float4* cs = ck_state + (size_t)unit * CK_F4;
+                const float4 cb = cs[lane];
+                pb.x = reinterpret_cast<const float*>(cs + 64)[lane];
+                float r0 = cb.z * pa.z + (cb.y * pa.y + cb.x * pa.x);
+                if (WITH_DEPTH) r0 = cb.w * pa.w + r0;
+                pb.y = r0;
+            }
         }
         s_gr[lane] = pa.x; s_gg[lane] = pa.y; s_gb[lane] = pa.z;
         if (WITH_DEPTH) s_gd[lane] = pa.w;
@@ -313,7 +334,7 @@
     }
 #ifdef S360_DBG_TIMING
     if (lane == 0 && dbg) {
-        const size_t di = seg_blk ? (size_t)sb.dbg_base + sb.seg_list[1 + sj] : (size_t)unit;
+        const size_t di = seg_blk ? (size_t)sb.dbg_base + sb.seg_list[1 + sj] : (size_t)unit + (ck_front ? gridDim.x / 2 : 0u);
         dbg[4 * di] = (uint32_t)t_begin;
         dbg[4 * di + 1] = (uint32_t)(wall_clock64() - t_begin);
         dbg[4 * di + 2] = n_surv;
@@ -329,6 +350,7 @@
                           const uint32_t* tile_start, const float4* surv, const uint32_t* surv_count, const uint2* slot_info,
                           const float* depths, const float* final_T, const uint32_t* n_contrib, const float* dL_dimages,
                           const float* dL_dimages_scale, const float* dL_ddepth, float4* part, uint8_t* valid, const uint32_t* order, int depth_mode,
-                          float* pairgrad_atomic, uint32_t* dbg, const SegBwd* sbp_host, uint32_t n_seg_blocks);
-
-}
+                          float* pairgrad_atomic, uint32_t* dbg, const SegBwd* sbp_host, uint32_t n_seg_blocks, const uint32_t* ck_k,
+                          const float4* ck_state);
+
+}
diff --git a/splatter360_amd/csrc/s360_device.h b/splatter360_amd/csrc/s360_device.h
--- a/splatter360_amd/csrc/s360_device.h
+++ b/splatter360_amd/csrc/s360_device.h
@@ -58,6 +58,12 @@
 #define S360_HDR_TILES_DONE 24
 #define S360_HDR_NLONG 25
 #define S360_SEG_CLAIM 0x80000000u
+#define S360_HDR_DEPTH_SPLIT 26
+constexpr int CK_F4 = 80;
+__host__ __device__ __forceinline__ uint32_t depth_split_k(uint32_t flags) {
+    const uint32_t f = flags >> S360_DEPTH_SPLIT_SHIFT;
+    return f == S360_DEPTH_SPLIT_OFF ? 0xFFFFFFFFu : (f ? 16u * f : S360_DEPTH_SPLIT_DEFAULT);
+}
 #define S360_HDR_SEGBUFS 32
 
 inline int device_cu_count() {
@@ -495,26 +501,35 @@
 }
 
 template <int THREADS>
-__device__ __forceinline__ void order_quadrants_body(const uint32_t* __restrict__ weight, uint32_t* __restrict__ order, int nt) {
+__device__ __forceinline__ void order_quadrants_body(const uint32_t* __restrict__ weight, uint32_t* __restrict__ order, int nt,
+                                                     const uint32_t* __restrict__ ck_k) {
     __shared__ uint32_t s_max;
     __shared__ uint32_t s_cnt[64];
     __shared__ uint32_t s_base[64];
     if (threadIdx.x == 0) s_max = 1;
     if (threadIdx.x < 64) s_cnt[threadIdx.x] = 0;
     __syncthreads();
+    const int nv = ck_k ? 2 * nt : nt;
+    auto vweight = [&](int i) -> uint32_t {
+        uint4 w;
+        if (i < nt) {
+            w = reinterpret_cast<const uint4*>(weight)[i];
+            if (ck_k) {
+                const uint4 k = reinterpret_cast<const uint4*>(ck_k)[i];
+                w.x -= min(k.x, w.x); w.y -= min(k.y, w.y); w.z -= min(k.z, w.z); w.w -= min(k.w, w.w);
+            }
+        } else {
+            w = reinterpret_cast<const uint4*>(ck_k)[i - nt];
+        }
+        return max(max(w.x, w.y), max(w.z, w.w));
+    };
     uint32_t mx = 0;
-    for (int i = threadIdx.x; i < nt; i += THREADS) {
-        const uint4 w = reinterpret_cast<const uint4*>(weight)[i];
-        mx = max(mx, max(max(w.x, w.y), max(w.z, w.w)));
-    }
+    for (int i = threadIdx.x; i < nv; i += THREADS) mx = max(mx, vweight(i));
     mx = wave_max_u32(mx);
     if ((threadIdx.x & 63) == 0) atomicMax(&s_max, mx);
     __syncthreads();
     const uint32_t wmax = s_max;
-    for (int i = threadIdx.x; i < nt; i += THREADS) {
-        const uint4 w = reinterpret_cast<const uint4*>(weight)[i];
-        atomicAdd(&s_cnt[63 - (uint32_t)(((uint64_t)max(max(w.x, w.y), max(w.z, w.w)) * 63) / wmax)], 1u);
-    }
+    for (int i = threadIdx.x; i < nv; i += THREADS) atomicAdd(&s_cnt[63 - (uint32_t)(((uint64_t)vweight(i) * 63) / wmax)], 1u);
     __syncthreads();
     if (threadIdx.x == 0) {
         uint32_t run = 0;
@@ -524,15 +539,15 @@
         }
     }
     __syncthreads();
-    const uint32_t full = (uint32_t)nt / 8u * 8u, tail = (uint32_t)nt - full;
-    for (int i = threadIdx.x; i < nt; i += THREADS) {
-        const uint4 w = reinterpret_cast<const uint4*>(weight)[i];
-        const uint32_t b = 63 - (uint32_t)(((uint64_t)max(max(w.x, w.y), max(w.z, w.w)) * 63) / wmax);
+    const uint32_t full = (uint32_t)nv / 8u * 8u, tail = (uint32_t)nv - full;
+    for (int i = threadIdx.x; i < nv; i += THREADS) {
+        const uint32_t b = 63 - (uint32_t)(((uint64_t)vweight(i) * 63) / wmax);
         const uint32_t r = atomicAdd(&s_base[b], 1u);
+        const uint32_t u0 = i < nt ? 4u * (uint32_t)i : (4u * (uint32_t)(i - nt)) | 0x80000000u;
 #pragma unroll
         for (uint32_t q = 0; q < 4; ++q) {
             const uint32_t slot = r < full ? (r / 8u) * 32u + q * 8u + (r & 7u) : full * 4u + q * tail + (r - full);
-            order[slot] = 4u * (uint32_t)i + q;
+            order[slot] = u0 + q;
         }
     }
 }
@@ -609,7 +624,8 @@
                                                      uint32_t cap, float4* __restrict__ pairgrad_atomic,
                                                      const uint8_t* __restrict__ vis_mask, int P, int V,
                                                      const uint32_t* __restrict__ seg_cnt, const uint32_t* __restrict__ chunk_start,
-                                                     uint32_t* __restrict__ seg_list, const uint2* __restrict__ seg_info, SegBwdPod sbpod) {
+                                                     uint32_t* __restrict__ seg_list, const uint2* __restrict__ seg_info, SegBwdPod sbpod,
+                                                     const uint32_t* __restrict__ ck_k) {
     if (blockIdx.x == 2 && seg_list) {
         if (threadIdx.x == 0) *reinterpret_cast<SegBwdPod*>(seg_list - 32) = sbpod;
         __shared__ uint32_t s_n;
@@ -647,8 +663,8 @@
         return;
     }
     if (!order) return;
-    order_quadrants_body<1024>(weight, order, n / 4);
-}
-
-
-}
+    order_quadrants_body<1024>(weight, order, n / 4, ck_k);
+}
+
+
+}
diff --git a/splatter360_amd/csrc/s360_forward.hip b/splatter360_amd/csrc/s360_forward.hip
--- a/splatter360_amd/csrc/s360_forward.hip
+++ b/splatter360_amd/csrc/s360_forward.hip
@@ -740,6 +740,7 @@
         *reinterpret_cast<SegBufs*>(header + S360_HDR_SEGBUFS) = sg_in;
         header[S360_HDR_SPLIT] = 0;
         header[6] = header[7] = 0;
+        header[S360_HDR_DEPTH_SPLIT] = 0;
         if (header_mirror) __hip_atomic_store(header_mirror, (unsigned long long)carry | ((unsigned long long)(carry > cap ? 1u : 0u) << 32) |
                                                              ((unsigned long long)ccarry << 33),
                                               __ATOMIC_RELAXED, __HIP_MEMORY_SCOPE_SYSTEM);
@@ -1561,7 +1562,7 @@
                                                       uint32_t* __restrict__ dbg, const float* __restrict__ depths,
                                                       float* __restrict__ depth_maps, int depth_mode, MseEp ep,
                                                       const uint32_t* __restrict__ tile_order, float4* __restrict__ surv,
-                                                      uint32_t* __restrict__ surv_count, uint32_t* __restrict__ hdr_loss,
+                                                      uint32_t* __restrict__ surv_count, uint32_t* __restrict__ ck_k, float4* ck_state, uint32_t* __restrict__ hdr_depth_split, uint32_t* __restrict__ hdr_loss,
                                                       const SegBufs* __restrict__ sgp, const uint32_t* __restrict__ chunk_start,
                                                       unsigned long long* __restrict__ cand_mirror, int nt, const uint32_t* __restrict__ list_all,
                                                       const float* __restrict__ depths_all) {
@@ -1702,6 +1703,8 @@
     bool done = !inside;
     float4* const sv = surv ? surv + 3 * ((size_t)4 * start + (size_t)wave * (end - start)) : nullptr;
     uint32_t scount = 0, sv_cnt = 0, sv_rel = 0;
+    const uint32_t ck_min = !SPLIT && ck_k ? depth_split_k(kp.flags) : 0xFFFFFFFFu;
+    uint32_t ck = 0;
     unsigned long long sv_m = 0ull;
     const int vcam = view_of_image(kp, v);
     const float inv_scale = WITH_DEPTH ? 1.0f / views[vcam].scale : 0.f;
@@ -1732,6 +1735,12 @@
                     break;
                 }
             }
+        }
+        if (!SPLIT && ck == 0u && scount >= ck_min) {
+            ck = scount;
+            float4* o = ck_state + (size_t)(4 * t + wave) * CK_F4;
+            o[lane] = make_float4(C01.x, C01.y, C2D.x, C2D.y);
+            reinterpret_cast<float*>(o + 64)[lane] = T;
         }
         const float4 ea = na, eb = nb;
         float ez = 0.f;
@@ -1942,10 +1951,23 @@
         }
     }
     const uint32_t wm = wave_max_u32(inside ? last : 0u);
+    const uint32_t n_replay = wm ? sv_cnt + (uint32_t)__popcll(sv_m & ((2ull << (wm - 1u - sv_rel)) - 1ull)) : 0u;
     if (lane == 0) {
         strip_last[4 * t + wave] = wm;
         if (wm) atomicMax(&tile_max_contrib[t], wm);
-        if (surv_count) surv_count[4 * t + wave] = wm ? sv_cnt + (uint32_t)__popcll(sv_m & ((2ull << (wm - 1u - sv_rel)) - 1ull)) : 0u;
+        if (surv_count) surv_count[4 * t + wave] = n_replay;
+    }
+    if (!SPLIT && ck_k) {
+        const bool two = ck != 0u && n_replay >= ck + (ck_min >> 1);
+        if (two) {
+            float4* o = ck_state + (size_t)(4 * t + wave) * CK_F4;
+            const float4 c = o[lane];
+            o[lane] = make_float4(C01.x - c.x, C01.y - c.y, C2D.x - c.z, C2D.y - c.w);
+        }
+        if (lane == 0) {
+            ck_k[4 * t + wave] = two ? ck : 0u;
+            if (two) atomicAdd(&hdr_depth_split[0], 1u);
+        }
     }
 #ifdef S360_DBG_TIMING
     if (lane == 0) {
@@ -2268,6 +2290,8 @@
     out->sh_jac = take((size_t)(prm->P > 0 ? prm->P : 1) * 36);
     out->surv = take(fwd_only ? 16 : cap * 4 * 48);
     out->surv_count = take(nt * 4 * 4);
+    out->ck_k = take(fwd_only ? 16 : nt * 4 * 4);
+    out->ck_state = take(fwd_only ? 16 : nt * 4 * (size_t)CK_F4 * 16);
     {
         const bool split = (prm->flags & S360_FLAG_SPLIT_LISTS) != 0;
         const size_t ns = split ? seg_slots_of(prm) : 1, nl = ns * 4 * 64;
@@ -2284,7 +2308,7 @@
     out->geo7 = take((prm->flags & S360_FLAG_RAW_INPUTS) && !fwd_only ? (size_t)(prm->P > 0 ? prm->P : 1) * 28 : 16);
     out->total_bytes = o;
     const bool atomic = (prm->flags & S360_FLAG_ATOMIC_GRADS) != 0;
-    out->backward_bytes = (atomic ? 0 : align_up(cap * 4 * (size_t)(16 * S360_PREC_F4)) + align_up(cap * 4)) + align_up(nt * 4 * 4) + 512 +
+    out->backward_bytes = (atomic ? 0 : align_up(cap * 4 * (size_t)(16 * S360_PREC_F4)) + align_up(cap * 4)) + align_up(nt * 8 * 4) + 512 +
                           align_up(np * 48) + align_up((size_t)(prm->P > 0 ? prm->P : 1) * 16) + 256 +
                           ((prm->flags & S360_FLAG_SPLIT_LISTS) ? align_up((seg_slots_of(prm) * 4 + 64 + 32) * 4) + 256 : 0);
     return S360_OK;
@@ -2480,6 +2504,9 @@
         const bool training = !(kp.flags & S360_FLAG_FORWARD_ONLY);
         float4* surv = training ? (float4*)(ws + L.surv) : nullptr;
         uint32_t* surv_count = training ? (uint32_t*)(ws + L.surv_count) : nullptr;
+        const bool cks = training && kp.P > 0 && !(kp.flags & S360_FLAG_SPLIT_LISTS) && depth_split_k(kp.flags) != 0xFFFFFFFFu;
+        uint32_t* ck_k = cks ? (uint32_t*)(ws + L.ck_k) : nullptr;
+        float4* ck_state = (float4*)(ws + L.ck_state);
 #ifdef S360_DBG_TIMING
         uint32_t* dbg = (uint32_t*)keys_alt;
 #else
@@ -2498,7 +2525,7 @@
 #define S360_LAUNCH_RENDER(WD, SP)                                                                                                         \
     hipLaunchKernelGGL((k_render<WD, SP>), SP ? dim3(nt + S360_P1_GRID + S360_P2_GRID) : rgrid, rblock, 0, st, kp, views, tile_start, list, recA, recB, recC, images, final_T, n_contrib,      \
                        tile_max_contrib, strip_last, dbg, depths, depth_maps, depth_mode, ep, kp.P > 0 ? tile_order : (const uint32_t*)nullptr, \
-                       surv, surv_count, hdr_loss, sgp, chunk_start, cand, nt, list, depths)
+                       surv, surv_count, ck_k, ck_state, header + S360_HDR_DEPTH_SPLIT, hdr_loss, sgp, chunk_start, cand, nt, list, depths)
         if (depth_maps) { if (split) S360_LAUNCH_RENDER(true, true); else S360_LAUNCH_RENDER(true, false); }
         else { if (split) S360_LAUNCH_RENDER(false, true); else S360_LAUNCH_RENDER(false, false); }
 #undef S360_LAUNCH_RENDER
diff --git a/splatter360_amd/rasterizer.py b/splatter360_amd/rasterizer.py
--- a/splatter360_amd/rasterizer.py
+++ b/splatter360_amd/rasterizer.py
@@ -45,6 +45,20 @@
 DROPIN_CHECK = os.environ.get("S360_DROPIN_CHECK", "sync")
 if DROPIN_CHECK not in ("sync", "lazy"):
     raise RuntimeError(f"S360_DROPIN_CHECK must be 'sync' or 'lazy', got {DROPIN_CHECK!r}")
+
+DEPTH_SPLIT_K = None
+
+
+def _depth_split_bits() -> int:
+    k = DEPTH_SPLIT_K
+    if k is None:
+        return 0
+    if k == 0:
+        return _lib.DEPTH_SPLIT_OFF << _lib.DEPTH_SPLIT_SHIFT
+    if k % 16 or not 16 <= k <= 16 * 254:
+        raise RuntimeError(f"DEPTH_SPLIT_K must be None, 0 or a multiple of 16 in [16, 4064], got {k!r}")
+    return (k // 16) << _lib.DEPTH_SPLIT_SHIFT
+
 
 DEPTH_MODES = {"depth": 0, "disparity": 1, "relative_disparity": 2, "log": 3}
 
@@ -242,6 +256,8 @@
             final_T=self._arr(l.final_T, p.V * p.H * p.W, torch.float32).view(p.V, p.H, p.W),
             n_contrib=self._arr(l.n_contrib, p.V * p.H * p.W, torch.int32).view(p.V, p.H, p.W),
             tile_max_contrib=self._arr(l.tile_max_contrib, nt, torch.int32),
+            surv_count=self._arr(l.surv_count, nt * 4, torch.int32),
+            ck_k=self._arr(l.ck_k, 4 if (p.flags & _lib.FLAG_FORWARD_ONLY) else nt * 4, torch.int32),
             seg_flag=self._arr(l.seg_flag, nt * 4, torch.int32),
         )
 
@@ -283,6 +299,9 @@
 
     def split_errors(self) -> int:
         return int(self.header()[7].item())
+
+    def depth_split_quadrants(self) -> int:
+        return int(self.header()[26].item())
 
     def mopup_items(self) -> int:
         n = int(self.header()[6].item())
@@ -387,7 +406,7 @@
                 _lib.FLAG_DEFER_LOSS if (mse_defer and mse_target is not None and needs_bwd) else 0) | (
                 _lib.FLAG_ATOMIC_GRADS if (atomic_grads and needs_bwd) else 0) | (
                 _lib.FLAG_SPLIT_LISTS if (split_lists and not (atomic_grads and needs_bwd)) else 0) | (
-                _lib.FLAG_COOP_WALK if coop_decision(hkey) else 0)
+                _lib.FLAG_COOP_WALK if coop_decision(hkey) else 0) | _depth_split_bits()
             prm.max_instances = int(max_instances) if max_instances else default_capacity(
                 p, v, int(h), int(w), device=m3.device, lean=lean, lazy=(check != "sync"))
             prm.header_mirror = _mirror(hkey).data_ptr()
@@ -554,7 +573,7 @@
             prm.flags = _lib.FLAG_SHARED_CAMPOS | _lib.FLAG_RAW_INPUTS | (0 if needs_bwd else _lib.FLAG_FORWARD_ONLY) | (
                 _lib.FLAG_LEAN_LISTS if lean else 0) | (_lib.FLAG_SPLIT_LISTS if split_lists else 0) | (
                 _lib.FLAG_DEFER_LOSS if (mse_defer and mse_target is not None and needs_bwd) else 0) | (
-                _lib.FLAG_COOP_WALK if coop_decision(hkey) else 0)
+                _lib.FLAG_COOP_WALK if coop_decision(hkey) else 0) | _depth_split_bits()
             prm.max_instances = int(max_instances) if max_instances else default_capacity(p, v, int(h), int(w), device=dev, lean=lean,
                                                                                           lazy=(check != "sync"))
             prm.header_mirror = _mirror(hkey).data_ptr()
```

Measured after the change: 1327 Msplats/s. -2.3%, worse.
